# AHartmaier/pyLabFEA

Hardware: AMD Instinct MI355X
Metric: integration-point updates/sec (wall-clock per load step in ms_per_step) (higher is better)
Workload: dtype f64

## Files before the change

### include/plfx.h

```cpp
#ifndef PLFX_H
#define PLFX_H

#include <stddef.h>
#include <stdint.h>

#ifdef __cplusplus
extern "C" {
#endif

typedef struct plfx_ctx plfx_ctx;

enum {
    PLFX_ELASTIC = 0,
    PLFX_HILL6 = 1,
    PLFX_PRINC3 = 2,
    PLFX_SVC6 = 3,
    PLFX_TRESCA = 4,
    PLFX_BARLAT = 5,
    PLFX_SVC3 = 6,
    PLFX_SVC_WH = 7,
    PLFX_SVC6_COLS = 8
};

enum {
// ... 29 lines not shown
int plfx_create(int device, plfx_ctx **out);
void plfx_destroy(plfx_ctx *ctx);
const char *plfx_last_error(plfx_ctx *ctx);
const char *plfx_version(void);
int plfx_device_count(void);
int plfx_device_info(plfx_ctx *ctx, char *name, int len, int *cus, int64_t *hbm_bytes);
void *plfx_stream(plfx_ctx *ctx);
int plfx_sync(plfx_ctx *ctx);

int plfx_set_materials(plfx_ctx *ctx, int nmat, const plfx_material *mats);

int plfx_seq_batch(plfx_ctx *ctx, int mat, int n, const double *sig, double *seq);
int plfx_fgrad_batch(plfx_ctx *ctx, int mat, int n, const double *sig, double *fgrad);
int plfx_fgrad_seq_batch(plfx_ctx *ctx, int mat, int n, const double *sig, const double *seq, double *fgrad);
int plfx_yf_batch(plfx_ctx *ctx, int mat, int n, const double *sig, const double *epl, double *yf);
int plfx_full_yf_batch(plfx_ctx *ctx, int mat, int n, const double *sig, const double *epl,
                       const double *ld, double *yf, int32_t *status);
int plfx_response_batch(plfx_ctx *ctx, int n, const int32_t *mat_id, const double *sig,
                        const double *epl, const double *deps, double *fy, double *sig_out,
                        double *depl, double *ct , int32_t *nsteps);
int plfx_set_response_maxit(plfx_ctx *ctx, int maxit);
int plfx_sig_princ_host(int n, const double *sig, double *sp);
int plfx_eig3_host(int n, const double *sig, double *w, double *V);
int plfx_response_batch_kh(plfx_ctx *ctx, int n, const int32_t *mat_id, const double *sig, const double *epl,
                           const double *deps, const double *khard_in, double *fy, double *sig_out, double *depl,
                           double *ct, int32_t *nsteps, double *khard_out);
int plfx_fgrad_batch_wh(plfx_ctx *ctx, int mat, int n, const double *sig, const double *epl, double *fgrad, double *khard_raw);
int plfx_hessian_batch(plfx_ctx *ctx, int mat, int n, const double *sig, const double *epl, double *hess);
int plfx_yield_scale(plfx_ctx *ctx, int mat, int n, const double *su, const double *epl, const double *x0, double *x,
                     int32_t *status);
int plfx_flow_curve(plfx_ctx *ctx, int mat, int n, const double *su, const double *epl0, int max_steps, double depl,
                    double epl_max, double predictor, double *x, double *epl, double *yf, double *hk, int32_t *nsteps,
                    int32_t *status);
int plfx_flow_info(plfx_ctx *ctx, int64_t *launches);

int plfx_load_path(plfx_ctx *ctx, int mat, int n, int K, const double *dload, int shared, const int32_t *control,
                   const double *sig0, const double *epl0, const int32_t *tex_id, int maxit, int newton, double stol,
                   double eps_cap, double *sig, double *epl, double *deps, double *fy, int32_t *nsteps, int32_t *newton_out,
                   int32_t *ksteps, int32_t *status, double *ct);
int plfx_load_path_info(plfx_ctx *ctx, int64_t *launches);

int plfx_committee_yf(plfx_ctx *ctx, int nmem, const int32_t *mats, const double *scale, int n, const double *su, double *yf,
                      double *mean, double *var, int32_t *best, double *best_var);
int plfx_committee_info(plfx_ctx *ctx, int64_t *launches, int32_t *staged_members);

int plfx_tex_svc_set(plfx_ctx *ctx, int nsv, int tdim, const double *sv, const double *dual, double intercept, double gamma,
                     const double *mean, const double *scale, int dev_only);
int plfx_tex_svc_yf(plfx_ctx *ctx, int n, const double *sig, int ntex, const double *tex, const int32_t *tex_id, double *yf);
int plfx_tex_svc_yield_scale(plfx_ctx *ctx, int nray, const double *su, int ntex, const double *tex, const double *x0, double *x,
                             int32_t *status);
int plfx_tex_svc_info(plfx_ctx *ctx, int *nsv, int *tdim, int64_t *yf_launches, int64_t *ray_launches, int *staged);
int plfx_tex_svc_fgrad(plfx_ctx *ctx, int n, const double *sig, int ntex, const double *tex, const int32_t *tex_id, double *grad);
int plfx_tex_svc_full_yf(plfx_ctx *ctx, int n, const double *sig, int ntex, const double *tex, const int32_t *tex_id, double *f,
                         int32_t *status);
int plfx_tex_svc_response(plfx_ctx *ctx, int mat, int n, const double *sig, const double *epl, const double *deps, int ntex,
                          const double *tex, const int32_t *tex_id, int maxit, double *fy, double *sig_out, double *depl,
                          double *ct, int32_t *nsteps);
int plfx_tex_svc_flow_info(plfx_ctx *ctx, int64_t *fgrad_launches, int64_t *full_yf_launches, int64_t *response_launches);

int plfx_gen_structured(int NX, int NY, int32_t *conn, int32_t *noleft, int32_t *noright, int32_t *nobot, int32_t *notop);

int plfx_set_mesh(plfx_ctx *ctx, int nel, int nnode, const int32_t *conn, const int32_t *mat_id,
                  const double *lxy, double thick, int planestress, int el_begin, int el_end);
int plfx_set_mesh_structured(plfx_ctx *ctx, int NX, int NY, const int32_t *mat_col, const int32_t *mat_el, const double *dx_col,
                             double dy, double thick, int planestress, int el_begin, int el_end);
int plfx_pattern_selftest(int nx, int ny);
int plfx_set_grid(plfx_ctx *ctx, int nx, int ny);
int plfx_set_precond(plfx_ctx *ctx, int kind, double omega, int nu);
int plfx_precond_info(plfx_ctx *ctx, int *kind_in_use, int *levels);
int plfx_precond_apply(plfx_ctx *ctx, const double *r, double *z);
int plfx_precond_bench(plfx_ctx *ctx, int reps, double *us_per_cycle, double *us_coarse);
int plfx_solve_fallbacks(plfx_ctx *ctx, int64_t *count);
int plfx_indefinite_info(plfx_ctx *ctx, int64_t *solves, int64_t *by_minres_surrogate, int64_t *by_gmres,
                         int64_t *surrogates_built, int64_t *elements_shifted);
int plfx_set_operator(plfx_ctx *ctx, int kind);
int plfx_matvec(plfx_ctx *ctx, const double *x, double *y);
int plfx_operator_info(plfx_ctx *ctx, int *matrix_free, int *levels_matrix_free);
int plfx_reuse_info(plfx_ctx *ctx, int *assemblies, int *bc_applications, int *solves);
int plfx_predict_info(plfx_ctx *ctx, int64_t *applied, int64_t *skipped, int64_t *rejected);
int plfx_sweep_info(plfx_ctx *ctx, int64_t *sweeps, int64_t *tangents_rewritten);
int plfx_sweep_launch_info(plfx_ctx *ctx, int64_t *heavy_skipped, int64_t *heavy_recovered);
int plfx_bc_info(plfx_ctx *ctx, int64_t *rhs_rows_only, int64_t *dinv_kept, int64_t *dinv_refreshed, int64_t *du_early);
int plfx_short_info(plfx_ctx *ctx, int64_t *dinv_deferred, int64_t *dinv_formed_late, int64_t *d_kept, int64_t *spec_merged);
int plfx_dead_store_info(plfx_ctx *ctx, int64_t *armed_sweeps, int64_t *tangents_rewritten_in_armed_sweeps,
                         int64_t *test_only_starts, int64_t *test_only_retries);
enum {
    PLFX_PLANE_ON = 0,
    PLFX_PLANE_NEVER_ON = 1,
    PLFX_PLANE_SWITCH = 2,
    PLFX_PLANE_SHARDED = 3,
    PLFX_PLANE_MATERIALS = 4,
    PLFX_PLANE_STATE_SET = 5,
    PLFX_PLANE_TANGENT_SET = 6
};
int plfx_plane_info(plfx_ctx *ctx, int *mode_on, int64_t *plane_sweeps, int64_t *plane_updates, int *switched_off_by);
enum {
    PLFX_MG_TAIL_NONE = 0,
    PLFX_MG_TAIL_GENERIC = 1,
    PLFX_MG_TAIL_LDS = 2,
    PLFX_MG_TAIL_MF = 3,
    PLFX_MG_TAIL_MF_RAGGED = 4
};
enum {
    PLFX_MG_COARSE_DENSE = 0,
    PLFX_MG_COARSE_CHEBY = 1,
    PLFX_MG_COARSE_PCG = 2
};
int plfx_mg_info(plfx_ctx *ctx, int max_levels, int *levels, int *dims, double *ratios, int *matfree, int *tail_level,
                 int *tail_kernel, int *coarse_solver, int *cheby_steps, double *cheby_kappa, int *march);
int plfx_svc_info(plfx_ctx *ctx, int *row_materials, int *thread_materials, int64_t *row_launches, int64_t *thread_launches);
int plfx_get_bmat(plfx_ctx *ctx, int e, double *B);
int plfx_get_kel(plfx_ctx *ctx, int e, double *Kel);

int plfx_state_get(plfx_ctx *ctx, int which, double *out);
int plfx_state_set(plfx_ctx *ctx, int which, const double *in);
int plfx_state_reset(plfx_ctx *ctx);
int plfx_gather(plfx_ctx *ctx, int which, int n, const int32_t *idx, double *out);

enum {
    PLFX_FIELD_STRAIN1 = 0,
    PLFX_FIELD_STRAIN2 = 1,
    PLFX_FIELD_STRAIN12 = 2,
    PLFX_FIELD_STRESS1 = 3,
    PLFX_FIELD_STRESS2 = 4,
    PLFX_FIELD_STRESS12 = 5,
    PLFX_FIELD_PLASTIC1 = 6,
    PLFX_FIELD_PLASTIC2 = 7,
    PLFX_FIELD_PLASTIC12 = 8,
    PLFX_FIELD_SEQ = 9,
    PLFX_FIELD_SEQJ2 = 10,
    PLFX_FIELD_PEEQ = 11,
    PLFX_FIELD_ETOT = 12,
    PLFX_FIELD_UX = 13,
    PLFX_FIELD_UY = 14
};
int plfx_element_fields(plfx_ctx *ctx, int nsel, const int32_t *sel, double *out, double *range);

int plfx_assemble(plfx_ctx *ctx);
int plfx_get_csr(plfx_ctx *ctx, int64_t *nnz, int32_t *rowptr, int32_t *colidx, double *val);

int plfx_apply_bc(plfx_ctx *ctx, int n, const int32_t *presc_idx, const double *du_presc,
                  const double *w, const double *fext);
int plfx_set_bc_plan(plfx_ctx *ctx, int nseg, const int32_t *seg_len, const int32_t *idx);
int plfx_apply_bc_plan(plfx_ctx *ctx, const double *seg_val, const double *fext, int *inconsistent_entry);
int plfx_solve(plfx_ctx *ctx, double rtol, int maxit, int warm, int *iters, double *relres);

int plfx_sweep(plfx_ctx *ctx, int nit, int *changed, int *conv);
int plfx_set_wh_mode(plfx_ctx *ctx, int sequential);
int plfx_wh_info(plfx_ctx *ctx, int *sequential_in_use, int64_t *sweeps, int64_t *passes,
                 int64_t *unresolved );
int plfx_wh_carry(plfx_ctx *ctx, int mat, const double *set, double *get);
int plfx_scf_stats(plfx_ctx *ctx, const double *sld, double *sum, double *sumsq_c, double *minv,
                   int64_t *count, double mean_in, int pass);
int plfx_scf_all(plfx_ctx *ctx, const double *sld, int64_t *count, double *minv, double *sum, double *sumsq_c);
int plfx_update_state(plfx_ctx *ctx);
int plfx_set_finish_set(plfx_ctx *ctx, int n, const int32_t *idx);
int plfx_finish_step(plfx_ctx *ctx, double *u_at , double *f_at , double *sums18);
int plfx_global_sums(plfx_ctx *ctx, double *out18);

typedef struct plfx_step {
    int32_t il, nonlin, has_nodeset, warm, maxit;
    int32_t defer_slot;
    double rtol;
    double bcl0[2], bcb0[2];
    double max_dbcr[2], max_dbct[2], max_dbcn[2];
    double bcr[2], bct[2], bcn[2];
// ... 65 lines not shown
```

### pylabfea_amd/_lib.py

```python
import ctypes as C
import os

import numpy as np

_HERE = os.path.dirname(os.path.abspath(__file__))
LIB_PATH = os.environ.get('PLFX_LIB', os.path.join(_HERE, 'libplfx.so'))

ELASTIC, HILL6, PRINC3, SVC6, TRESCA, BARLAT, SVC3, SVC_WH, SVC6_COLS = 0, 1, 2, 3, 4, 5, 6, 7, 8

ST_SIG, ST_EPS, ST_EPL, ST_RES_SIG, ST_RES_DEPL, ST_ELSTIFF, ST_U, ST_F, ST_DU, ST_FYN, ST_MAXSTEPS, ST_KHARD = range(12)

FIELD_NAMES = ('strain1', 'strain2', 'strain12', 'stress1', 'stress2', 'stress12', 'plastic1', 'plastic2', 'plastic12',
               'seq', 'seqJ2', 'peeq', 'etot', 'ux', 'uy')
FIELD_ID = {n: i for i, n in enumerate(FIELD_NAMES)}

T_SWEEP, T_SPMV, T_CGUPD, T_ASSEMBLE, T_VCYCLE, T_SMOOTH, T_SWEEP_HEAVY, T_COMM = range(8)


class PlfxError(RuntimeError):
    pass


class CMaterial(C.Structure):
    _fields_ = [('kind', C.c_int32), ('sdim', C.c_int32), ('CV', C.c_double * 36),
                ('E', C.c_double), ('nu', C.c_double), ('sy', C.c_double), ('khard', C.c_double),
                ('hill', C.c_double * 6), ('drucker', C.c_double), ('nsv', C.c_int32),
                ('nfeat', C.c_int32), ('dev_only', C.c_int32), ('_pad', C.c_int32),
                ('gamma', C.c_double), ('intercept', C.c_double), ('scale_seq', C.c_double),
                ('sv', C.c_void_p), ('dual', C.c_void_p), ('barlat', C.c_double * 18),
                ('barlat_exp', C.c_double), ('barlat_normal', C.c_int32), ('_pad2', C.c_int32),
                ('scale_wh', C.c_double)]


SYMBOLS = [
    'plfx_create', 'plfx_destroy', 'plfx_last_error', 'plfx_version', 'plfx_device_count', 'plfx_device_info',
    'plfx_stream', 'plfx_sync', 'plfx_set_materials', 'plfx_seq_batch', 'plfx_fgrad_batch',
    'plfx_yf_batch', 'plfx_full_yf_batch', 'plfx_response_batch', 'plfx_set_mesh', 'plfx_get_bmat',
    'plfx_get_kel', 'plfx_state_get', 'plfx_state_set', 'plfx_state_reset', 'plfx_gather',
    'plfx_assemble', 'plfx_get_csr', 'plfx_apply_bc', 'plfx_solve', 'plfx_sweep', 'plfx_scf_stats',
    'plfx_update_state', 'plfx_global_sums', 'plfx_comm_unique_id', 'plfx_comm_init',
    'plfx_timing_get', 'plfx_timing_reset', 'plfx_timing_enable', 'plfx_set_grid', 'plfx_set_precond',
    'plfx_precond_info', 'plfx_set_operator', 'plfx_operator_info', 'plfx_gen_structured', 'plfx_reuse_info', 'plfx_timing_select', 'plfx_finish_fetch', 'plfx_sweep_info', 'plfx_matvec', 'plfx_set_bc_plan', 'plfx_apply_bc_plan',
    'plfx_set_finish_set', 'plfx_finish_step', 'plfx_scf_all', 'plfx_comm_info', 'plfx_comm_init_callback',
    'plfx_set_bc_sources',
    'plfx_load_step', 'plfx_set_strip', 'plfx_strip_info', 'plfx_allreduce_host',
    'plfx_response_batch_kh', 'plfx_fgrad_batch_wh', 'plfx_timing_sample', 'plfx_solve_fallbacks', 'plfx_comm_selftest',
    'plfx_indefinite_info', 'plfx_pattern_selftest', 'plfx_precond_bench', 'plfx_set_wh_mode', 'plfx_wh_info', 'plfx_wh_carry', 'plfx_set_mesh_structured',
    'plfx_svc_info', 'plfx_fgrad_seq_batch', 'plfx_precond_apply', 'plfx_predict_info',
    'plfx_set_response_maxit', 'plfx_sig_princ_host', 'plfx_eig3_host',
    'plfx_svc_fit_batch', 'plfx_svc_decision_batch', 'plfx_svc_fit_wide', 'plfx_hessian_batch',
    'plfx_svr_fit_batch', 'plfx_svr_predict_multi', 'plfx_set_svr_flow', 'plfx_svr_flow_info',
    'plfx_sweep_launch_info', 'plfx_element_fields', 'plfx_bc_info', 'plfx_yield_scale',
    'plfx_committee_yf', 'plfx_committee_info',
    'plfx_tex_svc_set', 'plfx_tex_svc_yf', 'plfx_tex_svc_yield_scale', 'plfx_tex_svc_info',
    'plfx_tex_svc_fgrad', 'plfx_tex_svc_full_yf', 'plfx_tex_svc_response', 'plfx_tex_svc_flow_info',
    'plfx_flow_curve', 'plfx_flow_info', 'plfx_load_path', 'plfx_load_path_info',
    'plfx_dead_store_info', 'plfx_plane_info', 'plfx_short_info',
    'plfx_set_svc_cols', 'plfx_mg_info',
    'plfx_set_svc_textures', 'plfx_set_element_textures', 'plfx_response_batch_tid', 'plfx_full_yf_batch_tid',
    'plfx_svc_textures_info',
]

_lib = None


def load():
    global _lib
    if _lib is not None:
        return _lib
    if not os.path.exists(LIB_PATH):
        raise PlfxError('libplfx.so not found at %s - build it first (__graft_entry__.build()); '
                        'pylabfea_amd has no CPU fallback' % LIB_PATH)
    lib = C.CDLL(LIB_PATH)
    lib.plfx_last_error.restype = C.c_char_p
    lib.plfx_version.restype = C.c_char_p
    lib.plfx_stream.restype = C.c_void_p
    lib.plfx_destroy.restype = None
    _lib = lib
    return lib


class CStep(C.Structure):
    _fields_ = [('il', C.c_int32), ('nonlin', C.c_int32), ('has_nodeset', C.c_int32), ('warm', C.c_int32),
                ('maxit', C.c_int32), ('defer_slot', C.c_int32), ('rtol', C.c_double),
                ('bcl0', C.c_double * 2), ('bcb0', C.c_double * 2),
                ('max_dbcr', C.c_double * 2), ('max_dbct', C.c_double * 2), ('max_dbcn', C.c_double * 2),
                ('bcr', C.c_double * 2), ('bct', C.c_double * 2), ('bcn', C.c_double * 2),
                ('bcr0', C.c_double * 2), ('bct0', C.c_double * 2), ('bcn0', C.c_double * 2),
                ('sld', C.c_double * 6),
                ('dbcr', C.c_double * 2), ('dbct', C.c_double * 2), ('dbcn', C.c_double * 2),
                ('scale_bc', C.c_double),
                ('nit', C.c_int32), ('nconv', C.c_int32), ('nsweeps', C.c_int32), ('nsolves', C.c_int32),
                ('soft_fail', C.c_int32), ('inconsistent_entry', C.c_int32),
                ('its', C.c_int32 * 40), ('relres', C.c_double * 40)]


def device_count():
    return int(load().plfx_device_count())


def _dp(a):
    return a.ctypes.data_as(C.c_void_p) if a is not None else None


def _f64(a):
    return np.ascontiguousarray(a, dtype=np.float64)


def _i32(a):
    return np.ascontiguousarray(a, dtype=np.int32)


def gen_structured(NX, NY):
    lib = load()
    conn = np.empty((NX * NY, 4), dtype=np.int32)
    le, ri = np.empty(NY + 1, dtype=np.int32), np.empty(NY + 1, dtype=np.int32)
    bo, to = np.empty(NX + 1, dtype=np.int32), np.empty(NX + 1, dtype=np.int32)
    rc = lib.plfx_gen_structured(int(NX), int(NY), _dp(conn), _dp(le), _dp(ri), _dp(bo), _dp(to))
    if rc:
        raise PlfxError('plfx_gen_structured(%d, %d): error %d' % (NX, NY, rc))
    return conn, le, ri, bo, to


def sig_princ_host(sig):
    lib = load()
    s = _f64(sig).reshape(-1, 6)
    sp = np.empty((len(s), 3))
    rc = lib.plfx_sig_princ_host(len(s), _dp(s), _dp(sp))
    if rc < 0:
        raise PlfxError('plfx_sig_princ_host: error %d' % rc)
    return sp


def eig3_host(sig):
    lib = load()
    s = _f64(sig).reshape(-1, 6)
    w, V = np.empty((len(s), 3)), np.empty((len(s), 3, 3))
    rc = lib.plfx_eig3_host(len(s), _dp(s), _dp(w), _dp(V))
    if rc < 0:
        raise PlfxError('plfx_eig3_host: error %d' % rc)
# ... 514 lines not shown
            try:
                return self.response(sig, epl, deps, mat_id, khard_in, return_khard, tex_id=tex_id)
            finally:
                self.set_response_maxit(50)
        sig = _f64(sig).reshape(-1, 6)
        n = len(sig)
        epl = _f64(epl).reshape(-1, 6)
        deps = _f64(deps).reshape(-1, 6)
        mid = None if mat_id is None else _i32(mat_id)
        fy = np.empty(n)
        so = np.empty((n, 6))
        dp = np.empty((n, 6))
        ct = np.empty((n, 36))
        ns = np.empty(n, dtype=np.int32)
        if khard_in is not None or return_khard:
            kin = None if khard_in is None else _f64(np.broadcast_to(np.asarray(khard_in, dtype=float), (n,)).copy())
            kout = np.empty(n)
            self._chk(self.lib.plfx_response_batch_kh(self.h, n, _dp(mid), _dp(sig), _dp(epl), _dp(deps), _dp(kin),
                                                      _dp(fy), _dp(so), _dp(dp), _dp(ct), _dp(ns), _dp(kout)))
            if return_khard:
                return fy, so, dp, ct, ns, kout
            return fy, so, dp, ct, ns
        if tex_id is not None:
            tid = _i32(tex_id).reshape(-1)
            if len(tid) != n:
                raise ValueError('response: one texture row per point expected')
            self._chk(self.lib.plfx_response_batch_tid(self.h, n, _dp(mid), _dp(sig), _dp(epl), _dp(deps),
                                                       _dp(fy), _dp(so), _dp(dp), _dp(ct), _dp(ns), _dp(tid)))
            return fy, so, dp, ct, ns
        self._chk(self.lib.plfx_response_batch(self.h, n, _dp(mid), _dp(sig), _dp(epl), _dp(deps),
                                               _dp(fy), _dp(so), _dp(dp), _dp(ct), _dp(ns)))
        return fy, so, dp, ct, ns

    def set_mesh(self, conn, mat_id, lxy, nnode, thick, planestress, el_begin=0, el_end=None):
        conn = _i32(conn).reshape(-1, 4)
        nel = len(conn)
        mat_id = _i32(mat_id)
        lxy = _f64(lxy).reshape(nel, 2)
        if el_end is None:
            el_end = nel
        self._chk(self.lib.plfx_set_mesh(self.h, nel, int(nnode), _dp(conn), _dp(mat_id), _dp(lxy),
                                         C.c_double(thick), int(bool(planestress)), int(el_begin),
                                         int(el_end)))
        self.nel = nel
        self.nel_owned = el_end - el_begin
        self.ndof = 2 * int(nnode)

    def set_mesh_structured(self, NX, NY, dx_col, dy, thick, planestress, mat_col=None, mat_el=None, el_begin=0, el_end=None):
        nel = int(NX) * int(NY)
        dx = _f64(dx_col).reshape(int(NX))
        mc = None if mat_col is None else _i32(mat_col).reshape(int(NX))
        me = None if mat_el is None else _i32(mat_el).reshape(nel)
        if el_end is None:
            el_end = nel
        self._chk(self.lib.plfx_set_mesh_structured(self.h, int(NX), int(NY), _dp(mc), _dp(me), _dp(dx), C.c_double(dy),
                                                    C.c_double(thick), int(bool(planestress)), int(el_begin), int(el_end)))
        self.nel = nel
        self.nel_owned = el_end - el_begin
        self.ndof = 2 * (int(NX) + 1) * (int(NY) + 1)

    def set_grid(self, nx, ny):
        self._chk(self.lib.plfx_set_grid(self.h, int(nx), int(ny)))

    def sweep_info(self):
        a, b = C.c_int64(), C.c_int64()
        self._chk(self.lib.plfx_sweep_info(self.h, C.byref(a), C.byref(b)))
        return a.value, b.value

    def sweep_launch_info(self):
        a, b = C.c_int64(), C.c_int64()
        self._chk(self.lib.plfx_sweep_launch_info(self.h, C.byref(a), C.byref(b)))
        return a.value, b.value

    def bc_info(self):
        a, b, r, d = C.c_int64(), C.c_int64(), C.c_int64(), C.c_int64()
        self._chk(self.lib.plfx_bc_info(self.h, C.byref(a), C.byref(b), C.byref(r), C.byref(d)))
        return a.value, b.value, r.value, d.value

    def short_info(self):
        a, b, r, d = C.c_int64(), C.c_int64(), C.c_int64(), C.c_int64()
        self._chk(self.lib.plfx_short_info(self.h, C.byref(a), C.byref(b), C.byref(r), C.byref(d)))
        return a.value, b.value, r.value, d.value

    def dead_store_info(self):
        a, b, r, d = C.c_int64(), C.c_int64(), C.c_int64(), C.c_int64()
        self._chk(self.lib.plfx_dead_store_info(self.h, C.byref(a), C.byref(b), C.byref(r), C.byref(d)))
        return a.value, b.value, r.value, d.value

    PLANE_OFF_REASONS = ('on', 'no state reset yet', 'switch', 'sharded', 'materials', 'state_set', 'tangent set')

    def plane_info(self):
        on, a, b, why = C.c_int(), C.c_int64(), C.c_int64(), C.c_int()
        self._chk(self.lib.plfx_plane_info(self.h, C.byref(on), C.byref(a), C.byref(b), C.byref(why)))
        return bool(on.value), a.value, b.value, why.value

    MG_TAIL_KERNELS = ('none', 'tail', 'tail_lds', 'tail_mf', 'tail_mf_ragged')
    MG_COARSE_SOLVERS = ('dense', 'cheby', 'pcg')

    def mg_info(self):
        cap = 64
        nl, tl, tk, cs, st, ma = (C.c_int() for _ in range(6))
        kap = C.c_double()
        dims, rat, mf = np.zeros((cap, 2), dtype=np.int32), np.zeros((cap, 2)), np.zeros(cap, dtype=np.int32)
        self._chk(self.lib.plfx_mg_info(self.h, cap, C.byref(nl), _dp(dims), _dp(rat), _dp(mf), C.byref(tl), C.byref(tk),
                                        C.byref(cs), C.byref(st), C.byref(kap), C.byref(ma)))
        n = min(nl.value, cap)
        return {'levels': [(int(dims[l, 0]), int(dims[l, 1]), float(rat[l, 0]), float(rat[l, 1]), bool(mf[l])) for l in range(n)],
                'tail_level': tl.value, 'tail_kernel': self.MG_TAIL_KERNELS[tk.value],
                'coarse_solver': self.MG_COARSE_SOLVERS[cs.value], 'cheby_steps': st.value, 'cheby_kappa': kap.value,
                'march': bool(ma.value)}

    def svc_info(self):
        a, b, r, t = C.c_int(), C.c_int(), C.c_int64(), C.c_int64()
        self._chk(self.lib.plfx_svc_info(self.h, C.byref(a), C.byref(b), C.byref(r), C.byref(t)))
        return a.value, b.value, r.value, t.value

    def reuse_info(self):
        a, b, s = C.c_int(), C.c_int(), C.c_int()
        self._chk(self.lib.plfx_reuse_info(self.h, C.byref(a), C.byref(b), C.byref(s)))
        return a.value, b.value, s.value

    def predict_info(self):
        a, b, r = C.c_int64(), C.c_int64(), C.c_int64()
        self._chk(self.lib.plfx_predict_info(self.h, C.byref(a), C.byref(b), C.byref(r)))
        return a.value, b.value, r.value

    def set_precond(self, kind, omega=0., nu=0):
        self._chk(self.lib.plfx_set_precond(self.h, int(kind), C.c_double(omega), int(nu)))

    def precond_info(self):
        k = C.c_int()
        lv = C.c_int()
        self._chk(self.lib.plfx_precond_info(self.h, C.byref(k), C.byref(lv)))
        return k.value, lv.value

    def precond_apply(self, r):
        r = _f64(r).reshape(-1)
        z = np.empty_like(r)
        self._chk(self.lib.plfx_precond_apply(self.h, _dp(r), _dp(z)))
        return z

    def precond_bench(self, reps=100):
        a, b = C.c_double(), C.c_double()
        self._chk(self.lib.plfx_precond_bench(self.h, int(reps), C.byref(a), C.byref(b)))
        return a.value, b.value

    def set_wh_mode(self, sequential):
        self._chk(self.lib.plfx_set_wh_mode(self.h, 1 if sequential else 0))

    def wh_info(self):
        a, b, c_, u = C.c_int(), C.c_int64(), C.c_int64(), C.c_int64()
        self._chk(self.lib.plfx_wh_info(self.h, C.byref(a), C.byref(b), C.byref(c_), C.byref(u)))
        self.wh_unresolved = u.value
        return bool(a.value), b.value, c_.value

    def wh_unresolved_sweeps(self):
        self.wh_info()
        return self.wh_unresolved

    def wh_carry(self, mat, value=None):
        g = C.c_double()
        sv = None if value is None else C.byref(C.c_double(float(value)))
        self._chk(self.lib.plfx_wh_carry(self.h, int(mat), sv, C.byref(g)))
        return g.value

    def solve_fallbacks(self):
# ... 246 lines not shown
```

### pylabfea_amd/csrc/plfx.hip

```cpp
#define PLFX_UNIT_CONTEXT
#define PLFX_UNIT_MESH
#define PLFX_UNIT_OPERATOR
#include "plfx_host.hpp"
#include "plfx_mg.hpp"

namespace plfx {
namespace host {

typedef struct { char internal[128]; } ncclUniqueId;
typedef int (*fn_ncclGetUniqueId)(ncclUniqueId *);
typedef int (*fn_ncclCommInitRank)(ncclComm_t *, int, ncclUniqueId, int);
typedef int (*fn_ncclAllReduce)(const void *, void *, size_t, int, int, ncclComm_t, hipStream_t);
typedef int (*fn_ncclCommDestroy)(ncclComm_t);
typedef int (*fn_ncclSend)(const void *, size_t, int, int, ncclComm_t, hipStream_t);
typedef int (*fn_ncclRecv)(void *, size_t, int, int, ncclComm_t, hipStream_t);
typedef int (*fn_ncclGroup)(void);
struct Rccl {
    void *h = nullptr;
    fn_ncclGetUniqueId GetUniqueId = nullptr;
    fn_ncclCommInitRank CommInitRank = nullptr;
    fn_ncclAllReduce AllReduce = nullptr;
    fn_ncclCommDestroy CommDestroy = nullptr;
    fn_ncclSend Send = nullptr;
    fn_ncclRecv Recv = nullptr;
// ... 383 lines not shown
    dfree(c->eps);
    dfree(c->res_sig);
    dfree(c->res_depl);
    dfree(c->fld_buf);
    dfree(c->fld_part);
    c->fld_cap = 0;
    tan_free(c);
    dfree(c->Mel);
    dfree(c->fyn);
    dfree(c->scf_hh);
    dfree(c->kh_el);
    dfree(c->kh_out); dfree(c->kh_new); dfree(c->wh_snap_el); dfree(c->wh_snap_M); dfree(c->wh_snap_ms);
    dfree(c->kh_touch); dfree(c->wh_bmax); dfree(c->wh_cnt);
    c->kh_out_valid = false;
    dfree(c->max_steps);
    dfree(c->scf_mult);
    dfree(c->heavy_list);
    dfree(c->u);
    dfree(c->f);
    dfree(c->du);
    dfree(c->rhs);
    dfree(c->dinv);
    dfree(c->diag);
    dfree(c->is_presc);
    dfree(c->dup);
    dfree(c->wv);
    dfree(c->fext);
    dfree(c->x);
    dfree(c->r);
    dfree(c->z);
    dfree(c->q);
    dfree(c->pred_x);
    dfree(c->pred_d);
    c->pred_valid = c->pred_d_kept = false;
    for (auto &b : c->gm_blk) dfree(b);
    c->gm_blk.clear();
    c->gm_m = 0;
    dfree(c->gm_part);
    dfree(c->gm_part2);
    dfree(c->gm_red);
    dfree(c->gm_coef);
    dfree(c->p[0]);
    dfree(c->p[1]);
    for (auto &L : c->mg) {
        if (!L.owned) continue;
        dfree(L.col);
        dfree(L.contrib);
        dfree(L.cls0);
        dfree(L.val);
        dfree(L.diag);
        dfree(L.dinv);
        dfree(L.Mel);
        dfree(L.x);
        dfree(L.b);
    }
    for (auto &L : c->mg) {
        dfree(L.t);
        dfree(L.res);
        dfree(L.ainv);
    }
    c->mg.clear();
    dfree(c->mg_cls);
    dfree(c->mg_dev);
    dfree(c->dtab);
    dfree(c->Mop);
    dfree(c->colr);
    c->grid_ok = false;
    c->val_valid = false;
    c->mg_tail = -1;
    c->gx = c->gy = 0;
    c->assembled = c->bc_set = false;
    c->M_dirty = true;
    c->x_is_du = false;
    c->bc_valid = false;
    c->bc_idx.clear();
    c->plan.valid = false;
    dfree(c->fin_idx);
    dfree(c->fin_dev);
    c->fin_n = 0;
    dfree(c->kw);
    dfree(c->bc_rows);
    c->bc_nrows = 0;
    c->rhs_rows_ok = c->dinv_ok = c->dinv_late = false;
    dfree(c->tex_ids);
    c->htex_ids.clear();
    c->tex_ids_ok = false;
}

int ensure_tmp(plfx_ctx *c, size_t n)
{
    if (n <= c->tmp_cap) return 0;
    dfree(c->idx_tmp);
    dfree(c->val_tmp);
    int rc = dalloc(c, &c->idx_tmp, n);
    if (rc) return rc;
    rc = dalloc(c, &c->val_tmp, 4 * n);
    if (rc) return rc;
    c->tmp_cap = n;
    return 0;
}

int march_env()
{
    static const int v = getenv("PLFX_MARCH") ? atoi(getenv("PLFX_MARCH")) : -1;
    return v;
}
bool march_pcg(const plfx_ctx *c) { return matfree(c) && march_env() != 0 && !c->op.colr; }
bool march_mg(const plfx_ctx *c)
{
    if (!matfree(c) || march_env() == 0) return false;
    return march_env() == 1 || (size_t)c->nnode * 112 > ((size_t)192 << 20);
}
bool tail_mf(const plfx_ctx *c)
{
    return matfree(c) && c->mg_tail_T > 0 && c->mg_tail_E > 0 && c->mg_nu == 2 && !c->mg.empty() && c->mg.back().ainv;
}

void launch_spmv_plain(plfx_ctx *c, const double *in, double *out, CgScalars *sc)
{
    LAUNCH_OP2(k_spmv, 0, matfree(c), dim3(c->grid_nodes), c->op, 0, c->nnode, (const double2 *)in, nullptr, nullptr,
               (double2 *)out, nullptr, nullptr, nullptr, 0, nullptr, sc, 0, 0, 0);
}

int plain_spmv(plfx_ctx *c, const double *in, double *out)
{
    launch_spmv_plain(c, in, out, nullptr);
    HIPCHK(c, hipGetLastError());
    return 0;
}

int allreduce(plfx_ctx *c, void *dev, size_t count, int nccl_dtype, int nccl_op, const char *what)
{
    c->last_coll = what;
    c->n_coll++;
    if (c->comm) {
        EvPair *ev;
        tim_begin(c, 7, &ev);
        const int rcn = g_rccl.AllReduce(dev, dev, count, nccl_dtype, nccl_op, c->comm, c->stream);
        tim_end(c, ev);
        if (rcn != 0) return fail(c, PLFX_ERR_HIP, "ncclAllReduce(%s) failed", what);
        return 0;
    }
    if (c->host_ar) {
        const size_t bytes = count * (nccl_dtype == NCCL_INT32 ? 4 : 8);
        if (c->host_ar_buf.size() < bytes) c->host_ar_buf.resize(bytes);
        HIPCHK(c, hipMemcpyAsync(c->host_ar_buf.data(), dev, bytes, hipMemcpyDeviceToHost, c->stream));
        HIPCHK(c, stream_sync(c));
        if (c->host_ar(c->host_ar_user, c->host_ar_buf.data(), count, nccl_dtype == NCCL_INT32 ? 1 : 0,
                       nccl_op == NCCL_MIN ? 3 : 0) != 0)
            return fail(c, PLFX_ERR_HIP, "host all-reduce callback failed (%s)", what);
        HIPCHK(c, hipMemcpyAsync(dev, c->host_ar_buf.data(), bytes, hipMemcpyHostToDevice, c->stream));
        HIPCHK(c, stream_sync(c));
        return 0;
    }
    return 0;
}

int sync_M(plfx_ctx *c)
{
    if (!comm_active(c) || !c->sharded) return 0;
    if (c->strip.on) return strip_sync_M(c);
    hipLaunchKernelGGL(k_zero_foreign_M, dim3(grid_for((size_t)6 * c->nel_total)), dim3(BLOCK), 0, c->stream,
                       c->nel_total, c->e0, c->e0 + c->nel, c->Mel);
    HIPCHK(c, hipGetLastError());
    return allreduce(c, c->Mel, (size_t)6 * c->nel_total, NCCL_FLOAT64, NCCL_SUM, "M");
}


bool strip_coll(const plfx_ctx *c)
{
    static const bool force = getenv("PLFX_STRIP_FORCE_COLL") && atoi(getenv("PLFX_STRIP_FORCE_COLL")) != 0;
    return c->nranks > 1 || (force && (c->comm || c->host_ar));
}

int part_allreduce(plfx_ctx *c, double *p, size_t n)
{
    if (!c->strip.on || !strip_coll(c)) return 0;
    c->strip.n_part++;
    return allreduce(c, p, n, NCCL_FLOAT64, NCCL_SUM, "partial sums");
}

int halo_refresh(plfx_ctx *c, double *v)
{
    auto &S = c->strip;
    if (!S.on || !strip_coll(c)) return 0;
    const int nyn = c->gy + 1;
    const size_t n = (size_t)S.W * nyn * 2;
    double *sendL = v + (size_t)2 * (S.oc0 + 1) * nyn, *recvL = v + (size_t)2 * (S.oc0 - S.W) * nyn;
    double *sendR = v + (size_t)2 * (S.oc1 - S.W) * nyn, *recvR = v + (size_t)2 * (S.oc1 + 1) * nyn;
    S.n_halo++;
    c->last_coll = "halo refresh (ncclSend / ncclRecv with the strip neighbours)";
    c->n_coll++;
    if (c->comm) {
        if (!g_rccl.Send || !g_rccl.Recv || !g_rccl.GroupStart || !g_rccl.GroupEnd)
            return fail(c, PLFX_ERR_UNSUPPORTED, "this RCCL has no ncclSend/ncclRecv");
        EvPair *ev;
        tim_begin(c, 7, &ev);
        int rc = g_rccl.GroupStart();
        if (!rc && S.has_left) {
            rc = g_rccl.Send(sendL, n, NCCL_FLOAT64, c->rank - 1, c->comm, c->stream);
            if (!rc) rc = g_rccl.Recv(recvL, n, NCCL_FLOAT64, c->rank - 1, c->comm, c->stream);
        }
        if (!rc && S.has_right) {
            rc = g_rccl.Send(sendR, n, NCCL_FLOAT64, c->rank + 1, c->comm, c->stream);
            if (!rc) rc = g_rccl.Recv(recvR, n, NCCL_FLOAT64, c->rank + 1, c->comm, c->stream);
        }
        const int rc2 = g_rccl.GroupEnd();
        tim_end(c, ev);
        if (rc || rc2) return fail(c, PLFX_ERR_HIP, "halo refresh (ncclSend/ncclRecv) failed: %d / %d", rc, rc2);
        return 0;
    }
    if (c->host_ar) {
        S.hbuf.assign(2 * n, 0.);
        if (S.has_left) HIPCHK(c, hipMemcpyAsync(S.hbuf.data(), sendL, 8 * n, hipMemcpyDeviceToHost, c->stream));
        if (S.has_right) HIPCHK(c, hipMemcpyAsync(S.hbuf.data() + n, sendR, 8 * n, hipMemcpyDeviceToHost, c->stream));
        HIPCHK(c, stream_sync(c));
        if (c->host_ar(c->host_ar_user, S.hbuf.data(), 2 * n, 0, 100) != 0)
            return fail(c, PLFX_ERR_HIP, "host halo-exchange callback failed");
        if (S.has_left) HIPCHK(c, hipMemcpyAsync(recvL, S.hbuf.data(), 8 * n, hipMemcpyHostToDevice, c->stream));
        if (S.has_right) HIPCHK(c, hipMemcpyAsync(recvR, S.hbuf.data() + n, 8 * n, hipMemcpyHostToDevice, c->stream));
        HIPCHK(c, stream_sync(c));
    }
    return 0;
}

int strip_sync_M(plfx_ctx *c)
{
    auto &S = c->strip;
    if (!S.on || !strip_coll(c)) return 0;
    const int ny = c->gy;
    const size_t n = (size_t)S.W * ny, tot = (size_t)c->nel_total;
    double *M = c->Mel;
    const size_t sL = (size_t)S.oc0 * ny, rL = (size_t)(S.oc0 - S.W) * ny, sR = (size_t)(S.oc1 - S.W) * ny, rR = (size_t)S.oc1 * ny;
    S.n_gen++;
    c->last_coll = "stiffness generators of the halo columns (ncclSend / ncclRecv with the strip neighbours)";
    c->n_coll++;
    if (c->comm) {
        if (!g_rccl.Send || !g_rccl.Recv || !g_rccl.GroupStart || !g_rccl.GroupEnd)
            return fail(c, PLFX_ERR_UNSUPPORTED, "this RCCL has no ncclSend/ncclRecv");
        EvPair *ev;
        tim_begin(c, 7, &ev);
        int rc = g_rccl.GroupStart();
        for (int k = 0; k < 6 && !rc; k++) {
            if (S.has_left) {
                rc = g_rccl.Send(M + k * tot + sL, n, NCCL_FLOAT64, c->rank - 1, c->comm, c->stream);
                if (!rc) rc = g_rccl.Recv(M + k * tot + rL, n, NCCL_FLOAT64, c->rank - 1, c->comm, c->stream);
            }
            if (!rc && S.has_right) {
                rc = g_rccl.Send(M + k * tot + sR, n, NCCL_FLOAT64, c->rank + 1, c->comm, c->stream);
                if (!rc) rc = g_rccl.Recv(M + k * tot + rR, n, NCCL_FLOAT64, c->rank + 1, c->comm, c->stream);
            }
        }
        const int rc2 = g_rccl.GroupEnd();
        tim_end(c, ev);
        if (rc || rc2) return fail(c, PLFX_ERR_HIP, "generator halo exchange (ncclSend/ncclRecv) failed: %d / %d", rc, rc2);
        return 0;
    }
    if (c->host_ar) {
        S.hbuf.assign(12 * n, 0.);
        for (int k = 0; k < 6; k++) {
            if (S.has_left) HIPCHK(c, hipMemcpyAsync(S.hbuf.data() + k * n, M + k * tot + sL, 8 * n, hipMemcpyDeviceToHost, c->stream));
            if (S.has_right) HIPCHK(c, hipMemcpyAsync(S.hbuf.data() + (6 + k) * n, M + k * tot + sR, 8 * n, hipMemcpyDeviceToHost, c->stream));
        }
        HIPCHK(c, stream_sync(c));
        if (c->host_ar(c->host_ar_user, S.hbuf.data(), 12 * n, 0, 100) != 0)
            return fail(c, PLFX_ERR_HIP, "host halo-exchange callback failed (generators)");
        for (int k = 0; k < 6; k++) {
            if (S.has_left) HIPCHK(c, hipMemcpyAsync(M + k * tot + rL, S.hbuf.data() + k * n, 8 * n, hipMemcpyHostToDevice, c->stream));
            if (S.has_right) HIPCHK(c, hipMemcpyAsync(M + k * tot + rR, S.hbuf.data() + (6 + k) * n, 8 * n, hipMemcpyHostToDevice, c->stream));
        }
        HIPCHK(c, stream_sync(c));
    }
    return 0;
}


KOp make_op(const plfx_ctx *c, int nnode, int nslot, const int32_t *col, const double *val, int nx, int ny, int nel,
            const double *M, double rx, double ry)
{
    KOp o;
    o.rx = rx;
    o.ry = ry;
    o.nnode = nnode;
    o.nslot = nslot;
    o.col = col;
    o.val = val;
    o.nxn = nx + 1;
    o.nyn = ny + 1;
    o.nel = nel;
    o.M = M;
    o.tab = c->dtab;
    return o;
}

int ensure_dinv(plfx_ctx *c)
{
    if (!c->dinv_late) return 0;
    hipLaunchKernelGGL(k_dinv, dim3(grid_for(c->ndof)), dim3(BLOCK), 0, c->stream, (size_t)c->ndof, c->diag, c->is_presc, c->dinv);
    HIPCHK(c, hipGetLastError());
    c->dinv_late = false;
    c->n_dinv_late++;
    return 0;
}

int assemble_fine_val(plfx_ctx *c)
{
    if (int rc = ensure_dinv(c)) return rc;
    hipLaunchKernelGGL(k_assemble, dim3(grid_for(c->nnode), c->nslot), dim3(BLOCK), 0, c->stream,
                       c->dcls, c->ncls, c->nnode, c->nslot, c->nq, c->nel_total, c->dcontrib, c->dcls_all,
                       (matfree(c) && c->assembled) ? c->Mop : c->Mel, c->dcol, c->dval, c->diag,
                       (matfree(c) && c->assembled) ? 1 : 0);
    HIPCHK(c, hipGetLastError());
    c->dinv_ok = false;
    c->val_valid = true;
    return 0;
}

static bool level_from_generators(const plfx_ctx *c, int l)
{
    return matfree(c) && (c->mg[l].matfree || (tail_mf(c) && l < (int)c->mg.size() - 1));
}

int mg_assemble(plfx_ctx *c)
{
    const bool mf = matfree(c);
    const int nl = (int)c->mg.size();
    c->mg_dinv_current = mf && c->bc_valid;
    for (int l = 1; l < nl; l++) {
        auto &F = c->mg[l - 1];
        auto &L = c->mg[l];
        if (!(mf && (F.matfree || tail_mf(c))) || !level_plain(F))
            hipLaunchKernelGGL(k_mg_coarsen_M, dim3(grid_for(L.nel)), dim3(BLOCK), 0, c->stream, L.nx, L.ny, F.ny,
                               F.nel, (l == 1 && mf) ? c->mg[0].op.M : F.Mel, L.Mel, mf ? 1 : 0, mf ? 1 : 0, F.rx, F.ry);
        const bool setup_mf = level_from_generators(c, l);
        if (setup_mf)
            LAUNCH_SETUP(1, L.op, (double2 *)L.diag,
                               (double *)nullptr, (l + 1 < nl && level_plain(L)) ? c->mg[l + 1].Mel : (double *)nullptr,
                               (const double2 *)c->dinv, c->mg[0].ny + 1, l,
                               c->mg_dinv_current ? (double2 *)L.dinv : (double2 *)nullptr, c->mg[0].nx + 1);
        else
            hipLaunchKernelGGL(k_assemble, dim3(grid_for(L.nnode), L.nslot), dim3(BLOCK), 0, c->stream, L.cls4 ? L.cls4 : c->mg_cls,
                               L.cls4 ? 4 : 1, L.nnode, L.nslot, L.nq, L.nel, L.contrib, L.cls0, L.Mel, L.col, L.val, L.diag, mf ? 1 : 0);
    }
    HIPCHK(c, hipGetLastError());
    c->mg_inv_valid = false;
    return 0;
}

int mg_update_dinv(plfx_ctx *c, bool same_set)
{
    for (size_t l = 1; l < c->mg.size(); l++) {
        auto &F = c->mg[l - 1];
        auto &L = c->mg[l];
        if (same_set && c->mg_dinv_current && matfree(c) && (L.matfree || (tail_mf(c) && l + 1 < c->mg.size())))
            continue;
        hipLaunchKernelGGL(k_mg_coarse_dinv, dim3(grid_for(L.nnode)), dim3(BLOCK), 0, c->stream, L.nx + 1,
                           L.ny + 1, F.ny + 1, (const double2 *)F.dinv, (const double2 *)L.diag,
                           (double2 *)L.dinv, F.nx + 1, F.rx, F.ry);
    }
    auto &Lc = c->mg.back();
    if (Lc.ainv && !(c->mg_inv_valid && same_set)) {
        const int n = 2 * Lc.nnode;
        hipLaunchKernelGGL(k_mg_coarse_invert, dim3(1), dim3(BLOCK), (size_t)n * n * sizeof(double), c->stream,
                           Lc.nnode, Lc.nslot, Lc.col, Lc.val, (const double2 *)Lc.dinv, Lc.ainv);
        c->mg_inv_valid = true;
    }
    HIPCHK(c, hipGetLastError());
    return 0;
}

inline int level_nu(const plfx_ctx *c, int l)
{
    static const int nc = getenv("PLFX_MG_NU_COARSE") ? atoi(getenv("PLFX_MG_NU_COARSE")) : 0;
    return (nc > 0 && l >= 2 && !c->strip.on) ? nc : c->mg_nu;
}

int mg_down_level(plfx_ctx *c, int l)
{
    const double om = c->mg_omega;
    auto &L = c->mg[l];
    auto &C = c->mg[l + 1];
    const bool mf = L.matfree && matfree(c);
    const int nu = level_nu(c, l);
    EvPair *ev = nullptr;
    (void)ev;
    const bool march = l == 0 && mf && march_mg(c);
    if (nu == 2) {
        if (march)
            hipLaunchKernelGGL(k_mg_smooth2_zero_march, dim3(L.grid), dim3(BLOCK), 0, c->stream, L.op, (const double2 *)L.dinv,
                               (const double2 *)L.b, (double2 *)L.x, om, c->sc);
        else if (l == 0)
            LAUNCH_OP2(k_mg_smooth2_zero, 1, mf, dim3(L.grid), L.op, (const double2 *)L.dinv, (const double2 *)L.b,
                       (double2 *)L.x, om, c->sc);
        else
            LAUNCH_OP2R(k_mg_smooth2_zero, 0, mf, L.op, dim3(L.grid), L.op, (const double2 *)L.dinv, (const double2 *)L.b,
                       (double2 *)L.x, om, c->sc);
    } else {
        double *src = nullptr, *dst = (nu & 1) ? L.x : L.t;
        for (int k = 0; k < nu; k++) {
            if (l == 0)
                LAUNCH_OP2(k_mg_smooth, 1, mf, dim3(L.grid), L.op, (const double2 *)L.dinv, (const double2 *)L.b,
                           (const double2 *)src, (double2 *)dst, om, k == 0, c->sc);
            else
                LAUNCH_OP2R(k_mg_smooth, 0, mf, L.op, dim3(L.grid), L.op, (const double2 *)L.dinv, (const double2 *)L.b,
                           (const double2 *)src, (double2 *)dst, om, k == 0, c->sc);
            src = dst;
            dst = (dst == L.x) ? L.t : L.x;
        }
    }
// ... 292 lines not shown
    return rc;
}

int strip_child_dinv(plfx_ctx *c)
{
    auto &S = c->strip;
    plfx_ctx *k = S.child;
    auto &L = c->mg[S.Ld];
    const StripWin w = strip_window(c);
    const size_t nyc = L.ny + 1;
    const size_t nd = (size_t)2 * k->nnode;
    hipLaunchKernelGGL(k_strip_pack, dim3(grid_for(nd)), dim3(BLOCK), 0, c->stream, 1, nd, (size_t)2 * L.nnode,
                       (size_t)2 * (w.g0 + w.jc0) * nyc, (size_t)2 * (w.jc1 - w.jc0) * nyc, (size_t)2 * w.jc0 * nyc,
                       (const double *)L.dinv, k->dinv);
    HIPCHK(c, hipGetLastError());
    if (strip_coll(c)) {
        const int rc = allreduce(c, k->dinv, nd, NCCL_FLOAT64, NCCL_SUM, "coarse Jacobi scaling");
        if (rc) return rc;
    }
    k->mg_inv_valid = false;
    const int rc = mg_update_dinv(k, false);
    if (rc) c->err = k->err;
    return rc;
}

void strip_free(plfx_ctx *c)
{
    mg_graph_drop(c);
    plfx_ctx *k = c->strip.child;
    if (k) {
        mg_graph_drop(k);
        dfree(k->Mel);
        dfree(k->Mop);
        dfree(k->diag);
        dfree(k->dinv);
        dfree(k->r);
        dfree(k->z);
        for (auto &L : k->mg) {
            if (L.owned) {
                dfree(L.col); dfree(L.contrib); dfree(L.cls0); dfree(L.val); dfree(L.diag); dfree(L.dinv);
                dfree(L.Mel); dfree(L.x); dfree(L.b);
            }
            dfree(L.t); dfree(L.res); dfree(L.ainv); dfree(L.cls4);
        }
        dfree(k->mg_cls);
        dfree(k->mg_dev);
        delete k;
    }
    c->strip = plfx_ctx::Strip();
}

void plane_off(plfx_ctx *c, int why)
{
    if (c->plane_cols) c->plane_off_by = why;
    c->plane_cols = false;
}

void launch_jacobi_z(plfx_ctx *c)
{
    hipLaunchKernelGGL(k_jacobi_z, dim3(grid_for(c->nnode)), dim3(BLOCK), 0, c->stream, c->nnode, (const double2 *)c->dinv,
                       (const double2 *)c->r, (double2 *)c->z, c->sc);
}

void launch_mbox_post(plfx_ctx *c, const double *src, int n, double *dst, CgMbox *mb, unsigned long long seq)
{
    hipLaunchKernelGGL(k_mbox_post, dim3(1), dim3(BLOCK), 0, c->stream, src, n, dst, mb, seq);
}

void launch_kdu_uf(plfx_ctx *c, CgScalars *spec)
{
    LAUNCH_OP2(k_spmv, 3, matfree(c), dim3(c->grid_nodes), c->op, 0, c->nnode, (const double2 *)c->du, nullptr, (double2 *)c->u,
               (double2 *)c->f, nullptr, nullptr, nullptr, 0, nullptr, spec, 0, 0, 0);
}

void launch_spec_setup(plfx_ctx *c)
{
    KOp live = c->op;
    live.M = c->Mel;
    LAUNCH_SETUP(0, live, (double2 *)c->diag,
                       c->Mop, (mg_active(c) && level_plain(c->mg[0])) ? c->mg[1].Mel : (double *)nullptr, (const double2 *)nullptr, 0, 0,
                       (double2 *)nullptr, 0x7fffffff, (const int *)(c->flags + 8));
}

}
}

extern "C" {

const char *plfx_version(void) { return PLFX_VERSION; }

int plfx_create(int device, plfx_ctx **out)
{
    if (!out) return PLFX_ERR_ARG;
    *out = nullptr;
    plfx_ctx *c = new plfx_ctx();
    *out = c;
    c->device = device;
    int ndev = 0;
    hipError_t e = hipGetDeviceCount(&ndev);
    if (e != hipSuccess || ndev == 0)
        return fail(c, PLFX_ERR_HIP, "no HIP device available (%s); libplfx has no CPU fallback",
                    hipGetErrorString(e));
    HIPCHK(c, hipSetDevice(device));
    HIPCHK(c, hipGetDeviceProperties(&c->prop, device));
    HIPCHK(c, hipStreamCreateWithFlags(&c->stream, hipStreamNonBlocking));
    if (const char *e2 = getenv("PLFX_MATFREE")) c->want_matfree = atoi(e2) ? 1 : 0;
    if (const char *e3 = getenv("PLFX_SVC_WAVE")) c->want_svc_wave = atoi(e3) ? 1 : 0;
    if (const char *e4 = getenv("PLFX_COLL_TIMEOUT")) c->coll_timeout_s = atof(e4);
    if (const char *e4 = getenv("PLFX_MG_GRAPH")) c->want_mg_graph = atoi(e4) ? 1 : 0;
    if (const char *e8 = getenv("PLFX_REUSE")) c->reuse = atoi(e8) != 0;
    if (const char *e9 = getenv("PLFX_BC_ROWS")) c->bc_rows_on = atoi(e9) != 0;
    if (const char *e10 = getenv("PLFX_DEAD_STORES")) {
        const int v = atoi(e10);
        c->dead_stores = v == 1 || v == 2;
        c->test_starts = v == 1 || v == 3;
    }
    if (!c->reuse) c->dead_stores = c->test_starts = false;
    if (const char *e11 = getenv("PLFX_PLANE_COLS")) c->plane_switch = atoi(e11) != 0;
    if (!c->reuse) c->plane_switch = false;
    if (const char *e12 = getenv("PLFX_SHORT_SOLVE")) c->short_solve = atoi(e12) & 3;
    if (!c->reuse) c->short_solve = 0;
    if (const char *e9 = getenv("PLFX_PREDICT")) c->predict = atoi(e9) != 0;
    {
        const char *e5 = getenv("PLFX_MAILBOX");
        if (!e5 || atoi(e5)) {
            if (hipHostMalloc((void **)&c->mbox, sizeof(CgMbox), hipHostMallocMapped | hipHostMallocCoherent) == hipSuccess)
                memset(c->mbox, 0, sizeof(CgMbox));
            else
                c->mbox = nullptr;
            c->mb_cap = 1 << 16;
            if (c->mbox && hipHostMalloc((void **)&c->mb_buf, (size_t)8 * c->mb_cap,
                                         hipHostMallocMapped | hipHostMallocCoherent) != hipSuccess) {
                c->mb_buf = nullptr;
                c->mb_cap = 0;
            }
        }
    }
    size_t lds = std::max((size_t)c->prop.sharedMemPerBlock, (size_t)c->prop.maxSharedMemoryPerMultiProcessor);
    lds = std::min(lds, (size_t)160 * 1024);
    const size_t reserve = sizeof(MatDev) * MAXMAT + sizeof(ClassDev) * MAXCLS + 1024;
    c->lds_doubles = lds > reserve ? (int)((lds - reserve) / 8) : 0;
    int rc;
    if ((rc = dalloc(c, &c->part, (size_t)8 * MAXPART))) return rc;
    if ((rc = dalloc(c, &c->part_g, (size_t)18 * SUMPART))) return rc;
    if ((rc = dalloc(c, &c->sc, 1))) return rc;
    if ((rc = dalloc(c, &c->flags, 16))) return rc;
    if ((rc = dalloc(c, &c->spec_sc, 1))) return rc;
    if ((rc = dalloc(c, &c->bflags, (size_t)2 * SWEEP_SLOTS))) return rc;
    if ((rc = dalloc(c, &c->small, 64))) return rc;
    HIPCHK(c, stream_sync(c));
    return PLFX_OK;
}

void plfx_destroy(plfx_ctx *c)
{
    if (!c) return;
    if (c->stream) stream_sync(c);
#ifdef PLFX_PROF_REGIONS
    {
        unsigned long long h[16] = {0};
        if (prof_regions_add_step(h) && prof_regions_add_material(h) && h[7]) {
            static const char *nm[8] = {"fgrad", "plain", "ray_sample pass", "ray_sample post", "march", "brentq", "full() in corrector", "corrector loop"};
            for (int i = 0; i < 8; i++) fprintf(stderr, "[prof] %-22s %14llu ticks  %5.1f %% of the corrector loop\n", nm[i], h[i], 100. * h[i] / h[7]);
            fprintf(stderr, "[prof] rows: ray searches %llu, direct evaluations %llu (no polynomial %llu, outside its interval %llu, inside the margin %llu), of the outside ones: below lo %llu, at brentq iterates %llu, at the start point %llu\n",
                    h[8], h[9], h[10], h[11], h[12], h[13], h[14], h[15]);
        }
    }
#endif
    if (c->comm && g_rccl.CommDestroy) g_rccl.CommDestroy(c->comm);
    for (auto &e : c->tim.ring) {
        hipEventDestroy(e.a);
        hipEventDestroy(e.b);
    }
    free_mesh(c);
    free_materials(c);
    dfree(c->tex_sv);
    dfree(c->tex_dual);
    dfree(c->part);
    dfree(c->part_g);
    dfree(c->sc);
    dfree(c->flags);
    dfree(c->spec_sc);
    dfree(c->bflags);
    dfree(c->small);
    dfree(c->idx_tmp);
    dfree(c->val_tmp);
    if (c->stage) hipHostFree(c->stage);
    for (int h = 0; h < 2; h++)
        if (c->stage_ev[h]) hipEventDestroy(c->stage_ev[h]);
    dfree(c->bc_idx_dev);
    dfree(c->plan.seg4);
    dfree(c->bc_rows);
    dfree(c->kw);
    dfree(c->fin_idx);
    dfree(c->fin_dev);
    if (c->fin_host) hipHostFree(c->fin_host);
    for (int q = 0; q < 2; q++) {
        if (c->fin_pin[q]) hipHostFree(c->fin_pin[q]);
        if (c->fin_box[q]) hipHostFree(c->fin_box[q]);
    }
    if (c->mbox) hipHostFree(c->mbox);
    if (c->mb_buf) hipHostFree(c->mb_buf);
    if (c->stream) hipStreamDestroy(c->stream);
    delete c;
// ... 181 lines not shown
        HIPCHK(c, hipMemcpyAsync(c->dcol, c->hcol.data(), c->hcol.size() * 4, hipMemcpyHostToDevice, c->stream));
        HIPCHK(c, hipMemcpyAsync(c->dcontrib, hcontrib.data(), hcontrib.size() * 4, hipMemcpyHostToDevice, c->stream));
    }
    HIPCHK(c, stream_sync(c));
    c->grid_nodes = grid_xcd(nnode);
    c->grid_el = grid_xcd(nown);
    if (const char *cap = getenv("PLFX_SWEEP_BLOCKS"))
        if (atoi(cap) > 0 && c->grid_el > atoi(cap)) c->grid_el = atoi(cap);
    c->grid_ok = false;
    c->val_valid = false;
    c->op = make_op(c, nnode, nslot, c->dcol, c->dval, 0, 0, nel, c->Mel);
    return plfx_state_reset(c);
}

int plfx_set_mesh(plfx_ctx *c, int nel, int nnode, const int32_t *conn, const int32_t *mat_id,
                  const double *lxy, double thick, int planestress, int el_begin, int el_end)
{
    return set_mesh_impl(c, nel, nnode, conn, mat_id, lxy, thick, planestress, el_begin, el_end, nullptr);
}

int plfx_set_mesh_structured(plfx_ctx *c, int NX, int NY, const int32_t *mat_col, const int32_t *mat_el, const double *dx_col, double dy,
                             double thick, int planestress, int el_begin, int el_end)
{
    if (!c) return PLFX_ERR_STATE;
    if (NX < 1 || NY < 1 || (!mat_col && !mat_el) || !dx_col || (int64_t)(NX + 1) * (NY + 1) > INT32_MAX)
        return fail(c, PLFX_ERR_ARG, "bad structured mesh description");
    const int nel = NX * NY, nyn = NY + 1;
    std::vector<int32_t> conn((size_t)4 * nel), mid((size_t)nel);
    std::vector<double> lxy((size_t)2 * nel);
    bool uniform = true;
    for (int j = 0; j < NX; j++) {
        const double dx = dx_col[j];
        if (std::fabs(dx - dx_col[0]) > 1e-12 * std::fabs(dx_col[0])) uniform = false;
        const int32_t mc = mat_col ? mat_col[j] : 0;
        if (mat_col && (mc < 0 || mc >= c->nmat)) return fail(c, PLFX_ERR_ARG, "mat_col[%d] out of range", j);
        int32_t *q = conn.data() + (size_t)4 * j * NY;
        double *l = lxy.data() + (size_t)2 * j * NY;
        int32_t *m = mid.data() + (size_t)j * NY;
        const int32_t *me = mat_el ? mat_el + (size_t)j * NY : nullptr;
        const int n0 = j * nyn;
        for (int k = 0; k < NY; k++) {
            const int n1 = n0 + k;
            q[4 * k] = n1;
            q[4 * k + 1] = n1 + 1;
            q[4 * k + 2] = n1 + nyn;
            q[4 * k + 3] = n1 + nyn + 1;
            l[2 * k] = dx;
            l[2 * k + 1] = dy;
            m[k] = me ? me[k] : mc;
            if (me && (me[k] < 0 || me[k] >= c->nmat)) return fail(c, PLFX_ERR_ARG, "mat_el[%d] out of range", j * NY + k);
        }
    }
    const StructHint hint{NX, NY, uniform};
    return set_mesh_impl(c, nel, (NX + 1) * nyn, conn.data(), mid.data(), lxy.data(), thick, planestress, el_begin, el_end, &hint);
}

int plfx_get_bmat(plfx_ctx *c, int e, double *B)
{
    if (!c || c->hcls.empty()) return c ? fail(c, PLFX_ERR_STATE, "set_mesh first") : PLFX_ERR_STATE;
    if (e < 0 || e >= c->nel_total || !B) return fail(c, PLFX_ERR_ARG, "bad argument");
    const ClassDev &k = c->hcls[c->hcls_id[e]];
    for (int g = 0; g < 4; g++) {
        double x, y, bx[4], by[4];
        gauss_point(k.lx, k.ly, g, &x, &y);
        shape_b(k.lx, k.ly, x, y, bx, by);
        double *Bg = B + 48 * g;
        for (int i = 0; i < 48; i++) Bg[i] = 0.;
        for (int a = 0; a < 4; a++) {
            Bg[0 * 8 + 2 * a] = bx[a];
            Bg[1 * 8 + 2 * a + 1] = by[a];
            Bg[5 * 8 + 2 * a] = by[a];
            Bg[5 * 8 + 2 * a + 1] = bx[a];
            Bg[2 * 8 + 2 * a] = k.kappa * bx[a];
            Bg[2 * 8 + 2 * a + 1] = k.kappa * by[a];
        }
    }
    return PLFX_OK;
}

int plfx_get_kel(plfx_ctx *c, int e, double *Kel)
{
    if (!c || !c->Mel) return c ? fail(c, PLFX_ERR_STATE, "set_mesh first") : PLFX_ERR_STATE;
    if (e < c->e0 || e >= c->e0 + c->nel || !Kel) return fail(c, PLFX_ERR_ARG, "element not owned");
    double M[6];
    for (int k = 0; k < 6; k++)
        HIPCHK(c, hipMemcpy(&M[k], c->Mel + (size_t)k * c->nel_total + e, 8, hipMemcpyDeviceToHost));
    const ClassDev &k = c->hcls[c->hcls_id[e]];
    for (int a = 0; a < 4; a++)
        for (int b = 0; b < 4; b++) {
            const double sxx = k.Sxx[a * 4 + b], sxy = k.Sxy[a * 4 + b], syx = k.Sxy[b * 4 + a], syy = k.Syy[a * 4 + b];
            Kel[(2 * a) * 8 + 2 * b] = M[0] * sxx + M[2] * (sxy + syx) + M[5] * syy;
            Kel[(2 * a) * 8 + 2 * b + 1] = M[1] * sxy + M[2] * sxx + M[4] * syy + M[5] * syx;
            Kel[(2 * a + 1) * 8 + 2 * b] = M[1] * syx + M[4] * syy + M[2] * sxx + M[5] * sxy;
            Kel[(2 * a + 1) * 8 + 2 * b + 1] = M[3] * syy + M[4] * (syx + sxy) + M[5] * sxx;
        }
    return PLFX_OK;
}

static int build_hierarchy(plfx_ctx *c, int nx, int ny, const ClassDev &geom)
{
    int rc;
    std::vector<std::pair<int, int>> dims;
    dims.push_back({nx, ny});
    static const long long coarsest = getenv("PLFX_MG_COARSEST_ELEMS") ? atoll(getenv("PLFX_MG_COARSEST_ELEMS")) : 4;
    const int odd_mode = getenv("PLFX_MG_ODD") ? atoi(getenv("PLFX_MG_ODD")) : 1;
    const bool finest_odd = ((nx | ny) & 1) && (long long)(nx + 1) * (ny + 1) > 150000 && c->want_matfree;
    std::vector<std::pair<double, double>> ratio;
    ratio.push_back({1., 1.});
    for (;;) {
        const int fx = dims.back().first, fy = dims.back().second;
        const double rx = ratio.back().first, ry = ratio.back().second;
        const long long ne = (long long)fx * fy;
        const bool plain = fx % 2 == 0 && fy % 2 == 0 && rx == 1. && ry == 1.;
        const bool big = (long long)(fx + 1) * (fy + 1) > MG_COARSE_MAX;
        if (!(ne > 4 && (ne > coarsest || dims.size() < 2))) break;
        if (!plain && !((odd_mode == 1 || (odd_mode == 2 && finest_odd)) && (big || rx != 1. || ry != 1.) && fx >= 2 && fy >= 2)) break;
        if (plain) {
            ratio.push_back({1., 1.});
            dims.push_back({fx / 2, fy / 2});
        } else {
            ratio.push_back({mg_coarse_ratio(fx, rx), mg_coarse_ratio(fy, ry)});
            dims.push_back({mg_coarse_cells(fx, rx), mg_coarse_cells(fy, ry)});
        }
    }
    if (dims.size() < 2) return PLFX_OK;
    if (!c->mg_cls) {
        if ((rc = dalloc(c, &c->mg_cls, 1))) return rc;
        HIPCHK(c, hipMemcpyAsync(c->mg_cls, &geom, sizeof(ClassDev), hipMemcpyHostToDevice, c->stream));
        HIPCHK(c, stream_sync(c));
    }
    c->mg.resize(dims.size());
    for (size_t l = 0; l < dims.size(); l++) {
        auto &L = c->mg[l];
        L.nx = dims[l].first;
        L.ny = dims[l].second;
        L.rx = ratio[l].first;
        L.ry = ratio[l].second;
        L.nnode = (L.nx + 1) * (L.ny + 1);
        L.nel = L.nx * L.ny;
        L.grid = grid_xcd(L.nnode);
        if ((rc = dalloc(c, &L.t, (size_t)2 * L.nnode))) return rc;
        if ((rc = dalloc(c, &L.res, (size_t)2 * L.nnode))) return rc;
        if (l == 0) {
            L.owned = false;
            L.nslot = c->nslot;
            L.nq = c->nq;
            L.col = c->dcol;
            L.val = c->dval;
            L.diag = c->diag;
            L.dinv = c->dinv;
            L.Mel = c->Mel;
            L.nel = c->nel_total;
            L.x = c->z;
            L.b = c->r;
            continue;
        }
        L.owned = true;
        std::vector<int32_t> conn, hcol, hcontrib;
        const bool closed = L.nx >= 2 && L.ny >= 2 && !(getenv("PLFX_PATTERN_CLOSED_FORM") && atoi(getenv("PLFX_PATTERN_CLOSED_FORM")) == 0);
        if (closed) {
            L.nslot = 9;
            L.nq = 4;
        } else {
            conn.resize((size_t)4 * L.nel);
            const int nr = L.ny + 1;
            for (int e = 0; e < L.nel; e++) {
// ... 49 lines not shown
            if ((rc = dalloc(c, &Lc.ainv, (size_t)n * n))) return rc;
            HIPCHK(c, set_dyn_lds((const void *)k_mg_coarse_invert, n * n * (int)sizeof(double)));
        }
    }
    c->mg_cheby = 0;
    const bool small_coarsest = c->mg.back().nnode <= MG_COARSE_MAX;
    if (small_coarsest) {
        const int lds = c->mg.back().nnode * 4 * (int)sizeof(double2);
        HIPCHK(c, set_dyn_lds((const void *)k_mg_coarse_solve, lds));
        HIPCHK(c, set_dyn_lds((const void *)k_mg_tail, lds));
    }
    {
        std::vector<MgLevDev> hd(c->mg.size());
        c->mg_tail = -1;
        for (size_t l = 0; l < c->mg.size(); l++) {
            auto &L = c->mg[l];
            if (c->mg_tail < 0 && l > 0 && L.nnode <= MG_TAIL_NODES) c->mg_tail = (int)l;
            int off = 0;
            if (c->mg_tail >= 0)
                for (size_t m = c->mg_tail; m < l; m++) off += c->mg[m].nnode;
            int eoff = 0;
            if (c->mg_tail >= 0)
                for (size_t m = c->mg_tail; m < l; m++) eoff += c->mg[m].nel;
            hd[l] = MgLevDev{L.nx, L.ny, L.nnode, L.nslot, L.ainv, off, 0, L.col, L.val, (const double2 *)L.dinv,
                             (double2 *)L.x, (double2 *)L.b, (double2 *)L.t, (double2 *)L.res, L.Mel, L.nel, eoff, L.rx, L.ry};
        }
        c->mg_tail_T = 0;
        if (c->mg_tail >= 0 && c->mg.back().ainv && c->mg_nu == 2) {
            int T = 0;
            bool ok = true;
            for (size_t m = c->mg_tail; m < c->mg.size(); m++) {
                T += c->mg[m].nnode;
                ok = ok && c->mg[m].nslot <= 9;
            }
            const size_t bytes = (size_t)T * (4 * sizeof(double2) + 9 * sizeof(int));
            if (ok && bytes <= 150 * 1024) {
                c->mg_tail_T = T;
                HIPCHK(c, set_dyn_lds((const void *)k_mg_tail_lds, (int)bytes));
            }
            int E = 0;
            for (size_t m = c->mg_tail; m + 1 < c->mg.size(); m++) E += c->mg[m].nel;
            const size_t bytes_mf = (size_t)T * 3 * sizeof(double2) + (size_t)E * 6 * sizeof(double);
            c->mg_tail_lds = bytes_mf;
            c->mg_tail_E = 0;
            if (c->grid_ok && bytes_mf <= 154 * 1024 && E > 0 && c->mg.size() <= 16) {
                c->mg_tail_E = E;
                HIPCHK(c, set_dyn_lds((const void *)k_mg_tail_mf<false>, (int)bytes_mf));
                HIPCHK(c, set_dyn_lds((const void *)k_mg_tail_mf<true>, (int)bytes_mf));
            }
        }
        {
            const int nl = (int)c->mg.size();
            const int lt = (c->mg_tail > 0) ? c->mg_tail : nl - 1;
            c->mg_cheby = 0;
            if (!c->mg.back().ainv && lt == nl - 1) {
                const int n = std::max(c->mg.back().nx, c->mg.back().ny);
                c->mg_cheby = std::min(std::max(n, 16), 160);
                c->mg_cheby_kappa = std::max(4., 0.5 * (double)n * n);
                if (const char *e6 = getenv("PLFX_MG_CHEBY")) c->mg_cheby = std::max(0, atoi(e6));
                if (const char *e7 = getenv("PLFX_MG_CHEBY_KAPPA")) c->mg_cheby_kappa = std::max(1.5, atof(e7));
            }
            for (int l = 0; l < nl; l++) {
                auto &L = c->mg[l];
                L.op = make_op(c, L.nnode, L.nslot, L.col, L.val, L.nx, L.ny, L.nel, l == 0 ? c->Mop : L.Mel, L.rx, L.ry);
                L.matfree = l < lt || (c->mg_cheby > 0 && l == nl - 1);
            }
            if (c->mg_cheby == 0 && c->mg.back().nnode > MG_COARSE_MAX) c->precond = 0;
        }
        dfree(c->mg_dev);
        if ((rc = dalloc(c, &c->mg_dev, hd.size()))) return rc;
        HIPCHK(c, hipMemcpyAsync(c->mg_dev, hd.data(), hd.size() * sizeof(MgLevDev), hipMemcpyHostToDevice, c->stream));
        HIPCHK(c, stream_sync(c));
    }
    return PLFX_OK;
}

int plfx_set_grid(plfx_ctx *c, int nx, int ny)
{
    if (!c || !c->dval) return c ? fail(c, PLFX_ERR_STATE, "set_mesh first") : PLFX_ERR_STATE;
    if (nx < 1 || ny < 1 || (long long)nx * ny != c->nel_total || (long long)(nx + 1) * (ny + 1) != c->nnode)
        return fail(c, PLFX_ERR_ARG, "grid %dx%d does not match the mesh", nx, ny);
    if (c->strip.on)
        return fail(c, PLFX_ERR_STATE, "plfx_set_grid after plfx_set_strip: call plfx_set_mesh again");
    const int nrow = ny + 1;
    const bool known = c->hint_nx == nx && c->hint_ny == ny;
    for (int e = 0; e < c->nel_total && !known; e++) {
        const int n1 = (e / ny) * nrow + e % ny;
        const int32_t *q = &c->hconn[4 * (size_t)e];
        if (q[0] != n1 || q[1] != n1 + 1 || q[2] != n1 + nrow || q[3] != n1 + nrow + 1)
            return fail(c, PLFX_ERR_ARG, "connectivity of element %d is not the structured numbering", e);
    }
    c->gx = nx;
    c->gy = ny;
    mg_graph_drop(c);
    for (auto &L : c->mg) {
        if (L.owned) {
            dfree(L.col); dfree(L.contrib); dfree(L.cls0); dfree(L.val); dfree(L.diag); dfree(L.dinv);
            dfree(L.Mel); dfree(L.x); dfree(L.b);
        }
        dfree(L.t); dfree(L.res); dfree(L.ainv); dfree(L.cls4);
    }
    c->mg.clear();
    c->grid_ok = false;
    c->op = make_op(c, c->nnode, c->nslot, c->dcol, c->dval, 0, 0, c->nel_total, c->Mel);
    dfree(c->colr);
    c->colr = nullptr;
    bool uniform = known && c->hint_uniform;
    if (!uniform) {
        uniform = true;
        bool columns = true;
        std::vector<double> cr(nx, 1.);
        const double lx0 = c->hlxy[0], ly0 = c->hlxy[1];
        double rmin = 1., rmax = 1.;
        for (int e = 0; e < c->nel_total && columns; e++) {
            const double lx = c->hlxy[2 * (size_t)e], ly = c->hlxy[2 * (size_t)e + 1];
            const int j = e / ny;
            if (std::fabs(ly - ly0) > 1e-12 * std::fabs(ly0)) columns = false;
            if (e % ny == 0) {
                cr[j] = (std::fabs(lx - lx0) > 1e-12 * std::fabs(lx0)) ? lx / lx0 : 1.;
                if (cr[j] != 1.) uniform = false;
                rmin = std::min(rmin, cr[j]);
                rmax = std::max(rmax, cr[j]);
            } else if (std::fabs(lx - c->hlxy[2 * (size_t)(j * ny)]) > 1e-12 * std::fabs(lx0))
                columns = false;
        }
        if (!columns) return PLFX_OK;
        if (!uniform) {
            if (!(rmin > 0.) || rmax / rmin > 1.5) return PLFX_OK;
            int rc0;
            if ((rc0 = dalloc(c, &c->colr, (size_t)nx))) return rc0;
            HIPCHK(c, hipMemcpyAsync(c->colr, cr.data(), (size_t)8 * nx, hipMemcpyHostToDevice, c->stream));
            HIPCHK(c, stream_sync(c));
            c->colr_ratio = rmax / rmin;
        }
    }
    int rc;
    {
        double tab[64];
        const ClassDev &g = c->hcls[0];
        for (int pj = 0; pj < 2; pj++)
            for (int pk = 0; pk < 2; pk++) {
                const int a = (1 - pj) * 2 + (1 - pk), p = pj * 2 + pk;
                for (int b = 0; b < 4; b++) {
                    tab[p * 16 + b * 4 + 0] = g.Sxx[a * 4 + b];
                    tab[p * 16 + b * 4 + 1] = g.Syy[a * 4 + b];
                    tab[p * 16 + b * 4 + 2] = g.Sxy[a * 4 + b];
                    tab[p * 16 + b * 4 + 3] = g.Sxy[b * 4 + a];
                }
            }
        if (!c->dtab && (rc = dalloc(c, &c->dtab, 64))) return rc;
        HIPCHK(c, hipMemcpyAsync(c->dtab, tab, sizeof(tab), hipMemcpyHostToDevice, c->stream));
        HIPCHK(c, stream_sync(c));
        if ((rc = dalloc(c, &c->Mop, (size_t)6 * c->nel_total))) return rc;
        c->op = make_op(c, c->nnode, c->nslot, c->dcol, c->dval, nx, ny, c->nel_total, c->Mop);
        c->op.colr = c->colr;
        c->grid_ok = true;
    }
    if ((rc = build_hierarchy(c, nx, ny, c->hcls[0]))) return rc;
    c->assembled = false, c->M_dirty = true;
    return PLFX_OK;
}

int plfx_set_strip(plfx_ctx *c, int own_col0, int own_col1, int global_col0, int global_nx, int coarse_level)
{
    if (!c || !c->dval) return c ? fail(c, PLFX_ERR_STATE, "set_mesh / set_grid first") : PLFX_ERR_STATE;
    if (!c->grid_ok || !c->want_matfree || c->mg.size() < 2)
        return fail(c, PLFX_ERR_UNSUPPORTED, "a strip needs the uniform structured grid (matrix-free operator + multigrid)");
    if (c->colr) return fail(c, PLFX_ERR_UNSUPPORTED, "a strip needs element columns of one width");
    const int nx = c->gx, ny = c->gy, Ld = coarse_level;
    if (c->sharded && (c->e0 != own_col0 * ny || c->nel != (own_col1 - own_col0) * ny))
        return fail(c, PLFX_ERR_STATE, "the owned element range of plfx_set_mesh must be the owned columns of the strip (or the whole local mesh)");
    if (Ld < 1 || Ld >= (int)c->mg.size())
        return fail(c, PLFX_ERR_ARG, "coarse level %d outside 1..%d of the local hierarchy", Ld, (int)c->mg.size() - 1);
    const int al = 1 << Ld;
    if (own_col0 < 0 || own_col1 > nx || own_col0 >= own_col1) return fail(c, PLFX_ERR_ARG, "bad owned column range");
    const bool hl = own_col0 > 0, hr = own_col1 < nx;
    const int W = hl ? own_col0 : (hr ? nx - own_col1 : 0);
    if ((hl && own_col0 != W) || (hr && nx - own_col1 != W)) return fail(c, PLFX_ERR_ARG, "halo widths of the two sides differ");
    if ((own_col0 | own_col1 | global_col0 | global_nx | ny | W | nx) & (al - 1))
        return fail(c, PLFX_ERR_ARG, "columns, halo and NY must be multiples of 2^level = %d", al);
    if (global_col0 < 0 || global_col0 + nx > global_nx) return fail(c, PLFX_ERR_ARG, "local grid outside the global one");
    if ((hl != (global_col0 + own_col0 > 0)) || (hr != (global_col0 + own_col1 < global_nx)))
        return fail(c, PLFX_ERR_ARG, "a halo is needed exactly on the interior sides of the strip");
    if ((hl || hr) && own_col1 - own_col0 < W) return fail(c, PLFX_ERR_ARG, "owned width %d below the halo width %d", own_col1 - own_col0, W);
    if ((hl || hr) && c->nranks < 2) return fail(c, PLFX_ERR_STATE, "interior strip edges need a communicator (plfx_comm_init*)");
    if (c->mg_nu != 2) return fail(c, PLFX_ERR_UNSUPPORTED, "the validity widths of a strip are worked out for V(2,2)");
    if (hl || hr) {
        std::vector<int> a(Ld + 1);
        int v = W;
        for (int l = 0; l < Ld; l++) {
            a[l] = std::min(v, (W >> l) - 1);
            v = (a[l] - 3) >= 0 ? (a[l] - 3) / 2 : -1;
        }
        int g = W >> Ld;
        for (int l = Ld - 1; l >= 0 && v >= 0; l--) g = std::min(a[l] - 1, 2 * g) - 2;
        if (v < 0 || g < 1)
            return fail(c, PLFX_ERR_ARG, "halo of %d columns is too narrow for coarse level %d (need 4 * 2^level: 32 for level 3, 64 for level 4)", W, Ld);
    }
    mg_graph_drop(c);
    strip_free(c);
    auto &S = c->strip;
    for (size_t l = Ld + 1; l < c->mg.size(); l++) {
        auto &L = c->mg[l];
        if (L.owned) {
            dfree(L.col); dfree(L.contrib); dfree(L.cls0); dfree(L.val); dfree(L.diag); dfree(L.dinv);
            dfree(L.Mel); dfree(L.x); dfree(L.b);
        }
        dfree(L.t); dfree(L.res); dfree(L.ainv); dfree(L.cls4);
    }
    c->mg.resize(Ld + 1);
    dfree(c->mg.back().ainv);
    c->mg_tail = -1;
    c->mg_tail_T = c->mg_tail_E = 0;
    c->mg_cheby = 0;
    c->precond = 1;
    for (auto &L : c->mg) L.matfree = true;
    S.oc0 = own_col0;
    S.oc1 = own_col1;
    S.W = W;
    S.Ld = Ld;
    S.gcol0 = global_col0;
    S.gnx = global_nx;
    S.has_left = hl;
    S.has_right = hr;
    const int nyn = ny + 1;
    S.own_lo = own_col0 * nyn;
    S.own_hi = (hr ? own_col1 : nx + 1) * nyn;
    S.eown_lo = c->sharded ? 0 : own_col0 * ny;
    S.eown_hi = c->sharded ? c->nel : own_col1 * ny;
    plfx_ctx *k = new plfx_ctx();
    S.child = k;
    k->is_child = true;
    k->device = c->device;
    k->stream = c->stream;
    k->prop = c->prop;
    k->sc = c->sc;
    k->dtab = c->dtab;
    k->want_matfree = 1;
    k->want_mg_graph = c->want_mg_graph;
    k->mg_omega = c->mg_omega;
    k->mg_nu = c->mg_nu;
    k->gx = global_nx >> Ld;
    k->gy = ny >> Ld;
    k->nel_total = k->nel = k->gx * k->gy;
    k->nnode = (k->gx + 1) * (k->gy + 1);
    k->ndof = 2 * k->nnode;
    int rc;
#define KALLOC(ptr, n)                               \
    if ((rc = dalloc(c, &(ptr), (size_t)(n)))) {     \
        strip_free(c);                               \
        return rc;                                   \
    }
    KALLOC(k->Mel, (size_t)6 * k->nel_total);
    KALLOC(k->Mop, (size_t)6 * k->nel_total);
    KALLOC(k->diag, k->ndof);
    KALLOC(k->dinv, k->ndof);
    KALLOC(k->r, k->ndof);
    KALLOC(k->z, k->ndof);
#undef KALLOC
    k->grid_ok = true;
    k->grid_nodes = grid_xcd(k->nnode);
    k->op = make_op(k, k->nnode, 0, nullptr, nullptr, k->gx, k->gy, k->nel_total, k->Mop);
    rc = build_hierarchy(k, k->gx, k->gy, c->hcls[0]);
    if (rc || !mg_active(k)) {
        if (!rc) rc = fail(c, PLFX_ERR_UNSUPPORTED, "the global coarse grid %d x %d has no usable hierarchy", k->gx, k->gy);
        else c->err = k->err;
        strip_free(c);
        return rc;
    }
    S.on = true;
    c->grid_nodes = MAXPART;
    c->assembled = false, c->M_dirty = true;
    c->bc_set = false;
    c->bc_valid = false;
    c->rhs_rows_ok = c->dinv_ok = false;
    c->dinv_late = c->pred_d_kept = false;
    c->x_is_du = false;
    c->memo.valid = false;
    return PLFX_OK;
}

int plfx_strip_info(plfx_ctx *c, int *active, int *halo, int *coarse_level, int *coarse_levels, int64_t *halo_refreshes,
                    int64_t *coarse_gathers, int64_t *partial_allreduces, int64_t *generator_exchanges)
{
    if (!c) return PLFX_ERR_ARG;
    const auto &S = c->strip;
    if (active) *active = S.on ? 1 : 0;
    if (halo) *halo = S.W;
    if (coarse_level) *coarse_level = S.Ld;
    if (coarse_levels) *coarse_levels = S.child ? (int)S.child->mg.size() : 0;
    if (halo_refreshes) *halo_refreshes = S.n_halo;
    if (coarse_gathers) *coarse_gathers = S.n_coarse;
    if (partial_allreduces) *partial_allreduces = S.n_part;
    if (generator_exchanges) *generator_exchanges = S.n_gen;
    return PLFX_OK;
}

int plfx_allreduce_host(plfx_ctx *c, double *buf, int n, int op)
{
    if (!c || !c->small) return PLFX_ERR_STATE;
    if (!buf || n < 0 || n > 32 || (op != 0 && op != 3)) return fail(c, PLFX_ERR_ARG, "n must be in 0..32, op 0 (sum) or 3 (min)");
    if (n == 0 || !comm_active(c)) return PLFX_OK;
    HIPCHK(c, hipMemcpyAsync(c->small, buf, (size_t)8 * n, hipMemcpyHostToDevice, c->stream));
    const int rc = allreduce(c, c->small, n, NCCL_FLOAT64, op == 3 ? NCCL_MIN : NCCL_SUM, "host scalars");
    if (rc) return rc;
    HIPCHK(c, hipMemcpyAsync(buf, c->small, (size_t)8 * n, hipMemcpyDeviceToHost, c->stream));
    HIPCHK(c, stream_sync(c));
    return PLFX_OK;
}

int plfx_set_operator(plfx_ctx *c, int kind)
{
    if (!c) return PLFX_ERR_ARG;
    if (kind != 0 && kind != 1) return fail(c, PLFX_ERR_ARG, "operator kind must be 0 (assembled) or 1 (matrix-free)");
    if (c->strip.on && kind != 1) return fail(c, PLFX_ERR_UNSUPPORTED, "a strip (plfx_set_strip) runs the matrix-free operator only");
    if (kind != c->want_matfree) {
        mg_graph_drop(c);
        c->want_matfree = kind;
        c->assembled = false, c->M_dirty = true;
        c->bc_set = false;
    }
    return PLFX_OK;
}

int plfx_operator_info(plfx_ctx *c, int *matrix_free, int *levels_matrix_free)
{
    if (!c) return PLFX_ERR_ARG;
    if (matrix_free) *matrix_free = matfree(c) ? 1 : 0;
    if (levels_matrix_free) {
        int n = 0;
        if (matfree(c))
            for (auto &L : c->mg) n += L.matfree ? 1 : 0;
        *levels_matrix_free = n;
    }
    return PLFX_OK;
}

int plfx_sweep_info(plfx_ctx *c, int64_t *sweeps, int64_t *tangents_rewritten)
{
    if (!c) return PLFX_ERR_ARG;
    if (sweeps) *sweeps = c->n_sweeps;
    if (tangents_rewritten) *tangents_rewritten = c->n_tangents_rewritten;
    return PLFX_OK;
}

int plfx_bc_info(plfx_ctx *c, int64_t *rhs_rows_only, int64_t *dinv_kept, int64_t *dinv_refreshed, int64_t *du_early)
{
    if (!c) return PLFX_ERR_ARG;
    if (rhs_rows_only) *rhs_rows_only = c->n_rhs_rows;
    if (dinv_kept) *dinv_kept = c->n_dinv_kept;
    if (dinv_refreshed) *dinv_refreshed = c->n_dinv_refreshed;
    if (du_early) *du_early = c->n_du_early;
    return PLFX_OK;
}

int plfx_short_info(plfx_ctx *c, int64_t *dinv_deferred, int64_t *dinv_formed_late, int64_t *d_kept, int64_t *spec_merged)
{
    if (!c) return PLFX_ERR_ARG;
    if (dinv_deferred) *dinv_deferred = c->n_dinv_deferred;
    if (dinv_formed_late) *dinv_formed_late = c->n_dinv_late;
    if (d_kept) *d_kept = c->n_d_kept;
    if (spec_merged) *spec_merged = 0;
    return PLFX_OK;
}

int plfx_dead_store_info(plfx_ctx *c, int64_t *armed_sweeps, int64_t *tangents_rewritten_in_armed_sweeps, int64_t *test_only_starts,
                         int64_t *test_only_retries)
{
    if (!c) return PLFX_ERR_ARG;
    if (armed_sweeps) *armed_sweeps = c->n_dead_sweeps;
    if (tangents_rewritten_in_armed_sweeps) *tangents_rewritten_in_armed_sweeps = c->n_dead_tangents;
    if (test_only_starts) *test_only_starts = c->n_test_starts;
    if (test_only_retries) *test_only_retries = c->n_test_retries;
    return PLFX_OK;
}

int plfx_plane_info(plfx_ctx *c, int *mode_on, int64_t *plane_sweeps, int64_t *plane_updates, int *switched_off_by)
{
    if (!c) return PLFX_ERR_ARG;
    const bool on = plane_active(c);
    if (mode_on) *mode_on = on ? 1 : 0;
    if (plane_sweeps) *plane_sweeps = c->n_plane_sweeps;
    if (plane_updates) *plane_updates = c->n_plane_updates;
    if (switched_off_by) *switched_off_by = on ? PLFX_PLANE_ON : c->plane_cols ? PLFX_PLANE_SHARDED : c->plane_off_by;
    return PLFX_OK;
}

int plfx_mg_info(plfx_ctx *c, int max_levels, int *levels, int *dims, double *ratios, int *matfree_level, int *tail_level,
                 int *tail_kernel, int *coarse_solver, int *cheby_steps, double *cheby_kappa, int *march)
{
    if (!c) return PLFX_ERR_ARG;
    const int nl = mg_active(c) ? (int)c->mg.size() : 0;
    if (levels) *levels = nl;
    for (int l = 0; l < nl && l < max_levels; l++) {
        const auto &L = c->mg[l];
        if (dims) dims[2 * l] = L.nx, dims[2 * l + 1] = L.ny;
        if (ratios) ratios[2 * l] = L.rx, ratios[2 * l + 1] = L.ry;
        if (matfree_level) matfree_level[l] = (l == 0 ? matfree(c) : level_from_generators(c, l)) ? 1 : 0;
    }
    const int tail = (nl && !c->strip.on) ? mg_tail_kernel(c) : PLFX_MG_TAIL_NONE;
    if (tail_kernel) *tail_kernel = tail;
    if (tail_level) *tail_level = tail != PLFX_MG_TAIL_NONE ? c->mg_tail : -1;
    const bool dense = nl && c->mg.back().ainv;
    const bool cheby = nl && !dense && tail == PLFX_MG_TAIL_NONE && c->mg_cheby > 0;
    if (coarse_solver) *coarse_solver = dense ? PLFX_MG_COARSE_DENSE : cheby ? PLFX_MG_COARSE_CHEBY : PLFX_MG_COARSE_PCG;
    if (cheby_steps) *cheby_steps = cheby ? c->mg_cheby : 0;
    if (cheby_kappa) *cheby_kappa = cheby ? c->mg_cheby_kappa : 0.;
    if (march) *march = (nl && c->mg[0].matfree && march_mg(c)) ? 1 : 0;
    return PLFX_OK;
}

int plfx_sweep_launch_info(plfx_ctx *c, int64_t *heavy_skipped, int64_t *heavy_recovered)
{
    if (!c) return PLFX_ERR_ARG;
    if (heavy_skipped) *heavy_skipped = c->n_heavy_skipped;
    if (heavy_recovered) *heavy_recovered = c->n_heavy_recovered;
    return PLFX_OK;
}

int plfx_svc_info(plfx_ctx *c, int *row_materials, int *thread_materials, int64_t *row_launches, int64_t *thread_launches)
{
    if (!c) return PLFX_ERR_ARG;
    if (row_materials) *row_materials = (int)c->svc_row_all;
    if (thread_materials) *thread_materials = (int)(c->svc6_mask & ~c->svc_row_all);
    if (row_launches) *row_launches = c->n_svc_row_launches;
    if (thread_launches) *thread_launches = c->n_svc_thread_launches;
    return PLFX_OK;
}

int plfx_reuse_info(plfx_ctx *c, int *assemblies, int *bc_applications, int *solves)
{
    if (!c) return PLFX_ERR_ARG;
    if (assemblies) *assemblies = c->n_reuse_assemble;
    if (bc_applications) *bc_applications = c->n_reuse_bc;
    if (solves) *solves = c->n_reuse_solve;
    return PLFX_OK;
}

int plfx_gen_structured(int NX, int NY, int32_t *conn, int32_t *noleft, int32_t *noright, int32_t *nobot, int32_t *notop)
{
    if (NX < 1 || NY < 1 || (int64_t)(NX + 1) * (NY + 1) > INT32_MAX) return PLFX_ERR_ARG;
    const int nyn = NY + 1;
    if (conn)
        for (int ih = 0; ih < NX * NY; ih++) {
            const int n1 = (ih / NY) * nyn + ih % NY;
            conn[4 * (size_t)ih + 0] = n1;
            conn[4 * (size_t)ih + 1] = n1 + 1;
            conn[4 * (size_t)ih + 2] = n1 + nyn;
            conn[4 * (size_t)ih + 3] = n1 + nyn + 1;
        }
    for (int k = 0; k <= NY; k++) {
        if (noleft) noleft[k] = k;
        if (noright) noright[k] = NX * nyn + k;
    }
    for (int j = 0; j <= NX; j++) {
        if (nobot) nobot[j] = j * nyn;
        if (notop) notop[j] = j * nyn + NY;
    }
    return PLFX_OK;
}

int plfx_pattern_selftest(int nx, int ny)
{
    if (nx < 2 || ny < 2 || (int64_t)(nx + 1) * (ny + 1) > (1 << 24)) return PLFX_ERR_ARG;
    const int nel = nx * ny, nnode = (nx + 1) * (ny + 1), nyn = ny + 1;
    std::vector<int32_t> conn((size_t)4 * nel), hcol, hcontrib;
    for (int e = 0; e < nel; e++) {
        const int n1 = (e / ny) * nyn + e % ny;
        conn[4 * (size_t)e] = n1;
        conn[4 * (size_t)e + 1] = n1 + 1;
        conn[4 * (size_t)e + 2] = n1 + nyn;
        conn[4 * (size_t)e + 3] = n1 + nyn + 1;
    }
    int gx = 0, gy = 0;
    if (!structured_dims(nel, nnode, conn.data(), &gx, &gy) || gx != nx || gy != ny) return 1;
    int nslot = 0, nq = 0, nb = 0, ne = 0;
    if (!build_pattern(nnode, conn.data(), 0, nel, hcol, hcontrib, nslot, nq, nb, ne)) return 2;
    if (nslot != 9 || nq != 4 || nb != 0 || ne != nnode) return 3;
    for (int i = 0; i < nnode; i++)
        for (int s = 0; s < 9; s++) {
            int32_t cj, codes[4];
            structured_slot(nx, ny, i, s, &cj, codes);
            if (cj != hcol[(size_t)s * nnode + i]) return 4;
            for (int q = 0; q < 4; q++)
                if (codes[q] != hcontrib[((size_t)s * 4 + q) * nnode + i]) return 5;
        }
    std::swap(conn[4], conn[5]);
    if (structured_dims(nel, nnode, conn.data(), &gx, &gy)) return 6;
    return PLFX_OK;
}

int plfx_set_precond(plfx_ctx *c, int kind, double omega, int nu)
{
    if (!c) return PLFX_ERR_STATE;
    if (kind != 0 && kind != 1) return fail(c, PLFX_ERR_ARG, "precond kind must be 0 (Jacobi) or 1 (multigrid)");
    if (c->strip.on) {
        if (kind != 1 || (nu > 0 && nu != c->mg_nu) || (omega > 0. && omega != c->mg_omega))
            return fail(c, PLFX_ERR_UNSUPPORTED, "plfx_set_precond after plfx_set_strip: a strip runs multigrid V(2,2) with the "
                        "smoother chosen before plfx_set_strip");
        return PLFX_OK;
    }
    c->precond = kind;
    if (omega > 0.) c->mg_omega = omega;
    if (nu > 0) c->mg_nu = nu;
    mg_graph_drop(c);
    c->M_dirty = true;
    return PLFX_OK;
}

int plfx_precond_info(plfx_ctx *c, int *kind, int *levels)
{
    if (!c) return PLFX_ERR_STATE;
    if (kind) *kind = mg_active(c) ? 1 : 0;
    if (levels) *levels = (int)c->mg.size();
    return PLFX_OK;
}

int plfx_precond_apply(plfx_ctx *c, const double *r, double *z)
{
    if (!c || !mg_active(c) || c->strip.on || !c->assembled || !r || !z)
        return c ? fail(c, PLFX_ERR_STATE, "needs the multigrid hierarchy of a single-GPU solve, assembled") : PLFX_ERR_STATE;
    HIPCHK(c, hipMemsetAsync(&c->sc->done, 0, sizeof(int), c->stream));
    HIPCHK(c, hipMemcpyAsync(c->r, r, (size_t)8 * c->ndof, hipMemcpyHostToDevice, c->stream));
    const int rc = mg_vcycle(c);
    if (rc) return rc;
    HIPCHK(c, hipMemcpyAsync(z, c->z, (size_t)8 * c->ndof, hipMemcpyDeviceToHost, c->stream));
    HIPCHK(c, stream_sync(c));
    c->memo.valid = false;
    return PLFX_OK;
}

int plfx_precond_bench(plfx_ctx *c, int reps, double *us_per_cycle, double *us_coarse)
{
    if (!c || !mg_active(c) || c->strip.on) return c ? fail(c, PLFX_ERR_STATE, "needs the multigrid hierarchy of a single-GPU solve") : PLFX_ERR_STATE;
    if (reps < 1) reps = 1;
    {
        const int e = mg_ensure(c);
        if (e) return e;
    }
    hipEvent_t e0, e1;
    HIPCHK(c, hipEventCreate(&e0));
    HIPCHK(c, hipEventCreate(&e1));
    HIPCHK(c, hipMemsetAsync(&c->sc->done, 0, sizeof(int), c->stream));
    int rc = 0;
    float ms = 0.f;
    for (int w = 0; w < 3 && !rc; w++) rc = mg_vcycle(c);
    HIPCHK(c, hipEventRecord(e0, c->stream));
    for (int k = 0; k < reps && !rc; k++) {
        rc = mg_vcycle(c);
        if ((k & 63) == 63) HIPCHK(c, stream_sync(c));
    }
    HIPCHK(c, hipEventRecord(e1, c->stream));
    HIPCHK(c, hipEventSynchronize(e1));
    HIPCHK(c, hipEventElapsedTime(&ms, e0, e1));
    if (us_per_cycle) *us_per_cycle = 1e3 * ms / reps;
    if (us_coarse && !rc) {
        const int nl = (int)c->mg.size();
        const int lt = (c->mg_tail > 0) ? c->mg_tail : nl - 1;
        auto coarse_only = [&]() -> int {
            if (lt < 2 || !c->want_mg_graph) return mg_coarse_part(c);
            if (!c->mg_graph_exec) return mg_vcycle_rest(c, nullptr, nullptr);
            return hipGraphLaunch(c->mg_graph_exec, c->stream) == hipSuccess ? 0 : PLFX_ERR_HIP;
        };
        auto &L = c->mg[0];
        auto &C1 = c->mg[1];
        HIPCHK(c, hipEventRecord(e0, c->stream));
        for (int k = 0; k < reps && !rc; k++) {
            hipLaunchKernelGGL(k_mg_restrict, dim3(grid_for(C1.nnode)), dim3(BLOCK), 0, c->stream, C1.nx + 1, C1.ny + 1, L.nx + 1, L.ny + 1,
                               (const double2 *)L.res, (const double2 *)C1.dinv, (double2 *)C1.b);
            rc = coarse_only();
            hipLaunchKernelGGL(k_mg_prolong_add, dim3(grid_for(L.nnode)), dim3(BLOCK), 0, c->stream, L.nx + 1, L.ny + 1, C1.ny + 1,
                               (const double2 *)C1.x, (const double2 *)L.dinv, (double2 *)L.x);
        }
        HIPCHK(c, hipEventRecord(e1, c->stream));
        HIPCHK(c, hipEventSynchronize(e1));
        HIPCHK(c, hipEventElapsedTime(&ms, e0, e1));
        *us_coarse = 1e3 * ms / reps;
    }
    hipEventDestroy(e0);
    hipEventDestroy(e1);
    c->x_is_du = c->x_is_du && true;
    return rc;
}

int plfx_assemble(plfx_ctx *c)
{
    if (!c || !c->dval) return c ? fail(c, PLFX_ERR_STATE, "set_mesh first") : PLFX_ERR_STATE;
    const bool setup_done = c->spec_setup && c->spec_was_clean && c->spec_h0 != 0 && matfree(c);
    c->spec_setup = c->spec_kdu = false;
    if (c->reuse && c->assembled && !c->M_dirty) {
        c->n_reuse_assemble++;
        return PLFX_OK;
    }
    EvPair *ev;
    tim_begin(c, 3, &ev);
    if (matfree(c)) {
        KOp live = c->op;
        live.M = c->Mel;
        if (setup_done)
            c->n_spec_setup++;
        else
            LAUNCH_SETUP(0, live, (double2 *)c->diag,
                               c->Mop, (mg_active(c) && level_plain(c->mg[0])) ? c->mg[1].Mel : (double *)nullptr, (const double2 *)nullptr, 0, 0,
                               (double2 *)nullptr);
        c->dinv_ok = false;
        c->val_valid = false;
    } else {
        int rc = assemble_fine_val(c);
        if (rc) return rc;
    }
    tim_end(c, ev);
    HIPCHK(c, hipGetLastError());
    if (mg_active(c)) {
        if (mg_lazy(c)) {
            if (c->mg_pending) c->n_mg_setup_skipped++;
            else c->mg_pending_same = true;
            c->mg_pending = true;
        } else {
            int rc = mg_assemble(c);
            if (rc) return rc;
        }
    }
    if (c->strip.on) {
        int rc = strip_child_assemble(c);
        if (rc) return rc;
    }
    c->assembled = true;
    c->M_dirty = false;
    c->op_epoch++;
    c->memo.valid = false;
    return PLFX_OK;
}

int plfx_get_csr(plfx_ctx *c, int64_t *nnz, int32_t *rowptr, int32_t *colidx, double *val)
{
    if (!c || !c->assembled) return c ? fail(c, PLFX_ERR_STATE, "assemble first") : PLFX_ERR_STATE;
    const int nn = c->nnode, ns = c->nslot;
    int64_t cnt = 0;
    for (int i = 0; i < nn; i++) {
        int k = 0;
        for (int s = 0; s < ns; s++)
            if (host_col(c, s, i) >= 0) k++;
        cnt += 4 * (int64_t)k;
    }
    if (nnz) *nnz = cnt;
    if (!rowptr || !colidx || !val) return PLFX_OK;
    if (!c->val_valid) {
        int rc = assemble_fine_val(c);
        if (rc) return rc;
    }
    std::vector<double> hv((size_t)ns * 4 * nn);
    HIPCHK(c, hipMemcpyAsync(hv.data(), c->dval, hv.size() * 8, hipMemcpyDeviceToHost, c->stream));
    HIPCHK(c, stream_sync(c));
    int64_t pos = 0;
    for (int i = 0; i < nn; i++)
        for (int rr = 0; rr < 2; rr++) {
            rowptr[2 * i + rr] = (int32_t)pos;
            for (int s = 0; s < ns; s++) {
                const int j = host_col(c, s, i);
                if (j < 0) continue;
                for (int cc = 0; cc < 2; cc++) {
                    colidx[pos] = 2 * j + cc;
                    val[pos] = hv[((size_t)s * 4 + rr * 2 + cc) * nn + i];
                    pos++;
                }
            }
        }
    rowptr[2 * nn] = (int32_t)pos;
    return PLFX_OK;
}

namespace {
int apply_bc_impl(plfx_ctx *c, int n, const int32_t *idx, const double *du_presc, const double *w, const double *fext,
                  const int32_t *seg4, const BcSegVals *segv)
{
    const size_t nd = c->ndof;
    int rc = ensure_tmp(c, std::max(n, 1));
    if (rc) return rc;
    const bool same_set = c->bc_valid && (int)c->bc_idx.size() == n &&
                          (n == 0 || memcmp(c->bc_idx.data(), idx, (size_t)4 * n) == 0);
    if (!same_set) {
        c->x_is_du = false;
        c->pred_d_kept = false;
        HIPCHK(c, hipMemsetAsync(c->is_presc, 0, 8 * nd, c->stream));
        HIPCHK(c, hipMemsetAsync(c->dup, 0, 8 * nd, c->stream));
        HIPCHK(c, hipMemsetAsync(c->wv, 0, 8 * nd, c->stream));
        c->bc_idx.assign(idx, idx + n);
// ... 16 lines not shown
                }
            }
            std::vector<int32_t> rows;
            for (int i = 0; i < nn; i++)
                if (mark[i]) rows.push_back(i);
            c->bc_nrows = (int)rows.size();
            dfree(c->bc_rows);
            if ((rc = dalloc(c, &c->bc_rows, rows.size()))) return rc;
            if (!rows.empty())
                HIPCHK(c, hipMemcpyAsync(c->bc_rows, rows.data(), rows.size() * 4, hipMemcpyHostToDevice, c->stream));
            if (!c->kw && (rc = dalloc(c, &c->kw, nd))) return rc;
            HIPCHK(c, hipMemsetAsync(c->kw, 0, 8 * nd, c->stream));
            c->rhs_rows_ok = false;
            HIPCHK(c, stream_sync(c));
        }
        c->bc_valid = true;
        c->rhs_rows_ok = c->dinv_ok = false;
    }
    if (c->reuse && seg4 && same_set && c->bc_set && c->bc_memo && c->bc_epoch == c->op_epoch && !fext && !c->bc_memo_fext &&
        memcmp(&c->bc_last, segv, sizeof(BcSegVals)) == 0) {
        c->n_reuse_bc++;
        return PLFX_OK;
    }
    c->memo.valid = false;
    c->bc_memo = seg4 != nullptr;
    if (seg4) {
        c->bc_last = *segv;
        c->bc_epoch = c->op_epoch;
        c->bc_memo_fext = fext != nullptr;
    }
    if (n > 0 && seg4) {
        hipLaunchKernelGGL(k_scatter_bc_plan, dim3((n + BLOCK - 1) / BLOCK), dim3(BLOCK), 0, c->stream, n, c->bc_idx_dev,
                           seg4, *segv, c->dup, c->wv, c->is_presc, same_set ? 0 : 1);
        HIPCHK(c, hipGetLastError());
    } else if (n > 0) {
        if ((size_t)n > c->stage_cap) {
            HIPCHK(c, stream_sync(c));
            if (c->stage) hipHostFree(c->stage);
            c->stage = nullptr;
            HIPCHK(c, hipHostMalloc((void **)&c->stage, (size_t)32 * n));
            c->stage_cap = n;
            c->stage_busy[0] = c->stage_busy[1] = false;
        }
        const int h = c->stage_flip;
        c->stage_flip ^= 1;
        if (!c->stage_ev[h]) HIPCHK(c, hipEventCreateWithFlags(&c->stage_ev[h], hipEventDisableTiming));
        if (c->stage_busy[h]) HIPCHK(c, hipEventSynchronize(c->stage_ev[h]));
        double *st = c->stage + (size_t)h * 2 * c->stage_cap;
        memcpy(st, du_presc, (size_t)8 * n);
        memcpy(st + n, w, (size_t)8 * n);
        HIPCHK(c, hipMemcpyAsync(c->val_tmp, st, (size_t)16 * n, hipMemcpyHostToDevice, c->stream));
        HIPCHK(c, hipEventRecord(c->stage_ev[h], c->stream));
        c->stage_busy[h] = true;
        hipLaunchKernelGGL(k_scatter_bc, dim3((n + BLOCK - 1) / BLOCK), dim3(BLOCK), 0, c->stream, n, c->bc_idx_dev,
                           c->val_tmp, c->val_tmp + n, c->dup, c->wv, c->is_presc, same_set ? 0 : 1);
        HIPCHK(c, hipGetLastError());
    }
    if (fext) HIPCHK(c, hipMemcpyAsync(c->fext, fext, 8 * nd, hipMemcpyHostToDevice, c->stream));
    const bool rows_only = c->bc_rows_on && c->reuse && !c->strip.on && !comm_active(c) && c->rhs_rows_ok && same_set && !fext &&
                           c->bc_nrows > 0;
    const double2 *rm = rows_only ? (const double2 *)c->is_presc : nullptr;
    double2 *rr = rows_only ? (double2 *)c->rhs : nullptr;
    if (c->bc_nrows > 0)
    {
        if (matfree(c) && c->op.colr)
            hipLaunchKernelGGL(HIP_KERNEL_NAME(k_spmv_rows<2>), dim3((c->bc_nrows + BLOCK - 1) / BLOCK), dim3(BLOCK), 0,
                               c->stream, c->bc_nrows, c->bc_rows, c->op, (const double2 *)c->wv, (double2 *)c->kw, rm, rr);
        else if (matfree(c))
            hipLaunchKernelGGL(HIP_KERNEL_NAME(k_spmv_rows<1>), dim3((c->bc_nrows + BLOCK - 1) / BLOCK), dim3(BLOCK), 0,
                               c->stream, c->bc_nrows, c->bc_rows, c->op, (const double2 *)c->wv, (double2 *)c->kw, rm, rr);
        else
            hipLaunchKernelGGL(HIP_KERNEL_NAME(k_spmv_rows<0>), dim3((c->bc_nrows + BLOCK - 1) / BLOCK), dim3(BLOCK), 0,
                               c->stream, c->bc_nrows, c->bc_rows, c->op, (const double2 *)c->wv, (double2 *)c->kw, rm, rr);
    }
    if (rows_only) {
        c->n_rhs_rows++;
        if (c->dinv_ok)
            c->n_dinv_kept++;
        else if ((c->short_solve & 1) && mg_lazy(c) && mg_active(c) && c->mg_pending) {
            c->dinv_late = true;
            c->n_dinv_refreshed++;
            c->n_dinv_deferred++;
        } else {
            hipLaunchKernelGGL(k_dinv, dim3(grid_for(nd)), dim3(BLOCK), 0, c->stream, nd, c->diag, c->is_presc, c->dinv);
            c->n_dinv_refreshed++;
            c->dinv_late = false;
        }
    } else {
        hipLaunchKernelGGL(k_bc_finish, dim3(grid_for(nd)), dim3(BLOCK), 0, c->stream, nd,
                           fext ? c->fext : nullptr, c->kw, c->diag, c->is_presc, c->rhs, c->dinv);
        c->rhs_rows_ok = !fext;
        c->dinv_late = false;
    }
    c->dinv_ok = true;
    HIPCHK(c, hipGetLastError());
    if (fext) HIPCHK(c, stream_sync(c));
    if (mg_active(c)) {
        if (c->mg_pending)
            c->mg_pending_same = c->mg_pending_same && same_set;
        else {
            rc = mg_update_dinv(c, same_set);
            if (rc) return rc;
        }
    }
    if (c->strip.on && (rc = strip_child_dinv(c))) return rc;
    c->bc_set = true;
    return PLFX_OK;
}
}

int plfx_apply_bc(plfx_ctx *c, int n, const int32_t *idx, const double *du_presc, const double *w,
                  const double *fext)
{
    if (!c || !c->assembled) return c ? fail(c, PLFX_ERR_STATE, "assemble first") : PLFX_ERR_STATE;
    if (n < 0 || (n > 0 && (!idx || !du_presc || !w))) return fail(c, PLFX_ERR_ARG, "bad argument");
    for (int k = 0; k < n; k++)
        if (idx[k] < 0 || idx[k] >= c->ndof) return fail(c, PLFX_ERR_ARG, "presc_idx[%d] out of range", k);
    return apply_bc_impl(c, n, idx, du_presc, w, fext, nullptr, nullptr);
}

int plfx_set_bc_plan(plfx_ctx *c, int nseg, const int32_t *seg_len, const int32_t *idx)
{
    if (!c || !c->u) return c ? fail(c, PLFX_ERR_STATE, "set_mesh first") : PLFX_ERR_STATE;
    if (nseg < 0 || (nseg > 0 && (!seg_len || !idx))) return fail(c, PLFX_ERR_ARG, "bad argument");
    auto &P = c->plan;
    P.valid = false;
    c->bc_memo = false;
    c->memo.valid = false;
    P.nseg = nseg;
    P.seg_of.clear();
    std::vector<int32_t> all;
    for (int s2 = 0, o = 0; s2 < nseg; s2++) {
        if (seg_len[s2] < 0) return fail(c, PLFX_ERR_ARG, "negative segment length");
        for (int k = 0; k < seg_len[s2]; k++, o++) {
            if (idx[o] < 0 || idx[o] >= c->ndof) return fail(c, PLFX_ERR_ARG, "plan index %d out of range", o);
            all.push_back(idx[o]);
            P.seg_of.push_back(s2);
        }
    }
    const int n = (int)all.size();
    std::vector<int32_t> order(n);
    for (int i = 0; i < n; i++) order[i] = i;
    std::stable_sort(order.begin(), order.end(), [&](int a2, int b2) { return all[a2] < all[b2]; });
    P.presc.clear();
    P.first_pos.clear();
    P.inv.assign(n, 0);
    for (int q2 = 0; q2 < n; q2++) {
        const int i = order[q2];
        if (q2 == 0 || all[i] != all[order[q2 - 1]]) {
            P.presc.push_back(all[i]);
            P.first_pos.push_back(i);
        }
        P.inv[i] = (int32_t)P.presc.size() - 1;
    }
    P.first.assign(P.presc.size(), 0.);
    P.w.assign(P.presc.size(), 0.);
    dfree(P.seg4);
    if (nseg <= BcSegVals::N && !P.presc.empty()) {
        const size_t np = P.presc.size();
        std::vector<int32_t> t(4 * np, -1);
        std::vector<int> cnt(np, 0);
        bool ok = true;
        for (int i = 0; i < n && ok; i++) {
            const int k = P.inv[i];
            if (cnt[k] == 4)
                ok = false;
            else
                t[4 * (size_t)k + cnt[k]++] = P.seg_of[i];
        }
        if (ok) {
            int rc = dalloc(c, &P.seg4, t.size());
// ... 219 lines not shown
```

### pylabfea_amd/csrc/plfx_host.hpp

```cpp
#pragma once
#include "../../include/plfx.h"
#include "plfx_kernels.hpp"
#include "plfx_tex.hpp"
#include "plfx_path.hpp"

#include <dlfcn.h>
#include <algorithm>
#include <chrono>
#include <thread>
#include <cmath>
#include <cstdarg>
#include <cstdio>
#include <cstring>
#include <map>
#include <memory>
#include <mutex>
#include <string>
#include <type_traits>
#include <vector>

#define PLFX_VERSION "0.1.0-r1"

namespace plfx {
struct MgLevDev;
// ... 82 lines not shown

    int nel_total = 0, nnode = 0, ndof = 0, e0 = 0, nel = 0;
    int planestress = 0;
    double thick = 1.;
    int ncls = 0;
    std::vector<ClassDev> hcls;
    std::vector<int32_t> hcls_id;
    std::vector<int32_t> hconn;
    std::vector<double> hlxy;
    ClassDev *dcls = nullptr;
    int32_t *dconn = nullptr, *dcls_id = nullptr;
    int32_t *dcls_all = nullptr;
    bool sharded = false;
    int own_n0 = 0, own_n1 = 0;
    int nslot = 0, nq = 0;
    int32_t *dcol = nullptr, *dcontrib = nullptr;
    std::vector<int32_t> hcol;
    int pat_nx = 0, pat_ny = 0;
    double *dval = nullptr;
    int n_begin = 0, n_end = 0;
    bool nonlin = false;

    double *sig = nullptr, *epl = nullptr, *eps = nullptr, *res_sig = nullptr, *res_depl = nullptr;
    bool res_is_sig = false, res_fresh = false, eps_stale = false;
    double *fld_buf = nullptr, *fld_part = nullptr;
    size_t fld_cap = 0;
    std::vector<double> fld_host;
    double *Mel = nullptr, *fyn = nullptr, *scf_hh = nullptr;
    double *tan_buf = nullptr, *elstiff = nullptr, *elfac = nullptr;
    uint8_t *eltag = nullptr;
    double *kh_el = nullptr;
    int hint_nx = 0, hint_ny = 0;
    bool hint_uniform = false;
    double *colr = nullptr;
    double colr_ratio = 1.;
    int wh_mode = 1;
    double wh_carry[16] = {0};
    double *kh_out = nullptr, *kh_new = nullptr, *wh_snap_el = nullptr, *wh_snap_M = nullptr;
    int32_t *wh_snap_ms = nullptr;
    int32_t *kh_touch = nullptr, *wh_bmax = nullptr, *wh_cnt = nullptr;
    bool kh_out_valid = false;
    int64_t n_wh_passes = 0, n_wh_sweeps = 0, n_wh_unresolved = 0;
    int32_t *max_steps = nullptr, *scf_mult = nullptr, *heavy_list = nullptr;
    double *u = nullptr, *f = nullptr, *du = nullptr, *rhs = nullptr, *dinv = nullptr, *diag = nullptr,
           *is_presc = nullptr, *dup = nullptr, *wv = nullptr, *fext = nullptr;
    double *x = nullptr, *r = nullptr, *z = nullptr, *q = nullptr, *p[2] = {nullptr, nullptr};
    double *part = nullptr;
    double *part_g = nullptr;
    CgScalars *sc = nullptr;
    int *flags = nullptr;
    int *bflags = nullptr;
    double *small = nullptr;
    int32_t *idx_tmp = nullptr;
    double *val_tmp = nullptr;
    size_t tmp_cap = 0;
    bool assembled = false, bc_set = false;
    std::vector<int32_t> bc_idx;
    bool bc_valid = false;
    double *stage = nullptr;
    size_t stage_cap = 0;
    hipEvent_t stage_ev[2] = {nullptr, nullptr};
    bool stage_busy[2] = {false, false};
    int stage_flip = 0;
    int32_t *bc_idx_dev = nullptr;
    size_t bc_idx_cap = 0;
    int32_t *bc_rows = nullptr;
    int bc_nrows = 0;
    double *kw = nullptr;
    bool bc_rows_on = true;
    bool rhs_rows_ok = false, dinv_ok = false;
    long long n_rhs_rows = 0, n_dinv_kept = 0, n_dinv_refreshed = 0, n_du_early = 0;
    int short_solve = 3;
    bool dinv_late = false, pred_d_kept = false;
    long long n_dinv_deferred = 0, n_dinv_late = 0, n_d_kept = 0;
    int last_heavy = -1;
    long long n_heavy_skipped = 0, n_heavy_recovered = 0;
    bool x_is_du = false;
    double *pred_x = nullptr, *pred_d = nullptr;
    bool pred_valid = false;
    bool predict = true;
    bool mg_pending = false, mg_pending_same = true;
    long long n_mg_setup = 0, n_mg_setup_skipped = 0;
    bool spec_arm = false, spec_setup = false, spec_kdu = false, spec_was_clean = false;
    bool dead_stores = true, test_starts = true, dead_arm = false, res_partial = false;
    long long n_dead_sweeps = 0, n_dead_tangents = 0, n_test_starts = 0, n_test_retries = 0;
    bool plane_switch = true, plane_mats_ok = false, plane_cols = false;
    int plane_off_by = PLFX_PLANE_NEVER_ON;
    long long n_plane_sweeps = 0, n_plane_updates = 0;
    bool first_test_hint[2] = {false, false};
    int spec_h0 = 0, spec_h1 = 0;
    CgScalars *spec_sc = nullptr;
    long long n_spec_setup = 0, n_spec_kdu = 0;
    int resp_maxit = MAXIT;
    long long n_pred = 0, n_pred_skipped = 0, n_pred_rejected = 0;
    bool reuse = true;
    bool M_dirty = true;
    unsigned long long op_epoch = 0;
    bool bc_memo = false, bc_memo_fext = false;
    unsigned long long bc_epoch = 0;
    BcSegVals bc_last{};
    struct { bool valid = false; double rtol = 0., relres = 0.; } memo;
    int n_reuse_assemble = 0, n_reuse_bc = 0, n_reuse_solve = 0;
    long long n_sweeps = 0, n_tangents_rewritten = 0;
    long long n_svc_row_launches = 0, n_svc_thread_launches = 0;
    struct BcPlan {
        int nseg = 0;
        std::vector<int32_t> seg_of;
        std::vector<int32_t> presc;
        std::vector<int32_t> first_pos;
        std::vector<int32_t> inv;
        std::vector<double> first, w;
        bool valid = false;
        int32_t *seg4 = nullptr;
        std::vector<int32_t> src, k, fsrc, fk, flen, fidx;
        std::vector<double> fshare, fext;
        bool sources = false;
    } plan;
    int32_t *fin_idx = nullptr;
    int fin_n = 0;
    double *fin_dev = nullptr;
    double *fin_host = nullptr;
    CgMbox *fin_box[2] = {nullptr, nullptr};
    double *fin_pin[2] = {nullptr, nullptr};
    unsigned long long fin_seq[2] = {0, 0};
    bool fin_pending[2] = {false, false};
    int fin_pin_n = 0;
    int fin_defer = -1;
    int mg_fallbacks = 0;
    int n_indefinite = 0;
    std::vector<double *> gm_blk;
    double *gm_part = nullptr;
    double *gm_part2 = nullptr, *gm_red = nullptr, *gm_coef = nullptr;
    long long n_gmres_its = 0;
    int n_gmres = 0, gm_m = 0;
    bool strip_jacobi = false;
    int grid_nodes = 0, grid_el = 0;

    struct MgLevel {
        int nx = 0, ny = 0, nnode = 0, nel = 0, nslot = 0, nq = 0, grid = 1;
        int32_t *col = nullptr, *contrib = nullptr, *cls0 = nullptr;
        double *val = nullptr, *diag = nullptr, *dinv = nullptr, *Mel = nullptr;
        double *x = nullptr, *b = nullptr, *t = nullptr, *res = nullptr;
        double *ainv = nullptr;
        KOp op{};
        double rx = 1., ry = 1.;
        ClassDev *cls4 = nullptr;
        bool matfree = false;
        bool owned = false;
    };
    std::vector<MgLevel> mg;
    ClassDev *mg_cls = nullptr;
    MgLevDev *mg_dev = nullptr;
    int mg_tail = -1;
    int mg_tail_T = 0;
    int mg_cheby = 0;
    double mg_cheby_kappa = 1.;
    int mg_tail_E = 0;
    size_t mg_tail_lds = 0;
    bool mg_inv_valid = false;
    bool mg_dinv_current = false;
    CgMbox *mbox = nullptr;
    unsigned long long mbox_seq = 0;
    double *mb_buf = nullptr;
    int mb_cap = 0;
    hipGraph_t mg_graph = nullptr;
    hipGraphExec_t mg_graph_exec = nullptr;
// ... 160 lines not shown
            else                                                                                                         \
                hipLaunchKernelGGL(HIP_KERNEL_NAME(kern<false, true, true, TexFieldDev>), grid, dim3(512), 0, (c)->stream, __VA_ARGS__, tf_);  \
            (c)->tex_field_launches[k]++;                                                                                \
        } else if ((((c)->svc_row_lds >> (k)) & 1u) && cols_)                                                                   \
            hipLaunchKernelGGL(HIP_KERNEL_NAME(kern<true, true>), grid, dim3(512), (size_t)(c)->svc_wave_lds, (c)->stream, __VA_ARGS__);  \
        else if (cols_)                                                                                                  \
            hipLaunchKernelGGL(HIP_KERNEL_NAME(kern<false, true>), grid, dim3(512), 0, (c)->stream, __VA_ARGS__);        \
        else if (((c)->svc_row_lds >> (k)) & 1u)                                                                         \
            hipLaunchKernelGGL(kern<true>, grid, dim3(512), (size_t)(c)->svc_wave_lds, (c)->stream, __VA_ARGS__);        \
        else                                                                                                             \
            hipLaunchKernelGGL(kern<false>, grid, dim3(512), 0, (c)->stream, __VA_ARGS__);                               \
    } while (0)
#define LAUNCH_ROW2(c, k, ids_, kern, H, grid, ...)                                                                         \
    do {                                                                                                                 \
        const bool cols_ = ((c)->svc_cols_mask >> (k)) & 1u;                                                             \
        if (((c)->tex_field_mask >> (k)) & 1u) {                                                                         \
            TexFieldDev tf_ = (c)->tex_field[k];                                                                         \
            tf_.ids = (ids_);                                                                                            \
            if (((c)->svc_row_lds >> (k)) & 1u)                                                                          \
                hipLaunchKernelGGL(HIP_KERNEL_NAME(kern<H, true, true, true, TexFieldDev>), grid, dim3(512), (size_t)(c)->svc_wave_lds, (c)->stream, __VA_ARGS__, tf_);  \
            else                                                                                                         \
                hipLaunchKernelGGL(HIP_KERNEL_NAME(kern<H, false, true, true, TexFieldDev>), grid, dim3(512), 0, (c)->stream, __VA_ARGS__, tf_);  \
            (c)->tex_field_launches[k]++;                                                                                \
        } else if ((((c)->svc_row_lds >> (k)) & 1u) && cols_)                                                                   \
            hipLaunchKernelGGL(HIP_KERNEL_NAME(kern<H, true, true>), grid, dim3(512), (size_t)(c)->svc_wave_lds, (c)->stream, __VA_ARGS__);   \
        else if (cols_)                                                                                                  \
            hipLaunchKernelGGL(HIP_KERNEL_NAME(kern<H, false, true>), grid, dim3(512), 0, (c)->stream, __VA_ARGS__);     \
        else if (((c)->svc_row_lds >> (k)) & 1u)                                                                         \
            hipLaunchKernelGGL(HIP_KERNEL_NAME(kern<H, true>), grid, dim3(512), (size_t)(c)->svc_wave_lds, (c)->stream, __VA_ARGS__);   \
        else                                                                                                             \
            hipLaunchKernelGGL(HIP_KERNEL_NAME(kern<H, false>), grid, dim3(512), 0, (c)->stream, __VA_ARGS__);           \
    } while (0)

inline bool plane_active(const plfx_ctx *c) { return c->plane_cols && !c->strip.on && !comm_active(c) && !c->sharded; }

inline int row16_block(const plfx_ctx *c, int n, int cap)
{
    int block = 64;
    while (block < cap && (n + block / 16 - 1) / (block / 16) > 2 * c->prop.multiProcessorCount) block *= 2;
    return block;
}

inline dim3 row16_grid(const plfx_ctx *c, int n, int block, int rounds)
{
    const int rpb = block / 16;
    return dim3(std::max(1, std::min((n + rpb - 1) / rpb, rounds * c->prop.multiProcessorCount)));
}

hipError_t set_dyn_lds(const void *fn, int bytes);
int tan_alloc(plfx_ctx *c, size_t n);
void tan_free(plfx_ctx *c);
int grid_for(size_t n, int cap = MAXPART);
int grid_xcd(size_t n);
void tim_begin(plfx_ctx *c, int which, EvPair **out);
void tim_end(plfx_ctx *c, EvPair *e);
void tim_flush(plfx_ctx *c);
hipError_t stream_sync(plfx_ctx *c);
int mbox_wait(plfx_ctx *c, unsigned long long seq, CgMbox *box = nullptr);
int fetch_results(plfx_ctx *c, const double *src_dev, int n, double *dst_host);
int ensure_tmp(plfx_ctx *c, size_t n);
int allreduce(plfx_ctx *c, void *dev, size_t count, int nccl_dtype, int nccl_op, const char *what);
int part_allreduce(plfx_ctx *c, double *p, size_t n);
int halo_refresh(plfx_ctx *c, double *v);
int strip_sync_M(plfx_ctx *c);
int sync_M(plfx_ctx *c);
void plane_off(plfx_ctx *c, int why);
KOp make_op(const plfx_ctx *c, int nnode, int nslot, const int32_t *col, const double *val, int nx, int ny, int nel,
            const double *M, double rx = 1., double ry = 1.);
void mg_graph_drop(plfx_ctx *c);
int strip_coarse(plfx_ctx *c);
void strip_free(plfx_ctx *c);
int plain_spmv(plfx_ctx *c, const double *in, double *out);
bool march_pcg(const plfx_ctx *c);
int ensure_dinv(plfx_ctx *c);
int mg_ensure(plfx_ctx *c);
int mg_vcycle_head(plfx_ctx *c);
int mg_vcycle_rest(plfx_ctx *c, double *rz_part, bool *wrote);
int mg_vcycle(plfx_ctx *c);
void launch_spmv_plain(plfx_ctx *c, const double *in, double *out, CgScalars *sc);
void launch_jacobi_z(plfx_ctx *c);
void launch_mbox_post(plfx_ctx *c, const double *src, int n, double *dst, CgMbox *mb, unsigned long long seq);
void launch_kdu_uf(plfx_ctx *c, CgScalars *spec);
void launch_spec_setup(plfx_ctx *c);

int ensure_eps(plfx_ctx *c);
int split_res_sig(plfx_ctx *c);
int raise_step_lds(plfx_ctx *c);
void launch_response_row(plfx_ctx *c, int k, const int32_t *tex_id, int n, const int32_t *mat_id, const double *sig, const double *epl,
                         const double *deps, double *fy, double *sig_out, double *depl, double *ct, int32_t *nsteps);
void launch_path_row(plfx_ctx *c, int k, const int32_t *tex_id, const PathArgs &a);
void launch_tangent_expand(plfx_ctx *c, double *out, int to_full);
#ifdef PLFX_PROF_REGIONS
bool prof_regions_add_step(unsigned long long h[16]);
#endif

void free_materials(plfx_ctx *c);
#ifdef PLFX_PROF_REGIONS
bool prof_regions_add_material(unsigned long long h[16]);
#endif

int solve_impl(plfx_ctx *c, double rtol, int maxit, int warm, int site, int *iters, double *relres);

}
}
```

### pylabfea_amd/csrc/plfx_kernels.hpp

```cpp
#pragma once
#include "plfx_device.hpp"
#include "plfx_rayroot.hpp"

namespace plfx {

constexpr int BLOCK = 256;
constexpr int MAXMAT = 16;
constexpr int MAXCLS = 16;
constexpr int MAXPART = 1024;
#ifndef PLFX_SWEEP_WAVES
#define PLFX_SWEEP_WAVES 1
#endif

struct ClassDev {
    double bxs[4], bys[4];
    double Sxx[16], Sxy[16], Syy[16];
    double kappa, vel, lx, ly;
    int32_t mat, _pad;
};

__device__ __forceinline__ double wave_sum(double v)
{
#pragma unroll
    for (int off = 32; off > 0; off >>= 1) v += __shfl_down(v, off, 64);
// ... 704 lines not shown
    e[0] = ex;
    e[1] = ey;
    e[2] = c.kappa * (ex + ey);
    e[3] = 0.;
    e[4] = 0.;
    e[5] = gxy;
}

__device__ __forceinline__ void tangent_to_M(const double *D, double kappa, double *M)
{
    const double k = kappa;
    M[0] = D[sym_idx(0, 0)] + k * (2. * D[sym_idx(0, 2)] + k * D[sym_idx(2, 2)]);
    M[1] = D[sym_idx(0, 1)] + k * (D[sym_idx(0, 2)] + D[sym_idx(1, 2)] + k * D[sym_idx(2, 2)]);
    M[2] = D[sym_idx(0, 5)] + k * D[sym_idx(2, 5)];
    M[3] = D[sym_idx(1, 1)] + k * (2. * D[sym_idx(1, 2)] + k * D[sym_idx(2, 2)]);
    M[4] = D[sym_idx(1, 5)] + k * D[sym_idx(2, 5)];
    M[5] = D[sym_idx(5, 5)];
}

enum : uint8_t { TAN_CV = 0, TAN_FAC = 1, TAN_FULL = 2 };
struct TanStore {
    uint8_t *tag;
    double *fac;
    double *full;
};

__device__ __forceinline__ double tan_fac_entry(const double *CV, const double *f, int i, int j)
{
    return fma(-f[0] * f[1 + i], f[1 + j], CV[sym_idx(i, j)]);
}

__device__ __forceinline__ void tan_expand(int form, const double *CV, const double *T, double *D)
{
    if (form == TAN_FULL) {
#pragma unroll
        for (int k = 0; k < 21; k++) D[k] = T[k];
    } else if (form == TAN_FAC) {
#pragma unroll
        for (int i = 0; i < 6; i++)
#pragma unroll
            for (int j = i; j < 6; j++) D[sym_idx(i, j)] = tan_fac_entry(CV, T, i, j);
    } else {
#pragma unroll
        for (int k = 0; k < 21; k++) D[k] = CV[k];
    }
}

__device__ __forceinline__ void tan_load(const TanStore &ts, int nel, int e, const double *CV, double *D)
{
    const int form = ts.tag[e];
    if (form == TAN_FULL) {
#pragma unroll
        for (int k = 0; k < 21; k++) D[k] = ts.full[(size_t)k * nel + e];
    } else if (form == TAN_FAC) {
        double f[7];
#pragma unroll
        for (int k = 0; k < 7; k++) f[k] = ts.fac[(size_t)k * nel + e];
        tan_expand(TAN_FAC, CV, f, D);
    } else {
        tan_expand(TAN_CV, CV, nullptr, D);
    }
}

__device__ __forceinline__ int tan_load_fac(const TanStore &ts, int nel, int e, double *f)
{
    const int form = ts.tag[e];
    if (form == TAN_FAC) {
#pragma unroll
        for (int k = 0; k < 7; k++) f[k] = ts.fac[(size_t)k * nel + e];
    }
    return form;
}

constexpr __device__ __host__ bool plane_col(int k) { return k != 3 && k != 4; }
constexpr __device__ __host__ bool plane_fac(int k) { return k != 4 && k != 5; }

template <bool MAY_SKIP = false, bool PLANE = false, bool AHEAD = false>
__device__ __forceinline__ void sweep_epilogue(const ClassDev &c, const MatDev &m, int e, int nel,
                                               const double *s, const double *ep, const double *depl,
                                               int form, const double *Ct, double fy, int ns, const TanStore &ts,
                                               int oform, const double *ofac, int omax,
                                               double *Mel, int mel_stride, double *res_sig,
                                               double *res_depl, double *fyn, int32_t *max_steps, int nit,
                                               int &changed, int &nconv, double kh = -1., int dead_ok = 0)
{
    const bool late = MAY_SKIP && dead_ok;
    if (!late) {
#pragma unroll
        for (int k = 0; k < 6; k++) {
            if (PLANE && !plane_col(k)) continue;
            res_sig[(size_t)k * nel + e] = s[k];
            res_depl[(size_t)k * nel + e] = depl[k];
        }
    }
    const double f = fy / (kh >= 0. ? m.sy + eps_eq(ep) * kh : sflow_of(m, ep));
    if (!late) fyn[e] = f;
    if (!(f <= YF_TOL * 1.0001)) nconv = 1;
    double Dold[21], Dnew[21];
    if (oform == TAN_FULL) {
#pragma unroll
        for (int k = 0; k < 21; k++) Dold[k] = ts.full[(size_t)k * nel + e];
        if (AHEAD) {
#pragma unroll
            for (int k = 0; k < 21; k++) landed(Dold[k]);
        }
    } else {
        tan_expand(oform, m.CV, ofac, Dold);
    }
    tan_expand(form, m.CV, Ct, Dnew);
    double hh = 0.;
#pragma unroll
    for (int i = 0; i < 6; i++)
#pragma unroll
        for (int j = i; j < 6; j++) {
            const double d = Dold[sym_idx(i, j)] - Dnew[sym_idx(i, j)];
            hh += (i == j ? 1. : 2.) * d * d;
        }
    hh = sqrt(hh);
    if (late && !(hh > 1.e-3)) {
#pragma unroll
        for (int k = 0; k < 6; k++) {
            if (PLANE && !plane_col(k)) continue;
            res_sig[(size_t)k * nel + e] = s[k];
            res_depl[(size_t)k * nel + e] = depl[k];
        }
        fyn[e] = f;
    }
    if (hh > 1.e-3) {
        if (nit >= 15) {
#pragma unroll
            for (int k = 0; k < 21; k++) Dnew[k] = 0.5 * (Dnew[k] + Dold[k]);
            form = TAN_FULL;
        }
        ts.tag[e] = (uint8_t)form;
        if (form == TAN_FULL) {
#pragma unroll
            for (int k = 0; k < 21; k++) ts.full[(size_t)k * nel + e] = Dnew[k];
        } else if (form == TAN_FAC) {
#pragma unroll
            for (int k = 0; k < 7; k++)
                if (!PLANE || plane_fac(k)) ts.fac[(size_t)k * nel + e] = Ct[k];
        }
        double M[6];
        tangent_to_M(Dnew, c.kappa, M);
#pragma unroll
        for (int k = 0; k < 6; k++) Mel[(size_t)k * mel_stride + e] = M[k];
        changed += 1;
    }
    if (ns > omax) max_steps[e] = ns;
}

struct SweepIn {
    int cl, n[4], form, ms;
    double s[6], ep[6], fac[7];
};

template <bool PLANE = false, bool AHEAD = false>
__device__ __forceinline__ void sweep_in_load(SweepIn &in, long long e, int nel, int e_off, const int32_t *__restrict__ cls,
                                              const int32_t *__restrict__ conn, const double *__restrict__ sig,
                                              const double *__restrict__ epl, const TanStore &ts,
                                              const int32_t *max_steps)
{
    in = SweepIn{};
    if (AHEAD || e < nel) {
        const size_t ge = (size_t)e + e_off;
        in.cl = cls[e];
        if (!AHEAD) {
#pragma unroll
            for (int k = 0; k < 4; k++) in.n[k] = conn[ge * 4 + k];
        }
#pragma unroll
        for (int k = 0; k < 6; k++) {
            if (PLANE && !plane_col(k)) continue;
            in.s[k] = sig[(size_t)k * nel + e];
            in.ep[k] = epl[(size_t)k * nel + e];
        }
        in.form = ts.tag[e];
        if (!AHEAD) in.ms = max_steps[e];
#pragma unroll
        for (int k = 0; k < 7; k++)
            if (!PLANE || plane_fac(k)) in.fac[k] = ts.fac[(size_t)k * nel + e];
    }
}

struct SweepTables {
    MatDev smat[MAXMAT];
    ClassDev scls[MAXCLS];
};

__device__ __forceinline__ void stage_tables(SweepTables &t, const MatDev *gmat, int nmat,
                                             const ClassDev *gcls, int ncls)
{
    stage_materials(t.smat, gmat, nmat);
    const int words = ncls * (int)(sizeof(ClassDev) / 8);
    const double *src = reinterpret_cast<const double *>(gcls);
    double *dst = reinterpret_cast<double *>(t.scls);
    for (int i = threadIdx.x; i < words; i += blockDim.x) dst[i] = src[i];
}

constexpr int SWEEP_SLOTS = 1024;
static_assert(SWEEP_SLOTS >= MAXPART, "one slot per block of a sweep grid");

__device__ __forceinline__ void post_block_flags(int changed, int nconv, int *__restrict__ bflags)
{
    __shared__ int sh_c[16], sh_n[16];
    int cw = changed, nw = nconv ? 1 : 0;
    for (int o = 32; o; o >>= 1) {
        cw += __shfl_xor(cw, o, 64);
        nw |= __shfl_xor(nw, o, 64);
    }
    const int wave = threadIdx.x >> 6, nwaves = (blockDim.x + 63) >> 6;
    if ((threadIdx.x & 63) == 0) {
        sh_c[wave] = cw;
        sh_n[wave] = nw;
    }
    __syncthreads();
    if (threadIdx.x == 0) {
        int c2 = 0, n2 = 0;
        for (int w = 0; w < nwaves; w++) {
            c2 += sh_c[w];
            n2 |= sh_n[w];
        }
        if (c2) bflags[2 * blockIdx.x] += c2;
        if (n2) bflags[2 * blockIdx.x + 1] = 1;
    }
}

struct CgMbox;
__device__ void mbox_publish(CgMbox *mb, unsigned long long seq);
// ... 69 lines not shown
__global__ void __launch_bounds__(BLOCK, (KIND <= 2 && PLFX_SWEEP_WAVES < 2) ? 2 : PLFX_SWEEP_WAVES)
k_sweep_light(const MatDev *__restrict__ gmat, int nmat, const ClassDev *__restrict__ gcls, int ncls,
              int lds_doubles, int nel, int e_off, const int32_t *__restrict__ conn,
              const int32_t *__restrict__ cls, const double2 *__restrict__ du2,
              const double *__restrict__ sig, const double *__restrict__ epl, TanStore ts,
              double *Mel, int mel_stride, double *res_sig, double *res_depl, double *fyn,
              int32_t *max_steps, int nit, int *flags, int *bflags, int32_t *list, int first_kind, unsigned skip_mask,
              int dead_ok ,
              double *kh_el = nullptr ,
              double *kh_out = nullptr, int32_t *kh_touch = nullptr )
{
    __shared__ SweepTables tb;
    stage_tables(tb, gmat, nmat, gcls, ncls);
    __syncthreads();
    int svc_mat = -1;
    const double *sv = nullptr, *dual = nullptr;
    if (kind_is_svc(KIND)) {
        stage_svc(tb.smat, nmat, dyn_lds, lds_doubles, svc_mat, sv, dual, KIND);
        __syncthreads();
    }
    int changed = 0, nconv = 0;
    const int nb = gridDim.x;
    constexpr bool PREFETCH = (KIND == 1);
    constexpr bool DEAD_STORES = (KIND == 1 || KIND == 2);
    int t = xcd_tile(blockIdx.x, nb);
    SweepIn nx;
    if (PREFETCH) sweep_in_load(nx, (long long)t * BLOCK + threadIdx.x, nel, e_off, cls, conn, sig, epl, ts, max_steps);
    for (; t * BLOCK < nel; t += nb) {
        const int e = t * BLOCK + threadIdx.x;
        bool heavy = false;
        if (!PREFETCH) sweep_in_load(nx, (long long)t * BLOCK + threadIdx.x, nel, e_off, cls, conn, sig, epl, ts, max_steps);
        const SweepIn in = nx;
        if (PREFETCH) sweep_in_load(nx, (long long)(t + nb) * BLOCK + threadIdx.x, nel, e_off, cls, conn, sig, epl, ts, max_steps);
        asm volatile("" ::: "memory");
        if (e < nel) {
            const ClassDev &c = tb.scls[in.cl];
            const MatDev &m = tb.smat[c.mat];
            if (m.kind == 0) {
                if (first_kind) fyn[e] = 0.;
            } else if (m.kind == KIND && !((skip_mask >> c.mat) & 1u)) {
                double deps[6], s[6], ep[6], depl[6], Ct[21], dr[6], fy, st_scal;
                class_strain(c, du2, in.n[0], in.n[1], in.n[2], in.n[3], deps);
#pragma unroll
                for (int k = 0; k < 6; k++) {
                    s[k] = in.s[k];
                    ep[k] = in.ep[k];
                }
                const bool staged = (c.mat == svc_mat);
                const typename YfOf<KIND>::type yf =
                    make_policy<KIND>(m, staged ? sv : nullptr, staged ? dual : nullptr, (KIND == 7 && kh_el) ? kh_el[e] : m.khard);
                const int st = response_light<true>(m, yf, s, ep, deps, fy, depl, Ct, dr, st_scal);
                if (st == 2)
                    heavy = true;
                else {
                    sweep_epilogue<DEAD_STORES>(c, m, e, nel, s, ep, depl, st, Ct, fy, 0, ts, in.form, in.fac, in.ms, Mel, mel_stride, res_sig,
                                   res_depl, fyn, max_steps, nit, changed, nconv, KIND == 7 ? yf.kh() : -1., dead_ok);
                    if (KIND == 7 && kh_el) {
                        (kh_out ? kh_out : kh_el)[e] = yf.kh();
                        if (kh_touch) kh_touch[e] = yf.touched();
                    }
                }
            }
        }
        const unsigned long long mask = __ballot(heavy);
        if (mask) {
            const int lane = threadIdx.x & 63;
            int base = 0;
            if (lane == 0) base = atomicAdd(&flags[2], __popcll(mask));
            base = __shfl(base, 0, 64);
            if (heavy) list[base + __popcll(mask & ((1ull << lane) - 1ull))] = e;
        }
    }
    post_block_flags(changed, nconv, bflags);
}

constexpr int PLANE_SWEEP_WAVES = PLFX_SWEEP_WAVES < 2 ? 2 : PLFX_SWEEP_WAVES;
#ifdef PLFX_UNIT_STEP
__global__ void __launch_bounds__(BLOCK, PLANE_SWEEP_WAVES)
k_sweep_light_plane(const MatDev *__restrict__ gmat, int nmat, const ClassDev *__restrict__ gcls, int ncls,
                    int lds_doubles, int nel, int e_off, const int32_t *__restrict__ conn,
                    const int32_t *__restrict__ cls, const double2 *__restrict__ du2,
                    const double *__restrict__ sig, const double *__restrict__ epl, TanStore ts,
                    double *Mel, int mel_stride, double *res_sig, double *res_depl, double *fyn,
                    int32_t *max_steps, int nit, int *flags, int *bflags, int32_t *list, int first_kind, unsigned skip_mask, int dead_ok)
{
    __shared__ SweepTables tb;
    stage_tables(tb, gmat, nmat, gcls, ncls);
    __syncthreads();
    int changed = 0, nconv = 0;
    const int nb = gridDim.x;
    int t = xcd_tile(blockIdx.x, nb);
    const int4 *__restrict__ conn4 = reinterpret_cast<const int4 *>(conn);
    const auto el = [&](long long tile) { return (int)min(tile * BLOCK + threadIdx.x, (long long)nel - 1); };
    SweepIn nx;
    double2 nu[4];
    int4 cn;
    {
        const int4 c0 = conn4[(size_t)el(t) + e_off];
        cn = conn4[(size_t)el((long long)t + nb) + e_off];
        sweep_in_load<true, true>(nx, el(t), nel, e_off, cls, conn, sig, epl, ts, max_steps);
        nu[0] = du2[c0.x], nu[1] = du2[c0.y], nu[2] = du2[c0.z], nu[3] = du2[c0.w];
        landed(cn.x), landed(cn.y), landed(cn.z), landed(cn.w), landed(nx.cl), landed(nx.form);
#pragma unroll
        for (int k = 0; k < 7; k++) {
            if (k < 6 && plane_col(k)) landed(nx.s[k]), landed(nx.ep[k]);
            if (plane_fac(k)) landed(nx.fac[k]);
            if (k < 4) landed(nu[k].x), landed(nu[k].y);
        }
    }
    for (; t * BLOCK < nel; t += nb) {
        const int e = t * BLOCK + threadIdx.x;
        bool heavy = false;
        const SweepIn in = nx;
        const double2 u0 = nu[0], u1 = nu[1], u2_ = nu[2], u3 = nu[3];
        nu[0] = du2[cn.x], nu[1] = du2[cn.y], nu[2] = du2[cn.z], nu[3] = du2[cn.w];
        asm volatile("" ::: "memory");
        cn = conn4[(size_t)el((long long)t + 2 * nb) + e_off];
        asm volatile("" ::: "memory");
        sweep_in_load<true, true>(nx, el((long long)t + nb), nel, e_off, cls, conn, sig, epl, ts, max_steps);
        asm volatile("" ::: "memory");
        if (e < nel) {
            const ClassDev &c = tb.scls[in.cl];
            const MatDev &m = tb.smat[c.mat];
            if (m.kind == 0) {
                if (first_kind) fyn[e] = 0.;
            } else if (m.kind == 1 && !((skip_mask >> c.mat) & 1u)) {
                double deps[6], s[6], ep[6], depl[6], Ct[21], dr[6], fy, st_scal;
                class_strain_of(c, u0, u1, u2_, u3, deps);
#pragma unroll
                for (int k = 0; k < 6; k++) {
                    s[k] = in.s[k];
                    ep[k] = in.ep[k];
                }
                const YfOf<1>::type yf = make_policy<1>(m, nullptr, nullptr, m.khard);
                const int st = response_light<true>(m, yf, s, ep, deps, fy, depl, Ct, dr, st_scal);
                if (st == 2)
                    heavy = true;
                else
                    sweep_epilogue<true, true, true>(c, m, e, nel, s, ep, depl, st, Ct, fy, 0, ts, in.form, in.fac, 0, Mel, mel_stride,
                                                     res_sig, res_depl, fyn, max_steps, nit, changed, nconv, -1., dead_ok);
            }
        }
        const unsigned long long mask = __ballot(heavy);
        if (mask) {
            const int lane = threadIdx.x & 63;
            int base = 0;
            if (lane == 0) base = atomicAdd(&flags[2], __popcll(mask));
            base = __shfl(base, 0, 64);
            if (heavy) list[base + __popcll(mask & ((1ull << lane) - 1ull))] = e;
        }
    }
    post_block_flags(changed, nconv, bflags);
}
#endif

template <int KIND>
__global__ void __launch_bounds__(BLOCK)
k_sweep_heavy(const MatDev *__restrict__ gmat, int nmat, const ClassDev *__restrict__ gcls, int ncls,
              int lds_doubles, int nel, int e_off, const int32_t *__restrict__ conn,
              const int32_t *__restrict__ cls, const double2 *__restrict__ du2,
              const double *__restrict__ sig, const double *__restrict__ epl, TanStore ts,
              double *Mel, int mel_stride, double *res_sig, double *res_depl, double *fyn,
              int32_t *max_steps, int nit, int *flags, int *bflags, const int32_t *__restrict__ list, unsigned skip_mask,
              double *kh_el = nullptr, double *kh_out = nullptr, int32_t *kh_touch = nullptr)
{
    const int count = flags[2];
    if (count == 0) return;
    __shared__ SweepTables tb;
    stage_tables(tb, gmat, nmat, gcls, ncls);
    __syncthreads();
    int svc_mat = -1;
    const double *sv = nullptr, *dual = nullptr;
    if (kind_is_svc(KIND)) {
        stage_svc(tb.smat, nmat, dyn_lds, lds_doubles, svc_mat, sv, dual, KIND);
        __syncthreads();
    }
    int changed = 0, nconv = 0;
    for (int i = blockIdx.x * BLOCK + threadIdx.x; i < count; i += gridDim.x * BLOCK) {
        const int e = list[i];
        const ClassDev &c = tb.scls[cls[e]];
        const MatDev &m = tb.smat[c.mat];
        if (m.kind != KIND || ((skip_mask >> c.mat) & 1u)) continue;
        const size_t ge = (size_t)e + e_off;
        double deps[6], s[6], ep[6], depl[6], Ct[21], dr[6], ofac[7], fy, st_scal;
        class_strain(c, du2, conn[ge * 4], conn[ge * 4 + 1], conn[ge * 4 + 2], conn[ge * 4 + 3], deps);
#pragma unroll
        for (int k = 0; k < 6; k++) {
            s[k] = sig[(size_t)k * nel + e];
            ep[k] = epl[(size_t)k * nel + e];
        }
        const bool staged = (c.mat == svc_mat);
        const typename YfOf<KIND>::type yf =
            make_policy<KIND>(m, staged ? sv : nullptr, staged ? dual : nullptr, (KIND == 7 && kh_el) ? kh_el[e] : m.khard);
        response_light<true>(m, yf, s, ep, deps, fy, depl, Ct, dr, st_scal);
        response_heavy(m, yf, s, ep, dr, st_scal, fy, depl, Ct);
        sweep_epilogue(c, m, e, nel, s, ep, depl, TAN_FULL, Ct, fy, MAXIT - 1, ts, tan_load_fac(ts, nel, e, ofac), ofac, max_steps[e], Mel, mel_stride, res_sig,
                       res_depl, fyn, max_steps, nit, changed, nconv, KIND == 7 ? yf.kh() : -1.);
        if (KIND == 7 && kh_el) {
            (kh_out ? kh_out : kh_el)[e] = yf.kh();
            if (kh_touch) kh_touch[e] = yf.touched();
        }
    }
    post_block_flags(changed, nconv, bflags);
}

__device__ __forceinline__ int stage_svc_row(const MatDev *smat, int mat)
{
    const MatDev &m = smat[mat];
    const int n = m.nsv, npad = (n + 63) / 64 * 64;
    for (int i = threadIdx.x; i < npad; i += blockDim.x) {
#pragma unroll
        for (int c = 0; c < 6; c++) dyn_lds[c * npad + i] = (i < n) ? m.sv[6 * (size_t)i + c] : 0.;
        dyn_lds[6 * npad + i] = (i < n) ? m.dual[i] : 0.;
        double vv = 0.;
        if (i < n) {
#pragma unroll
            for (int c = 0; c < 6; c++) vv = fma(m.sv[6 * (size_t)i + c], m.sv[6 * (size_t)i + c], vv);
        }
        dyn_lds[7 * npad + i] = vv;
    }
    double *ext = dyn_lds + 9 * npad;
    for (int i = threadIdx.x; i < RAYPOLY_N * RAYPOLY_N; i += blockDim.x) ext[i] = RAYPOLY_MT[i];
    if (threadIdx.x < 64) {
// ... 203 lines not shown
                           max_steps, nit, changed, nconv, yf.kh());
            if (kh_el) {
                (kh_out ? kh_out : kh_el)[e] = yf.kh();
                if (kh_touch) kh_touch[e] = yf.touched();
            }
        }
    }
    post_block_flags(lane == 0 ? changed : 0, lane == 0 ? nconv : 0, bflags);
}

#ifdef PLFX_UNIT_STEP
__global__ void __launch_bounds__(BLOCK)
k_init_tangent(const MatDev *gmat, const ClassDev *gcls, int nel, const int32_t *cls,
               TanStore ts, double *Mel, int mel_stride)
{
    const int e = blockIdx.x * BLOCK + threadIdx.x;
    if (e >= nel) return;
    const ClassDev &c = gcls[cls[e]];
    const MatDev &m = gmat[c.mat];
    ts.tag[e] = TAN_CV;
    double M[6];
    tangent_to_M(m.CV, c.kappa, M);
#pragma unroll
    for (int k = 0; k < 6; k++) Mel[(size_t)k * mel_stride + e] = M[k];
}

__global__ void __launch_bounds__(BLOCK)
k_init_M_all(const MatDev *gmat, const ClassDev *gcls, int nel, const int32_t *cls, double *Mel)
{
    const int e = blockIdx.x * BLOCK + threadIdx.x;
    if (e >= nel) return;
    const ClassDev &c = gcls[cls[e]];
    double M[6];
    tangent_to_M(gmat[c.mat].CV, c.kappa, M);
#pragma unroll
    for (int k = 0; k < 6; k++) Mel[(size_t)k * nel + e] = M[k];
}
#endif

#ifdef PLFX_UNIT_OPERATOR
__global__ void __launch_bounds__(BLOCK)
k_zero_foreign_M(int nel_total, int e0, int e1, double *Mel)
{
    const size_t n = (size_t)6 * nel_total;
    for (size_t i = blockIdx.x * (size_t)BLOCK + threadIdx.x; i < n; i += (size_t)gridDim.x * BLOCK) {
        const int e = (int)(i % nel_total);
        if (e < e0 || e >= e1) Mel[i] = 0.;
    }
}
#endif

#ifdef PLFX_UNIT_STEP
__global__ void __launch_bounds__(BLOCK)
k_refresh_M(const MatDev *gmat, const ClassDev *gcls, int nel, const int32_t *cls, TanStore ts, double *Mel,
            int mel_stride)
{
    const int e = blockIdx.x * BLOCK + threadIdx.x;
    if (e >= nel) return;
    const ClassDev &c = gcls[cls[e]];
    double D[21], M[6];
    tan_load(ts, nel, e, gmat[c.mat].CV, D);
    tangent_to_M(D, c.kappa, M);
#pragma unroll
    for (int k = 0; k < 6; k++) Mel[(size_t)k * mel_stride + e] = M[k];
}

__global__ void __launch_bounds__(BLOCK)
k_tangent_expand(const MatDev *gmat, const ClassDev *gcls, int nel, const int32_t *cls, TanStore ts, double *out, int to_full)
{
    const int e = blockIdx.x * BLOCK + threadIdx.x;
    if (e >= nel) return;
    double D[21];
    tan_load(ts, nel, e, gmat[gcls[cls[e]].mat].CV, D);
#pragma unroll
    for (int k = 0; k < 21; k++) out[(size_t)k * nel + e] = D[k];
    if (to_full) ts.tag[e] = TAN_FULL;
}
#endif

__host__ __device__ __forceinline__ size_t gen_index(bool pair, int c, size_t nel, size_t e)
{
    return pair ? ((size_t)(c >> 1) * nel + e) * 2 + (c & 1) : (size_t)c * nel + e;
}

__host__ __device__ inline void structured_slot(int nx, int ny, int i, int s, int32_t *col, int32_t *codes )
{
    const int nyn = ny + 1;
    const int j = i / nyn, k = i - j * nyn;
    const int jlo = j > 0 ? j - 1 : 0, jhi = j < nx ? j + 1 : nx;
    const int klo = k > 0 ? k - 1 : 0, khi = k < ny ? k + 1 : ny;
    const int nkk = khi - klo + 1, cnt = (jhi - jlo + 1) * nkk;
    codes[0] = codes[1] = codes[2] = codes[3] = -1;
    if (s >= cnt) {
        *col = -1;
        return;
    }
    const int jj = jlo + s / nkk, kk = klo + s % nkk;
    *col = jj * nyn + kk;
    int qn = 0;
    for (int ej = j - 1; ej <= j; ej++) {
        if (ej < 0 || ej >= nx || jj < ej || jj > ej + 1) continue;
        for (int ek = k - 1; ek <= k; ek++) {
            if (ek < 0 || ek >= ny || kk < ek || kk > ek + 1) continue;
            const int e = ej * ny + ek, a = (j - ej) * 2 + (k - ek), b = (jj - ej) * 2 + (kk - ek);
            codes[qn++] = e * 16 + a * 4 + b;
        }
    }
}

#ifdef PLFX_UNIT_MESH
__global__ void __launch_bounds__(256)
k_structured_pattern(int nx, int ny, int32_t *__restrict__ col, int32_t *__restrict__ contrib)
{
    const int nnode = (nx + 1) * (ny + 1);
    for (int i = blockIdx.x * 256 + threadIdx.x; i < nnode; i += gridDim.x * 256) {
#pragma unroll
        for (int s = 0; s < 9; s++) {
            int32_t cj, codes[4];
            structured_slot(nx, ny, i, s, &cj, codes);
            col[(size_t)s * nnode + i] = cj;
#pragma unroll
            for (int q = 0; q < 4; q++) contrib[((size_t)s * 4 + q) * nnode + i] = codes[q];
        }
    }
}
#endif

#ifdef PLFX_UNIT_OPERATOR
__global__ void __launch_bounds__(BLOCK)
k_assemble(const ClassDev *gcls, int ncls, int nnode, int nslot, int nq, int nel,
           const int32_t *contrib, const int32_t *cls, const double *Mel, const int32_t *col,
           double *val, double *diag, int pair )
{
    __shared__ ClassDev scls[MAXCLS];
    {
        const int words = ncls * (int)(sizeof(ClassDev) / 8);
        const double *src = reinterpret_cast<const double *>(gcls);
        double *dst = reinterpret_cast<double *>(scls);
        for (int i = threadIdx.x; i < words; i += BLOCK) dst[i] = src[i];
    }
    __syncthreads();
    const int s = blockIdx.y;
    for (int i = blockIdx.x * BLOCK + threadIdx.x; i < nnode; i += gridDim.x * BLOCK) {
        double k00 = 0., k01 = 0., k10 = 0., k11 = 0.;
        for (int q = 0; q < nq; q++) {
            const int code = contrib[((size_t)s * nq + q) * nnode + i];
            if (code < 0) continue;
            const int e = code >> 4, a = (code >> 2) & 3, b = code & 3;
            const ClassDev &c = scls[cls[e]];
            const double Mxx = Mel[gen_index(pair, 0, nel, e)], Mxy = Mel[gen_index(pair, 1, nel, e)],
                         Mxs = Mel[gen_index(pair, 2, nel, e)], Myy = Mel[gen_index(pair, 3, nel, e)],
                         Mys = Mel[gen_index(pair, 4, nel, e)], Mss = Mel[gen_index(pair, 5, nel, e)];
            const double sxx = c.Sxx[a * 4 + b], sxy = c.Sxy[a * 4 + b], syx = c.Sxy[b * 4 + a],
                         syy = c.Syy[a * 4 + b];
            k00 += Mxx * sxx + Mxs * (sxy + syx) + Mss * syy;
            k01 += Mxy * sxy + Mxs * sxx + Mys * syy + Mss * syx;
            k10 += Mxy * syx + Mys * syy + Mxs * sxx + Mss * sxy;
            k11 += Myy * syy + Mys * (syx + sxy) + Mss * sxx;
        }
        val[((size_t)s * 4 + 0) * nnode + i] = k00;
        val[((size_t)s * 4 + 1) * nnode + i] = k01;
        val[((size_t)s * 4 + 2) * nnode + i] = k10;
        val[((size_t)s * 4 + 3) * nnode + i] = k11;
        if (col[(size_t)s * nnode + i] == i) {
            diag[2 * (size_t)i] = k00;
            diag[2 * (size_t)i + 1] = k11;
// ... 1793 lines not shown
```

### pylabfea_amd/csrc/plfx_step.hip

```cpp
#define PLFX_UNIT_STEP
#include "plfx_host.hpp"

using namespace plfx;
using namespace plfx::host;

namespace plfx {
namespace host {

int ensure_eps(plfx_ctx *c)
{
    if (!c->eps_stale) return 0;
    hipLaunchKernelGGL(k_eps_from_u, dim3(grid_for(c->nel, MAXPART)), dim3(BLOCK), 0, c->stream, c->dmat, c->nmat, c->dcls, c->ncls,
                       c->nel, c->e0, c->dconn, c->dcls_id, (const double2 *)c->u, c->eps);
    HIPCHK(c, hipGetLastError());
    c->eps_stale = false;
    return 0;
}

int split_res_sig(plfx_ctx *c)
{
    if (!c->res_is_sig) return 0;
    HIPCHK(c, hipMemcpyAsync(c->res_sig, c->sig, (size_t)48 * c->nel, hipMemcpyDeviceToDevice, c->stream));
    c->res_is_sig = false;
    return 0;
// ... 61 lines not shown
            HIPCHK(c, set_dyn_lds((const void *)k_response_row<true, true>, c->svc_wave_lds));
            HIPCHK(c, set_dyn_lds((const void *)k_response_row<true, true, true, TexFieldDev>, c->svc_wave_lds));
        }
        HIPCHK(c, set_dyn_lds((const void *)k_path_row<true>, c->svc_wave_lds));
        if (c->svc_cols_mask & c->svc_row_lds) {
            HIPCHK(c, set_dyn_lds((const void *)k_path_row<true, true>, c->svc_wave_lds));
            HIPCHK(c, set_dyn_lds((const void *)k_path_row<true, true, true, TexFieldDev>, c->svc_wave_lds));
        }
    }
    return 0;
}

void launch_path_row(plfx_ctx *c, int k, const int32_t *tex_id, const PathArgs &a)
{
    LAUNCH_ROW1(c, k, tex_id, k_path_row, dim3(std::max(1, std::min((a.n + 31) / 32, 1024))), c->dmat, c->nmat, k, a);
}

}
}

extern "C" {

static int plane_sweep_grid(const plfx_ctx *c)
{
    const int resident = c->prop.multiProcessorCount * (PLANE_SWEEP_WAVES * 4 * 64 / BLOCK);
    int g = std::min(c->grid_el, std::max(resident, 1));
    if (g >= 16) g &= ~7;
    return g;
}

static int tex_field_check(plfx_ctx *c)
{
    if (!c->tex_field_mask) return PLFX_OK;
    if (c->strip.on || c->sharded || comm_active(c))
        return fail(c, PLFX_ERR_UNSUPPORTED, "a texture field runs on one GPU without strips or shards");
    if (c->tex_ids_ok || !c->tex_ids) return PLFX_OK;
    for (int e = 0; e < c->nel; e++) {
        const int k = c->hcls[c->hcls_id[(size_t)c->e0 + e]].mat;
        if (!((c->tex_field_mask >> k) & 1u)) continue;
        const int32_t t = c->htex_ids[e];
        if (t < 0 || t >= c->tex_field_rows[k])
            return fail(c, PLFX_ERR_ARG, "texture row %d of element %d is outside the %d rows of material %d", (int)t, e,
                        c->tex_field_rows[k], k);
    }
    c->tex_ids_ok = true;
    return PLFX_OK;
}

int plfx_state_reset(plfx_ctx *c)
{
    if (!c || !c->sig) return c ? fail(c, PLFX_ERR_STATE, "set_mesh first") : PLFX_ERR_STATE;
    const size_t ne = c->nel, nd = c->ndof;
    HIPCHK(c, hipMemsetAsync(c->sig, 0, 48 * ne, c->stream));
    HIPCHK(c, hipMemsetAsync(c->epl, 0, 48 * ne, c->stream));
    HIPCHK(c, hipMemsetAsync(c->eps, 0, 48 * ne, c->stream));
    HIPCHK(c, hipMemsetAsync(c->res_sig, 0, 48 * ne, c->stream));
    HIPCHK(c, hipMemsetAsync(c->res_depl, 0, 48 * ne, c->stream));
    HIPCHK(c, hipMemsetAsync(c->fyn, 0, 8 * ne, c->stream));
    HIPCHK(c, hipMemsetAsync(c->max_steps, 0, 4 * ne, c->stream));
    HIPCHK(c, hipMemsetAsync(c->u, 0, 8 * nd, c->stream));
    HIPCHK(c, hipMemsetAsync(c->f, 0, 8 * nd, c->stream));
    HIPCHK(c, hipMemsetAsync(c->du, 0, 8 * nd, c->stream));
    HIPCHK(c, hipMemsetAsync(c->flags, 0, 32, c->stream));
    HIPCHK(c, hipMemsetAsync(c->bflags, 0, (size_t)8 * SWEEP_SLOTS, c->stream));
    {
        std::vector<double> kh(c->nel);
        for (int e = 0; e < c->nel; e++) kh[e] = c->hmat[c->hcls[c->hcls_id[c->e0 + e]].mat].khard;
        HIPCHK(c, hipMemcpyAsync(c->kh_el, kh.data(), (size_t)8 * c->nel, hipMemcpyHostToDevice, c->stream));
        HIPCHK(c, stream_sync(c));
        for (int m = 0; m < c->nmat && m < 16; m++) c->wh_carry[m] = c->hmat[m].khard;
        c->kh_out_valid = false;
    }
    hipLaunchKernelGGL(k_init_tangent, dim3((c->nel + BLOCK - 1) / BLOCK), dim3(BLOCK), 0, c->stream,
                       c->dmat, c->dcls, c->nel, c->dcls_id, tan_store(c), c->Mel + c->e0, c->nel_total);
    if (c->sharded)
        hipLaunchKernelGGL(k_init_M_all, dim3((c->nel_total + BLOCK - 1) / BLOCK), dim3(BLOCK), 0, c->stream,
                           c->dmat, c->dcls, c->nel_total, c->dcls_all, c->Mel);
    HIPCHK(c, hipGetLastError());
    c->plane_off_by = !c->plane_switch ? PLFX_PLANE_SWITCH : (c->sharded || c->strip.on || comm_active(c)) ? PLFX_PLANE_SHARDED :
                      !c->plane_mats_ok ? PLFX_PLANE_MATERIALS : PLFX_PLANE_ON;
    c->plane_cols = c->plane_off_by == PLFX_PLANE_ON;
    if (c->plane_cols) HIPCHK(c, hipMemsetAsync(c->elfac + 4 * ne, 0, 16 * ne, c->stream));
    c->assembled = false, c->M_dirty = true;
    c->x_is_du = false;
    c->rhs_rows_ok = c->dinv_ok = false;
    c->pred_d_kept = false;
    c->res_is_sig = c->res_fresh = c->eps_stale = c->res_partial = false;
    c->last_heavy = -1;
    return PLFX_OK;
}

static int finish_mode(plfx_ctx *c, bool *swap)
{
    *swap = c->nonlin && !c->has_elastic && c->res_fresh;
    if (*swap) return 0;
    return split_res_sig(c);
}

static void finish_done(plfx_ctx *c, bool swap)
{
    if (swap) {
        std::swap(c->sig, c->res_sig);
        c->res_is_sig = true;
        c->res_fresh = false;
    }
    c->eps_stale = true;
}

static int res_complete(plfx_ctx *c, const char *who)
{
    if (!c->res_partial) return 0;
    return fail(c, PLFX_ERR_STATE, "%s: the last sweep left res_sig / res_depl / fyn partial (a load step ended in an error "
                                   "between two sweeps): sweep again first", who);
}

static int state_ptr(plfx_ctx *c, int which, double **p, size_t *comps, size_t *n, bool *soa)
{
    *soa = true;
    *n = c->nel;
    if (which == 3 || which == 4 || which == 9) {
        const int rcp = res_complete(c, "state");
        if (rcp) return rcp;
    }
    if (which == 1 || which == 6) {
        const int rce = ensure_eps(c);
        if (rce) return rce;
    }
    switch (which) {
    case 0: *p = c->sig; *comps = 6; break;
    case 1: *p = c->eps; *comps = 6; break;
    case 2: *p = c->epl; *comps = 6; break;
    case 3: *p = c->res_is_sig ? c->sig : c->res_sig; *comps = 6; break;
    case 4: *p = c->res_depl; *comps = 6; break;
    case 5: *p = c->elstiff; *comps = 21; break;
    case 6: *p = c->u; *comps = 1; *n = c->ndof; *soa = false; break;
    case 7: *p = c->f; *comps = 1; *n = c->ndof; *soa = false; break;
    case 8: *p = c->du; *comps = 1; *n = c->ndof; *soa = false; break;
    case 9: *p = c->fyn; *comps = 1; *soa = false; break;
    case 11: *p = (wh_sequential(c) && c->kh_out_valid) ? c->kh_out : c->kh_el; *comps = 1; *soa = false; break;
    default: return fail(c, PLFX_ERR_ARG, "unknown state id %d", which);
    }
    return 0;
}

int plfx_state_get(plfx_ctx *c, int which, double *out)
{
    if (!c || !c->sig) return c ? fail(c, PLFX_ERR_STATE, "set_mesh first") : PLFX_ERR_STATE;
    if (!out) return fail(c, PLFX_ERR_ARG, "null output");
    if (which == 10) {
        std::vector<int32_t> t(c->nel);
        HIPCHK(c, hipMemcpyAsync(t.data(), c->max_steps, (size_t)4 * c->nel, hipMemcpyDeviceToHost, c->stream));
        HIPCHK(c, stream_sync(c));
        for (int e = 0; e < c->nel; e++) out[e] = t[e];
        return PLFX_OK;
    }
    double *p;
    size_t comps, n;
    bool soa;
    int rc = state_ptr(c, which, &p, &comps, &n, &soa);
    if (rc) return rc;
    if (!soa) {
        HIPCHK(c, hipMemcpyAsync(out, p, 8 * n, hipMemcpyDeviceToHost, c->stream));
        HIPCHK(c, stream_sync(c));
        return PLFX_OK;
    }
    std::vector<double> t(comps * n);
    if (which == 5) {
        double *tmp = nullptr;
        if ((rc = dalloc(c, &tmp, 21 * n))) return rc;
        launch_tangent_expand(c, tmp, 0);
        hipError_t er = hipGetLastError();
        if (er == hipSuccess) er = hipMemcpyAsync(t.data(), tmp, 8 * comps * n, hipMemcpyDeviceToHost, c->stream);
        if (er == hipSuccess) er = stream_sync(c);
        dfree(tmp);
        HIPCHK(c, er);
    } else {
        HIPCHK(c, hipMemcpyAsync(t.data(), p, 8 * comps * n, hipMemcpyDeviceToHost, c->stream));
        HIPCHK(c, stream_sync(c));
    }
    if (comps == 6) {
        for (size_t e = 0; e < n; e++)
            for (int k = 0; k < 6; k++) out[6 * e + k] = t[(size_t)k * n + e];
    } else {
        for (size_t e = 0; e < n; e++)
            for (int i = 0; i < 6; i++)
                for (int j = 0; j < 6; j++) out[36 * e + 6 * i + j] = t[(size_t)sym_idx(i, j) * n + e];
    }
    return PLFX_OK;
}

int plfx_state_set(plfx_ctx *c, int which, const double *in)
{
    if (!c || !c->sig) return c ? fail(c, PLFX_ERR_STATE, "set_mesh first") : PLFX_ERR_STATE;
    if (!in) return fail(c, PLFX_ERR_ARG, "null input");
    if (which == 10) return fail(c, PLFX_ERR_ARG, "max_steps is read-only");
    double *p;
    size_t comps, n;
    bool soa;
    int rc = (which == 0 || which == 3) ? split_res_sig(c) : 0;
    if (rc) return rc;
    rc = state_ptr(c, which, &p, &comps, &n, &soa);
    if (rc) return rc;
    if (!soa) {
        c->x_is_du = false;
        c->pred_d_kept = false;
        HIPCHK(c, hipMemcpyAsync(p, in, 8 * n, hipMemcpyHostToDevice, c->stream));
        HIPCHK(c, stream_sync(c));
        return PLFX_OK;
    }
    std::vector<double> t(comps * n);
    if (comps == 6) {
        for (size_t e = 0; e < n; e++)
            for (int k = 0; k < 6; k++) t[(size_t)k * n + e] = in[6 * e + k];
    } else {
        for (size_t e = 0; e < n; e++)
            for (int i = 0; i < 6; i++)
                for (int j = i; j < 6; j++) t[(size_t)sym_idx(i, j) * n + e] = in[36 * e + 6 * i + j];
    }
    if (c->plane_cols && (which == 0 || which == 2 || which == 3 || which == 4)) {
        const double *c34 = t.data() + 3 * n;
        for (size_t i = 0; i < 2 * n; i++)
            if (c34[i] != 0.) {
                plane_off(c, PLFX_PLANE_STATE_SET);
                break;
            }
    }
    if (which == 5) plane_off(c, PLFX_PLANE_TANGENT_SET);
    HIPCHK(c, hipMemcpyAsync(p, t.data(), 8 * comps * n, hipMemcpyHostToDevice, c->stream));
    if (which == 5) {
        c->M_dirty = true;
        HIPCHK(c, hipMemsetAsync(c->eltag, TAN_FULL, n, c->stream));
        hipLaunchKernelGGL(k_refresh_M, dim3((c->nel + BLOCK - 1) / BLOCK), dim3(BLOCK), 0, c->stream,
                           c->dmat, c->dcls, c->nel, c->dcls_id, tan_store(c), c->Mel + c->e0, c->nel_total);
        HIPCHK(c, hipGetLastError());
        int rcm = sync_M(c);
        if (rcm) return rcm;
    }
    HIPCHK(c, stream_sync(c));
    return PLFX_OK;
}

int plfx_gather(plfx_ctx *c, int which, int n, const int32_t *idx, double *out)
{
    if (!c || !c->u) return c ? fail(c, PLFX_ERR_STATE, "set_mesh first") : PLFX_ERR_STATE;
    if (n < 0 || !idx || !out) return fail(c, PLFX_ERR_ARG, "bad argument");
    if (n == 0) return PLFX_OK;
    const double *src = which == 6 ? c->u : which == 7 ? c->f : which == 8 ? c->du : nullptr;
    if (!src) return fail(c, PLFX_ERR_ARG, "gather supports u(6), f(7), du(8)");
    for (int k = 0; k < n; k++)
        if (idx[k] < 0 || idx[k] >= c->ndof) return fail(c, PLFX_ERR_ARG, "idx[%d] out of range", k);
    int rc = ensure_tmp(c, n);
    if (rc) return rc;
    HIPCHK(c, hipMemcpyAsync(c->idx_tmp, idx, (size_t)4 * n, hipMemcpyHostToDevice, c->stream));
    hipLaunchKernelGGL(k_gather, dim3((n + BLOCK - 1) / BLOCK), dim3(BLOCK), 0, c->stream, n, c->idx_tmp, src, c->val_tmp);
    HIPCHK(c, hipGetLastError());
    HIPCHK(c, hipMemcpyAsync(out, c->val_tmp, (size_t)8 * n, hipMemcpyDeviceToHost, c->stream));
    HIPCHK(c, stream_sync(c));
    return PLFX_OK;
}

}

namespace {

int step_apply_bc(plfx_ctx *c, const plfx_step *st, const double *dbcr, const double *dbct, const double *dbcn, int *bad)
{
    auto &P = c->plan;
    const double *val[5] = {st->bcl0, st->bcb0, dbcr, dbct, dbcn};
    std::vector<double> seg(P.nseg);
    for (int i = 0; i < P.nseg; i++) seg[i] = val[P.src[i]][P.k[i]];
    const double *fext = nullptr;
    bool any = false;
    size_t o = 0;
    for (size_t f = 0; f < P.fsrc.size(); f++) {
        const double v = val[P.fsrc[f]][P.fk[f]];
        if (v != 0.) {
            if (!any) P.fext.assign(c->ndof, 0.);
            any = true;
            for (int q = 0; q < P.flen[f]; q++) P.fext[P.fidx[o + q]] += v * P.fshare[o + q];
        }
        o += P.flen[f];
    }
    if (any) fext = P.fext.data();
    int b = -1;
    int rc = plfx_apply_bc_plan(c, seg.data(), fext, &b);
    if (bad && *bad < 0) *bad = b;
    return rc;
}

int step_solve(plfx_ctx *c, plfx_step *st, int warm, int site)
{
    int it = 0;
    double rr = 0.;
    const int rc = solve_impl(c, st->rtol, st->maxit, warm, site, &it, &rr);
    if (rc < 0) return rc;
    if (st->nsolves < 40) {
        st->its[st->nsolves] = it;
        st->relres[st->nsolves] = rr;
    }
    st->nsolves++;
    if (rc == 1) st->soft_fail++;
    return 0;
}
}

extern "C" {

int plfx_load_step(plfx_ctx *c, plfx_step *st, double *u_at, double *f_at, double *sums18)
{
    if (!c || !st) return PLFX_ERR_ARG;
    if (!c->plan.valid || !c->plan.sources) return fail(c, PLFX_ERR_STATE, "set_bc_plan / set_bc_sources first");
    if (!c->fin_dev) return fail(c, PLFX_ERR_STATE, "set_finish_set first");
    st->nit = st->nconv = st->nsweeps = st->nsolves = st->soft_fail = 0;
// ... 103 lines not shown
        launch_kdu_uf(c, nullptr);
    else {
        if ((rc = plain_spmv(c, c->du, c->q))) return rc;
        hipLaunchKernelGGL(k_axpy_uf, dim3(grid_for(nd)), dim3(BLOCK), 0, c->stream, nd, c->du, c->q, c->u, c->f);
    }
    const int g = grid_for(c->nel, SUMPART);
    bool swap;
    if ((rc = finish_mode(c, &swap))) return rc;
    if (plane_active(c)) {
        hipLaunchKernelGGL(HIP_KERNEL_NAME(k_update_state_plane<1>), dim3(g), dim3(BLOCK), 0, c->stream, c->dmat, c->nmat, c->dcls, c->ncls,
                           c->nel, c->e0, c->dconn, c->dcls_id, (const double2 *)c->du, (const double2 *)c->u, c->sig, c->epl,
                           tan_store(c), c->res_sig, c->res_depl, c->nonlin ? 1 : 0, swap ? 1 : 0, c->part_g);
        c->n_plane_updates++;
    } else
        hipLaunchKernelGGL(HIP_KERNEL_NAME(k_update_state<1>), dim3(g), dim3(BLOCK), 0, c->stream, c->dmat, c->nmat, c->dcls, c->ncls,
                           c->nel, c->e0, c->dconn, c->dcls_id, (const double2 *)c->du, (const double2 *)c->u, c->sig, c->epl,
                           tan_store(c), c->res_sig, c->res_depl, c->nonlin ? 1 : 0, swap ? 1 : 0, c->part_g,
                           c->strip.on ? c->strip.eown_lo : 0, c->strip.on ? c->strip.eown_hi : 0x7fffffff);
    finish_done(c, swap);
    const int n = c->fin_n;
    const int tot = 2 * n + 18;
    const int sl = c->fin_defer;
    c->fin_defer = -1;
    if (sl >= 0 && c->fin_pin_n < tot) {
        HIPCHK(c, stream_sync(c));
        for (int q = 0; q < 2; q++) {
            if (c->fin_pin[q]) hipHostFree(c->fin_pin[q]);
            c->fin_pin[q] = nullptr;
            HIPCHK(c, hipHostMalloc((void **)&c->fin_pin[q], (size_t)8 * tot, hipHostMallocMapped | hipHostMallocCoherent));
            if (!c->fin_box[q]) {
                HIPCHK(c, hipHostMalloc((void **)&c->fin_box[q], sizeof(CgMbox), hipHostMallocMapped | hipHostMallocCoherent));
                memset(c->fin_box[q], 0, sizeof(CgMbox));
            }
            c->fin_pending[q] = false;
        }
        c->fin_pin_n = tot;
    }
    static const bool direct_ok = !(getenv("PLFX_FINISH_DIRECT") && atoi(getenv("PLFX_FINISH_DIRECT")) == 0);
    const bool direct = sl >= 0 && direct_ok && !comm_active(c);
    double *out = direct ? c->fin_pin[sl] : c->fin_dev;
    hipLaunchKernelGGL(k_finish_out, dim3((n + BLOCK - 1) / BLOCK + 18), dim3(BLOCK), 0, c->stream, n, c->fin_idx, (const double *)c->u,
                       (const double *)c->f, out, out + n, (const double *)c->part_g, 18, g, out + 2 * (size_t)n);
    HIPCHK(c, hipGetLastError());
    if (comm_active(c) &&
        (rc = allreduce(c, c->fin_dev + 2 * (size_t)n, 18, NCCL_FLOAT64, NCCL_SUM, "sums")))
        return rc;
    if (sl >= 0) {
        const unsigned long long seq = ++c->fin_seq[sl];
        launch_mbox_post(c, c->fin_dev, direct ? 0 : tot, c->fin_pin[sl], c->fin_box[sl], seq);
        HIPCHK(c, hipGetLastError());
        c->fin_pending[sl] = true;
        return PLFX_OK;
    }
    if ((rc = fetch_results(c, c->fin_dev, 2 * n + 18, c->fin_host))) return rc;
    if (u_at && n > 0) memcpy(u_at, c->fin_host, (size_t)8 * n);
    if (f_at && n > 0) memcpy(f_at, c->fin_host + n, (size_t)8 * n);
    if (sums18) memcpy(sums18, c->fin_host + 2 * (size_t)n, 18 * 8);
    return PLFX_OK;
}

int plfx_finish_fetch(plfx_ctx *c, int slot, double *u_at, double *f_at, double *sums18)
{
    if (!c || !c->fin_dev) return c ? fail(c, PLFX_ERR_STATE, "set_finish_set first") : PLFX_ERR_STATE;
    if (slot < 0 || slot > 1 || !c->fin_pending[slot]) return fail(c, PLFX_ERR_STATE, "no deferred results in slot %d", slot);
    int rc = mbox_wait(c, c->fin_seq[slot], c->fin_box[slot]);
    if (rc) return rc;
    c->fin_pending[slot] = false;
    const int n = c->fin_n;
    const double *h = c->fin_pin[slot];
    if (u_at && n > 0) memcpy(u_at, h, (size_t)8 * n);
    if (f_at && n > 0) memcpy(f_at, h + n, (size_t)8 * n);
    if (sums18) memcpy(sums18, h + 2 * (size_t)n, 18 * 8);
    return PLFX_OK;
}

static int sweep_once(plfx_ctx *c, int nit, int *changed, int *conv, bool wh_seq)
{
    if (int rct = tex_field_check(c)) return rct;
    c->res_is_sig = false;
    c->res_fresh = true;
    const int dead = (c->dead_arm && c->dead_stores && !comm_active(c) && !c->strip.on && !wh_seq && (c->has_analytic || c->has_princ)) ? 1 : 0;
    c->dead_arm = false;
    c->res_partial = dead != 0;
    EvPair *ev;
    tim_begin(c, 0, &ev);
#define SWEEP_ARGS(lds) c->dmat, c->nmat, c->dcls, c->ncls, lds, c->nel, c->e0, c->dconn, c->dcls_id,          \
                        (const double2 *)c->du, c->sig, c->epl, tan_store(c), c->Mel + c->e0, c->nel_total, \
                        c->res_sig, c->res_depl, c->fyn, c->max_steps, nit, c->flags, c->bflags, c->heavy_list
    int first = 1;
    const unsigned fast = c->svc_row_all;
    const bool svc_thread = c->has_svc && (c->svc6_mask & ~fast);
    const int grid_r = std::max(1, std::min((c->nel + 31) / 32, 1024));
#define ROW_ARGS c->dmat, c->nmat, c->dcls, c->ncls, c->nel, c->e0, c->dconn, c->dcls_id, (const double2 *)c->du,  \
                  c->sig, c->epl, tan_store(c), c->Mel + c->e0, c->nel_total, c->res_sig, c->res_depl, c->fyn,       \
                  c->max_steps, nit, c->flags, c->bflags, c->heavy_list
    if (c->has_analytic || (c->has_elastic && !c->has_princ && !c->has_svc && !c->has_svc3 && !c->has_barlat && !c->has_svcwh && !c->svc_cols_mask)) {
        if (plane_active(c)) {
            hipLaunchKernelGGL(k_sweep_light_plane, dim3(plane_sweep_grid(c)), dim3(BLOCK), 0, c->stream, SWEEP_ARGS(0), first, 0u, dead);
            c->n_plane_sweeps++;
        } else
            hipLaunchKernelGGL(HIP_KERNEL_NAME(k_sweep_light<1>), dim3(c->grid_el), dim3(BLOCK), 0, c->stream,
                               SWEEP_ARGS(0), first, 0u, dead);
        first = 0;
    }
    if (c->has_princ) {
        hipLaunchKernelGGL(HIP_KERNEL_NAME(k_sweep_light<2>), dim3(c->grid_el), dim3(BLOCK), 0, c->stream,
                           SWEEP_ARGS(0), first, 0u, dead);
        first = 0;
    }
    if (c->has_barlat) {
        hipLaunchKernelGGL(HIP_KERNEL_NAME(k_sweep_light<5>), dim3(c->grid_el), dim3(BLOCK), 0, c->stream,
                           SWEEP_ARGS(0), first, 0u, 0);
        first = 0;
    }
    if (svc_thread) {
        hipLaunchKernelGGL(HIP_KERNEL_NAME(k_sweep_light<3>), dim3(c->grid_el), dim3(BLOCK), dyn_lds_bytes(c),
                           c->stream, SWEEP_ARGS(c->svc_lds_need), first, fast, 0);
        first = 0;
        c->n_svc_thread_launches++;
    }
    if (fast) {
        for (int k = 0; k < c->nmat; k++)
            if ((fast >> k) & 1u) {
                LAUNCH_ROW2(c, k, (const int32_t *)c->tex_ids, k_sweep_svc_row, 0, dim3(grid_r), ROW_ARGS, first, k);
                first = 0;
                c->n_svc_row_launches++;
            }
    }
    if (c->has_svc3) {
        hipLaunchKernelGGL(HIP_KERNEL_NAME(k_sweep_light<6>), dim3(c->grid_el), dim3(BLOCK), dyn_lds_bytes(c),
                           c->stream, SWEEP_ARGS(c->svc_lds_need), first, 0u, 0);
        first = 0;
    }
    const bool wh_wave = !(getenv("PLFX_WH_WAVE") && atoi(getenv("PLFX_WH_WAVE")) == 0);
    const int grid_wh = std::max(1, std::min((c->nel + 3) / 4, SWEEP_SLOTS));
    if (c->has_svcwh && wh_wave) {
        hipLaunchKernelGGL(HIP_KERNEL_NAME(k_sweep_wh_wave<0>), dim3(grid_wh), dim3(BLOCK), dyn_lds_bytes(c), c->stream,
                           c->dmat, c->nmat, c->dcls, c->ncls, c->svc_lds_need, c->nel, c->e0, c->dconn, c->dcls_id,
                           (const double2 *)c->du, c->sig, c->epl, tan_store(c), c->Mel + c->e0, c->nel_total, c->res_sig, c->res_depl,
                           c->fyn, c->max_steps, nit, c->flags, c->bflags, c->heavy_list, first, c->kh_el,
                           wh_seq ? c->kh_out : (double *)nullptr, wh_seq ? c->kh_touch : (int32_t *)nullptr);
        first = 0;
    } else if (c->has_svcwh) {
        hipLaunchKernelGGL(HIP_KERNEL_NAME(k_sweep_light<7>), dim3(c->grid_el), dim3(BLOCK), dyn_lds_bytes(c),
                           c->stream, SWEEP_ARGS(c->svc_lds_need), first, 0u, 0, c->kh_el, wh_seq ? c->kh_out : (double *)nullptr,
                           wh_seq ? c->kh_touch : (int32_t *)nullptr);
        first = 0;
    }
    tim_end(c, ev);
    const bool mb_flags = !comm_active(c) && c->mbox && c->mb_cap >= 2;
    const bool skip_heavy = mb_flags && !c->strip.on && c->last_heavy == 0;
    auto launch_phase2 = [&]() {
        tim_begin(c, 6, &ev);
        if (c->has_analytic)
            hipLaunchKernelGGL(HIP_KERNEL_NAME(k_sweep_heavy<1>), dim3(c->grid_el), dim3(BLOCK), 0, c->stream,
                               SWEEP_ARGS(0), 0u);
        if (c->has_princ)
            hipLaunchKernelGGL(HIP_KERNEL_NAME(k_sweep_heavy<2>), dim3(c->grid_el), dim3(BLOCK), 0, c->stream,
                               SWEEP_ARGS(0), 0u);
        if (c->has_barlat)
            hipLaunchKernelGGL(HIP_KERNEL_NAME(k_sweep_heavy<5>), dim3(c->grid_el), dim3(BLOCK), 0, c->stream,
                               SWEEP_ARGS(0), 0u);
        if (svc_thread)
            hipLaunchKernelGGL(HIP_KERNEL_NAME(k_sweep_heavy<3>), dim3(c->grid_el), dim3(BLOCK), dyn_lds_bytes(c),
                               c->stream, SWEEP_ARGS(c->svc_lds_need), fast);
        if (fast)
            for (int k = 0; k < c->nmat; k++)
                if ((fast >> k) & 1u) LAUNCH_ROW2(c, k, (const int32_t *)c->tex_ids, k_sweep_svc_row, 1, dim3(grid_r), ROW_ARGS, 0, k);
        if (c->has_svc3)
            hipLaunchKernelGGL(HIP_KERNEL_NAME(k_sweep_heavy<6>), dim3(c->grid_el), dim3(BLOCK), dyn_lds_bytes(c),
                               c->stream, SWEEP_ARGS(c->svc_lds_need), 0u);
        if (c->has_svcwh && wh_wave)
            hipLaunchKernelGGL(HIP_KERNEL_NAME(k_sweep_wh_wave<1>), dim3(grid_wh), dim3(BLOCK), dyn_lds_bytes(c), c->stream,
                               c->dmat, c->nmat, c->dcls, c->ncls, c->svc_lds_need, c->nel, c->e0, c->dconn, c->dcls_id,
                               (const double2 *)c->du, c->sig, c->epl, tan_store(c), c->Mel + c->e0, c->nel_total, c->res_sig, c->res_depl,
                               c->fyn, c->max_steps, nit, c->flags, c->bflags, c->heavy_list, 0, c->kh_el,
                               wh_seq ? c->kh_out : (double *)nullptr, wh_seq ? c->kh_touch : (int32_t *)nullptr);
        else if (c->has_svcwh)
            hipLaunchKernelGGL(HIP_KERNEL_NAME(k_sweep_heavy<7>), dim3(c->grid_el), dim3(BLOCK), dyn_lds_bytes(c),
                               c->stream, SWEEP_ARGS(c->svc_lds_need), 0u, c->kh_el, wh_seq ? c->kh_out : (double *)nullptr,
                               wh_seq ? c->kh_touch : (int32_t *)nullptr);
        tim_end(c, ev);
    };
#undef SWEEP_ARGS
#undef ROW_ARGS
    if (skip_heavy)
        c->n_heavy_skipped++;
    else
        launch_phase2();
    int h[4];
    const bool spec = c->spec_arm && !comm_active(c) && c->mbox && c->mb_cap >= 2 && matfree(c) && !c->strip.on && c->assembled;
    c->spec_arm = false;
    if (mb_flags) {
        const unsigned long long seq = ++c->mbox_seq;
        hipLaunchKernelGGL(k_sweep_flags, dim3(1), dim3(BLOCK), 0, c->stream, c->bflags, c->flags, c->flags + 4,
                           reinterpret_cast<int *>(c->mb_buf), c->mbox, seq, spec ? c->flags + 8 : (int *)nullptr,
                           spec ? c->spec_sc : (CgScalars *)nullptr, skip_heavy ? 1 : 0);
        if (spec) {
            launch_spec_setup(c);
            launch_kdu_uf(c, c->spec_sc);
            c->spec_was_clean = !c->M_dirty;
            c->spec_setup = c->spec_kdu = true;
        }
        HIPCHK(c, hipGetLastError());
        const int rcw = mbox_wait(c, seq);
        if (rcw) return rcw;
        memcpy(h, c->mb_buf, sizeof(h));
        if (skip_heavy && h[0] < 0) {
            c->n_heavy_recovered++;
            c->spec_setup = c->spec_kdu = false;
            launch_phase2();
            const unsigned long long seq2 = ++c->mbox_seq;
            hipLaunchKernelGGL(k_sweep_flags, dim3(1), dim3(BLOCK), 0, c->stream, c->bflags, c->flags, c->flags + 4,
                               reinterpret_cast<int *>(c->mb_buf), c->mbox, seq2, (int *)nullptr, (CgScalars *)nullptr, 0);
            HIPCHK(c, hipGetLastError());
            const int rcw2 = mbox_wait(c, seq2);
            if (rcw2) return rcw2;
            memcpy(h, c->mb_buf, sizeof(h));
        }
        c->spec_h0 = h[0];
        c->spec_h1 = h[1];
        if (spec && h[0]) c->dinv_ok = false;
    } else {
        hipLaunchKernelGGL(k_sweep_flags, dim3(1), dim3(BLOCK), 0, c->stream, c->bflags, c->flags, c->flags + 4);
        HIPCHK(c, hipGetLastError());
        if (comm_active(c)) {
            const int rca = allreduce(c, c->flags + 4, c->strip.on ? 2 : 4, NCCL_INT32, NCCL_SUM, "flags");
            if (rca) return rca;
        }
        const int rcf = fetch_results(c, reinterpret_cast<const double *>(c->flags + 4), 2, reinterpret_cast<double *>(h));
        if (rcf) return rcf;
    }
    if (h[0] || !c->reuse) {
        int rcm = sync_M(c);
        if (rcm) return rcm;
    }
    if (changed) *changed = h[0];
    if (conv) *conv = h[1] ? 0 : 1;
    if (h[0]) c->M_dirty = true;
    c->n_sweeps++;
    c->n_tangents_rewritten += h[3];
    c->res_partial = dead && h[0];
    if (dead) {
        c->n_dead_sweeps++;
        c->n_dead_tangents += h[3];
    }
    c->last_heavy = h[2];
    return PLFX_OK;
}

static int sweep_wh_sequential(plfx_ctx *c, int nit, int *changed, int *conv)
{
    int rc;
    const size_t ne = c->nel;
    const int nblk = (int)((ne + BLOCK - 1) / BLOCK);
    if (!c->kh_out) {
        if ((rc = dalloc(c, &c->kh_out, ne)) || (rc = dalloc(c, &c->kh_new, ne)) || (rc = dalloc(c, &c->kh_touch, ne)) ||
            (rc = dalloc(c, &c->wh_bmax, (size_t)nblk)) || (rc = dalloc(c, &c->wh_cnt, 4)) ||
            (rc = dalloc(c, &c->wh_snap_el, tan_words(ne))) || (rc = dalloc(c, &c->wh_snap_M, (size_t)6 * c->nel_total)) ||
            (rc = dalloc(c, &c->wh_snap_ms, ne)))
            return rc;
    }
    HIPCHK(c, hipMemcpyAsync(c->wh_snap_el, c->tan_buf, tan_words(ne) * 8, hipMemcpyDeviceToDevice, c->stream));
    HIPCHK(c, hipMemcpyAsync(c->wh_snap_M, c->Mel, (size_t)6 * c->nel_total * 8, hipMemcpyDeviceToDevice, c->stream));
    HIPCHK(c, hipMemcpyAsync(c->wh_snap_ms, c->max_steps, ne * 4, hipMemcpyDeviceToDevice, c->stream));
    const int64_t sw0 = c->n_sweeps, tr0 = c->n_tangents_rewritten;
    int64_t tr_before = tr0;
    bool any_changed = false;
    const bool dirty0 = c->M_dirty;
    int32_t last[16];
    static const int wh_cap = getenv("PLFX_WH_MAXPASS") ? std::max(2, atoi(getenv("PLFX_WH_MAXPASS"))) : 512;
    const int max_pass = (int)std::min<size_t>(ne + 2, (size_t)wh_cap);
    int pass = 0;
    for (;; pass++) {
        if (pass > 0) {
            HIPCHK(c, hipMemcpyAsync(c->tan_buf, c->wh_snap_el, tan_words(ne) * 8, hipMemcpyDeviceToDevice, c->stream));
            HIPCHK(c, hipMemcpyAsync(c->Mel, c->wh_snap_M, (size_t)6 * c->nel_total * 8, hipMemcpyDeviceToDevice, c->stream));
            HIPCHK(c, hipMemcpyAsync(c->max_steps, c->wh_snap_ms, ne * 4, hipMemcpyDeviceToDevice, c->stream));
        }
        int ch = 0, cv = 0;
        tr_before = c->n_tangents_rewritten;
        if ((rc = sweep_once(c, nit, &ch, &cv, true))) return rc;
        any_changed = (ch != 0);
        if (changed) *changed = ch;
        if (conv) *conv = cv;
        HIPCHK(c, hipMemcpyAsync(c->kh_new, c->kh_el, ne * 8, hipMemcpyDeviceToDevice, c->stream));
        HIPCHK(c, hipMemsetAsync(c->wh_cnt, 0, 16, c->stream));
        for (int m = 0; m < c->nmat && m < 16; m++) {
            last[m] = -1;
            if (c->hmat[m].kind != 7) continue;
            hipLaunchKernelGGL(k_wh_blockmax, dim3(nblk), dim3(BLOCK), 0, c->stream, c->nel, m, c->dcls, c->dcls_id, c->kh_touch, c->wh_bmax);
            hipLaunchKernelGGL(k_wh_scan, dim3(1), dim3(BLOCK), 0, c->stream, nblk, c->wh_bmax, c->wh_cnt + 1);
            hipLaunchKernelGGL(k_wh_entry, dim3(nblk), dim3(BLOCK), 0, c->stream, c->nel, m, c->dcls, c->dcls_id, c->kh_touch, c->wh_bmax,
                               (const double *)c->kh_out, c->wh_carry[m], (const double *)c->kh_el, c->kh_new, c->wh_cnt);
            HIPCHK(c, hipGetLastError());
            int32_t h2[2];
            HIPCHK(c, hipMemcpyAsync(h2, c->wh_cnt, 8, hipMemcpyDeviceToHost, c->stream));
            HIPCHK(c, stream_sync(c));
            last[m] = h2[1];
        }
        int32_t nch = 0;
        HIPCHK(c, hipMemcpyAsync(&nch, c->wh_cnt, 4, hipMemcpyDeviceToHost, c->stream));
        HIPCHK(c, stream_sync(c));
        c->n_wh_passes++;
        if (getenv("PLFX_WH_DEBUG")) {
            std::vector<double> ko(ne), ki(ne);
            std::vector<int32_t> tc(ne);
            hipMemcpy(ko.data(), c->kh_out, ne * 8, hipMemcpyDeviceToHost);
            hipMemcpy(ki.data(), c->kh_el, ne * 8, hipMemcpyDeviceToHost);
            hipMemcpy(tc.data(), c->kh_touch, ne * 4, hipMemcpyDeviceToHost);
            int nt = 0;
            double kmax = 0., imax = 0.;
            for (size_t e = 0; e < ne; e++) nt += tc[e], kmax = std::max(kmax, ko[e]), imax = std::max(imax, ki[e]);
            fprintf(stderr, "[wh] sweep %lld pass %d: %d entries changed, %d touched, max entry %.6g, max exit %.6g, last touched %d, carry %.6g\n",
                    (long long)c->n_wh_sweeps, pass, nch, nt, imax, kmax, last[0], c->wh_carry[0]);
        }
        if (nch == 0) break;
        if (pass + 1 >= max_pass) {
            if (c->n_wh_unresolved++ == 0)
                fprintf(stderr, "[plfx] work-hardening carry chain not resolved after %d passes (%d entry moduli still changed): "
                                "PLFX_WH_MAXPASS raises the cap (plfx_wh_info counts such sweeps)\n", pass + 1, (int)nch);
            break;
        }
        std::swap(c->kh_el, c->kh_new);
    }
    for (int m = 0; m < c->nmat && m < 16; m++)
        if (c->hmat[m].kind == 7 && last[m] >= 0)
            HIPCHK(c, hipMemcpy(&c->wh_carry[m], c->kh_out + last[m], 8, hipMemcpyDeviceToHost));
    c->kh_out_valid = true;
    c->n_wh_sweeps++;
    c->n_sweeps = sw0 + 1;
    c->n_tangents_rewritten = tr0 + (c->n_tangents_rewritten - tr_before);
    c->M_dirty = dirty0 || any_changed;
    return PLFX_OK;
}

int plfx_sweep(plfx_ctx *c, int nit, int *changed, int *conv)
{
    if (!c || !c->sig) return c ? fail(c, PLFX_ERR_STATE, "set_mesh first") : PLFX_ERR_STATE;
    if (c->n_noflow) return fail(c, PLFX_ERR_UNSUPPORTED, "a Tresca / Barlat material without flow rule is loaded (material.py:822-825)");
    c->spec_setup = c->spec_kdu = false;
    if (wh_sequential(c)) return sweep_wh_sequential(c, nit, changed, conv);
    return sweep_once(c, nit, changed, conv, false);
}

// ... 267 lines not shown
```

Measured before the change: 5.592 billion.

## Let the plane sweep write tangents straight into the operator snapshot and defer setup

When a speculative, heavy-free, plane-only matrix-free sweep is possible, the light plane sweep kernel writes each changed element tangent directly into the packed operator copy (Mop). With mode bit 2 it can also skip writing the live Mel array. The assembly step then skips its separate setup pass and marks setup and the live Mel copy as owed. These are rebuilt lazily through new ensure_setup, ensure_live_M and before_M_write hooks placed at every consumer and writer of M. The aim is to cut one full-array pass and a kernel launch per load step. The cost is considerable state-tracking complexity and a risk of stale operator or tangent data if any path misses a hook.

```diff
diff --git a/include/plfx.h b/include/plfx.h
--- a/include/plfx.h
+++ b/include/plfx.h
@@ -135,6 +135,7 @@
 int plfx_sweep_launch_info(plfx_ctx *ctx, int64_t *heavy_skipped, int64_t *heavy_recovered);
 int plfx_bc_info(plfx_ctx *ctx, int64_t *rhs_rows_only, int64_t *dinv_kept, int64_t *dinv_refreshed, int64_t *du_early);
 int plfx_short_info(plfx_ctx *ctx, int64_t *dinv_deferred, int64_t *dinv_formed_late, int64_t *d_kept, int64_t *spec_merged);
+int plfx_snap_info(plfx_ctx *ctx, int64_t *direct_sweeps, int64_t *direct_acknowledged, int64_t *setup_formed_late, int64_t *live_restored);
 int plfx_dead_store_info(plfx_ctx *ctx, int64_t *armed_sweeps, int64_t *tangents_rewritten_in_armed_sweeps,
                          int64_t *test_only_starts, int64_t *test_only_retries);
 enum {
diff --git a/pylabfea_amd/_lib.py b/pylabfea_amd/_lib.py
--- a/pylabfea_amd/_lib.py
+++ b/pylabfea_amd/_lib.py
@@ -55,7 +55,7 @@
     'plfx_tex_svc_set', 'plfx_tex_svc_yf', 'plfx_tex_svc_yield_scale', 'plfx_tex_svc_info',
     'plfx_tex_svc_fgrad', 'plfx_tex_svc_full_yf', 'plfx_tex_svc_response', 'plfx_tex_svc_flow_info',
     'plfx_flow_curve', 'plfx_flow_info', 'plfx_load_path', 'plfx_load_path_info',
-    'plfx_dead_store_info', 'plfx_plane_info', 'plfx_short_info',
+    'plfx_dead_store_info', 'plfx_plane_info', 'plfx_short_info', 'plfx_snap_info',
     'plfx_set_svc_cols', 'plfx_mg_info',
     'plfx_set_svc_textures', 'plfx_set_element_textures', 'plfx_response_batch_tid', 'plfx_full_yf_batch_tid',
     'plfx_svc_textures_info',
@@ -736,6 +736,11 @@
         self._chk(self.lib.plfx_short_info(self.h, C.byref(a), C.byref(b), C.byref(r), C.byref(d)))
         return a.value, b.value, r.value, d.value
 
+    def snap_info(self):
+        a, b, r, d = C.c_int64(), C.c_int64(), C.c_int64(), C.c_int64()
+        self._chk(self.lib.plfx_snap_info(self.h, C.byref(a), C.byref(b), C.byref(r), C.byref(d)))
+        return a.value, b.value, r.value, d.value
+
     def dead_store_info(self):
         a, b, r, d = C.c_int64(), C.c_int64(), C.c_int64(), C.c_int64()
         self._chk(self.lib.plfx_dead_store_info(self.h, C.byref(a), C.byref(b), C.byref(r), C.byref(d)))
diff --git a/pylabfea_amd/csrc/plfx.hip b/pylabfea_amd/csrc/plfx.hip
--- a/pylabfea_amd/csrc/plfx.hip
+++ b/pylabfea_amd/csrc/plfx.hip
@@ -489,6 +489,7 @@
     dfree(c->bc_rows);
     c->bc_nrows = 0;
     c->rhs_rows_ok = c->dinv_ok = c->dinv_late = false;
+    c->direct_done = c->setup_owed = c->live_owed = false;
     dfree(c->tex_ids);
     c->htex_ids.clear();
     c->tex_ids_ok = false;
@@ -566,6 +567,7 @@
 int sync_M(plfx_ctx *c)
 {
     if (!comm_active(c) || !c->sharded) return 0;
+    if (int rc = before_M_write(c)) return rc;
     if (c->strip.on) return strip_sync_M(c);
     hipLaunchKernelGGL(k_zero_foreign_M, dim3(grid_for((size_t)6 * c->nel_total)), dim3(BLOCK), 0, c->stream,
                        c->nel_total, c->e0, c->e0 + c->nel, c->Mel);
@@ -703,6 +705,7 @@
 int ensure_dinv(plfx_ctx *c)
 {
     if (!c->dinv_late) return 0;
+    if (int rc = ensure_setup(c)) return rc;
     hipLaunchKernelGGL(k_dinv, dim3(grid_for(c->ndof)), dim3(BLOCK), 0, c->stream, (size_t)c->ndof, c->diag, c->is_presc, c->dinv);
     HIPCHK(c, hipGetLastError());
     c->dinv_late = false;
@@ -713,6 +716,8 @@
 int assemble_fine_val(plfx_ctx *c)
 {
     if (int rc = ensure_dinv(c)) return rc;
+    if (int rc = ensure_setup(c)) return rc;
+    if (int rc = ensure_live_M(c)) return rc;
     hipLaunchKernelGGL(k_assemble, dim3(grid_for(c->nnode), c->nslot), dim3(BLOCK), 0, c->stream,
                        c->dcls, c->ncls, c->nnode, c->nslot, c->nq, c->nel_total, c->dcontrib, c->dcls_all,
                        (matfree(c) && c->assembled) ? c->Mop : c->Mel, c->dcol, c->dval, c->diag,
@@ -732,6 +737,7 @@
 {
     const bool mf = matfree(c);
     const int nl = (int)c->mg.size();
+    if (int rc = ensure_setup(c)) return rc;
     c->mg_dinv_current = mf && c->bc_valid;
     for (int l = 1; l < nl; l++) {
         auto &F = c->mg[l - 1];
@@ -1190,6 +1196,47 @@
                        (double2 *)nullptr, 0x7fffffff, (const int *)(c->flags + 8));
 }
 
+int ensure_live_M(plfx_ctx *c)
+{
+    if (!c->live_owed) return 0;
+    hipLaunchKernelGGL(k_restore_M, dim3(grid_for((size_t)c->nel_total, 1 << 16)), dim3(BLOCK), 0, c->stream, (size_t)c->nel_total,
+                       (const double2 *)c->Mop, c->Mel);
+    HIPCHK(c, hipGetLastError());
+    c->live_owed = false;
+    c->n_live_restored++;
+    return 0;
+}
+
+int ensure_setup(plfx_ctx *c)
+{
+    if (!c->setup_owed) return 0;
+    if (int rc = ensure_live_M(c)) return rc;
+    KOp live = c->op;
+    live.M = c->Mel;
+    LAUNCH_SETUP(0, live, (double2 *)c->diag,
+                       c->Mop, (mg_active(c) && level_plain(c->mg[0])) ? c->mg[1].Mel : (double *)nullptr, (const double2 *)nullptr, 0, 0,
+                       (double2 *)nullptr);
+    HIPCHK(c, hipGetLastError());
+    c->setup_owed = false;
+    c->n_setup_late++;
+    return 0;
+}
+
+int before_M_write(plfx_ctx *c)
+{
+    c->direct_done = false;
+    if (int rc = ensure_setup(c)) return rc;
+    return ensure_live_M(c);
+}
+
+static int snap_settle(plfx_ctx *c)
+{
+    if (int rc = ensure_live_M(c)) return rc;
+    c->direct_done = c->setup_owed = false;
+    c->M_dirty = true;
+    return 0;
+}
+
 }
 }
 
@@ -1228,6 +1275,8 @@
     if (!c->reuse) c->plane_switch = false;
     if (const char *e12 = getenv("PLFX_SHORT_SOLVE")) c->short_solve = atoi(e12) & 3;
     if (!c->reuse) c->short_solve = 0;
+    if (const char *e13 = getenv("PLFX_DIRECT_SNAP")) c->direct_snap = atoi(e13) & 3;
+    if (!(c->direct_snap & 1) || !c->reuse) c->direct_snap = 0;
     if (const char *e9 = getenv("PLFX_PREDICT")) c->predict = atoi(e9) != 0;
     {
         const char *e5 = getenv("PLFX_MAILBOX");
@@ -1575,6 +1624,10 @@
 {
     if (!c || !c->Mel) return c ? fail(c, PLFX_ERR_STATE, "set_mesh first") : PLFX_ERR_STATE;
     if (e < c->e0 || e >= c->e0 + c->nel || !Kel) return fail(c, PLFX_ERR_ARG, "element not owned");
+    if (c->live_owed) {
+        if (int rc = ensure_live_M(c)) return rc;
+        HIPCHK(c, stream_sync(c));
+    }
     double M[6];
     for (int k = 0; k < 6; k++)
         HIPCHK(c, hipMemcpy(&M[k], c->Mel + (size_t)k * c->nel_total + e, 8, hipMemcpyDeviceToHost));
@@ -1790,6 +1843,7 @@
         return fail(c, PLFX_ERR_ARG, "grid %dx%d does not match the mesh", nx, ny);
     if (c->strip.on)
         return fail(c, PLFX_ERR_STATE, "plfx_set_grid after plfx_set_strip: call plfx_set_mesh again");
+    if (int rcs = snap_settle(c)) return rcs;
     const int nrow = ny + 1;
     const bool known = c->hint_nx == nx && c->hint_ny == ny;
     for (int e = 0; e < c->nel_total && !known; e++) {
@@ -1875,6 +1929,7 @@
     if (!c->grid_ok || !c->want_matfree || c->mg.size() < 2)
         return fail(c, PLFX_ERR_UNSUPPORTED, "a strip needs the uniform structured grid (matrix-free operator + multigrid)");
     if (c->colr) return fail(c, PLFX_ERR_UNSUPPORTED, "a strip needs element columns of one width");
+    if (int rcs = snap_settle(c)) return rcs;
     const int nx = c->gx, ny = c->gy, Ld = coarse_level;
     if (c->sharded && (c->e0 != own_col0 * ny || c->nel != (own_col1 - own_col0) * ny))
         return fail(c, PLFX_ERR_STATE, "the owned element range of plfx_set_mesh must be the owned columns of the strip (or the whole local mesh)");
@@ -2023,6 +2078,7 @@
     if (kind != 0 && kind != 1) return fail(c, PLFX_ERR_ARG, "operator kind must be 0 (assembled) or 1 (matrix-free)");
     if (c->strip.on && kind != 1) return fail(c, PLFX_ERR_UNSUPPORTED, "a strip (plfx_set_strip) runs the matrix-free operator only");
     if (kind != c->want_matfree) {
+        if (int rcs = snap_settle(c)) return rcs;
         mg_graph_drop(c);
         c->want_matfree = kind;
         c->assembled = false, c->M_dirty = true;
@@ -2069,6 +2125,16 @@
     if (dinv_formed_late) *dinv_formed_late = c->n_dinv_late;
     if (d_kept) *d_kept = c->n_d_kept;
     if (spec_merged) *spec_merged = 0;
+    return PLFX_OK;
+}
+
+int plfx_snap_info(plfx_ctx *c, int64_t *direct_sweeps, int64_t *direct_acknowledged, int64_t *setup_formed_late, int64_t *live_restored)
+{
+    if (!c) return PLFX_ERR_STATE;
+    if (direct_sweeps) *direct_sweeps = c->n_direct_sweeps;
+    if (direct_acknowledged) *direct_acknowledged = c->n_direct_ack;
+    if (setup_formed_late) *setup_formed_late = c->n_setup_late;
+    if (live_restored) *live_restored = c->n_live_restored;
     return PLFX_OK;
 }
 
@@ -2208,6 +2274,7 @@
                         "smoother chosen before plfx_set_strip");
         return PLFX_OK;
     }
+    if (int rcs = snap_settle(c)) return rcs;
     c->precond = kind;
     if (omega > 0.) c->mg_omega = omega;
     if (nu > 0) c->mg_nu = nu;
@@ -2294,8 +2361,9 @@
 int plfx_assemble(plfx_ctx *c)
 {
     if (!c || !c->dval) return c ? fail(c, PLFX_ERR_STATE, "set_mesh first") : PLFX_ERR_STATE;
-    const bool setup_done = c->spec_setup && c->spec_was_clean && c->spec_h0 != 0 && matfree(c);
-    c->spec_setup = c->spec_kdu = false;
+    const bool direct = c->direct_done && matfree(c) && c->M_dirty;
+    const bool setup_done = (c->spec_setup && c->spec_was_clean && c->spec_h0 != 0 && matfree(c)) || direct;
+    c->spec_setup = c->spec_kdu = c->direct_done = false;
     if (c->reuse && c->assembled && !c->M_dirty) {
         c->n_reuse_assemble++;
         return PLFX_OK;
@@ -2305,12 +2373,18 @@
     if (matfree(c)) {
         KOp live = c->op;
         live.M = c->Mel;
-        if (setup_done)
+        if (direct) {
+            c->n_direct_ack++;
+            c->setup_owed = true;
+        } else if (setup_done)
             c->n_spec_setup++;
-        else
+        else {
+            if (int rc = ensure_live_M(c)) return rc;
             LAUNCH_SETUP(0, live, (double2 *)c->diag,
                                c->Mop, (mg_active(c) && level_plain(c->mg[0])) ? c->mg[1].Mel : (double *)nullptr, (const double2 *)nullptr, 0, 0,
                                (double2 *)nullptr);
+            c->setup_owed = false;
+        }
         c->dinv_ok = false;
         c->val_valid = false;
     } else {
@@ -2493,11 +2567,13 @@
             c->n_dinv_refreshed++;
             c->n_dinv_deferred++;
         } else {
+            if ((rc = ensure_setup(c))) return rc;
             hipLaunchKernelGGL(k_dinv, dim3(grid_for(nd)), dim3(BLOCK), 0, c->stream, nd, c->diag, c->is_presc, c->dinv);
             c->n_dinv_refreshed++;
             c->dinv_late = false;
         }
     } else {
+        if ((rc = ensure_setup(c))) return rc;
         hipLaunchKernelGGL(k_bc_finish, dim3(grid_for(nd)), dim3(BLOCK), 0, c->stream, nd,
                            fext ? c->fext : nullptr, c->kw, c->diag, c->is_presc, c->rhs, c->dinv);
         c->rhs_rows_ok = !fext;
diff --git a/pylabfea_amd/csrc/plfx_host.hpp b/pylabfea_amd/csrc/plfx_host.hpp
--- a/pylabfea_amd/csrc/plfx_host.hpp
+++ b/pylabfea_amd/csrc/plfx_host.hpp
@@ -188,6 +188,9 @@
     bool mg_pending = false, mg_pending_same = true;
     long long n_mg_setup = 0, n_mg_setup_skipped = 0;
     bool spec_arm = false, spec_setup = false, spec_kdu = false, spec_was_clean = false;
+    int direct_snap = 3;
+    bool direct_done = false, setup_owed = false, live_owed = false;
+    long long n_direct_sweeps = 0, n_direct_ack = 0, n_setup_late = 0, n_live_restored = 0;
     bool dead_stores = true, test_starts = true, dead_arm = false, res_partial = false;
     long long n_dead_sweeps = 0, n_dead_tangents = 0, n_test_starts = 0, n_test_retries = 0;
     bool plane_switch = true, plane_mats_ok = false, plane_cols = false;
@@ -514,6 +517,9 @@
 void launch_mbox_post(plfx_ctx *c, const double *src, int n, double *dst, CgMbox *mb, unsigned long long seq);
 void launch_kdu_uf(plfx_ctx *c, CgScalars *spec);
 void launch_spec_setup(plfx_ctx *c);
+int ensure_live_M(plfx_ctx *c);
+int ensure_setup(plfx_ctx *c);
+int before_M_write(plfx_ctx *c);
 
 int ensure_eps(plfx_ctx *c);
 int split_res_sig(plfx_ctx *c);
diff --git a/pylabfea_amd/csrc/plfx_kernels.hpp b/pylabfea_amd/csrc/plfx_kernels.hpp
--- a/pylabfea_amd/csrc/plfx_kernels.hpp
+++ b/pylabfea_amd/csrc/plfx_kernels.hpp
@@ -810,7 +810,8 @@
                                                int oform, const double *ofac, int omax,
                                                double *Mel, int mel_stride, double *res_sig,
                                                double *res_depl, double *fyn, int32_t *max_steps, int nit,
-                                               int &changed, int &nconv, double kh = -1., int dead_ok = 0)
+                                               int &changed, int &nconv, double kh = -1., int dead_ok = 0,
+                                               double *snap = nullptr, size_t snap_nel = 0, size_t snap_e = 0)
 {
     const bool late = MAY_SKIP && dead_ok;
     if (!late) {
@@ -871,8 +872,16 @@
         }
         double M[6];
         tangent_to_M(Dnew, c.kappa, M);
-#pragma unroll
-        for (int k = 0; k < 6; k++) Mel[(size_t)k * mel_stride + e] = M[k];
+        if (!AHEAD || Mel) {
+#pragma unroll
+            for (int k = 0; k < 6; k++) Mel[(size_t)k * mel_stride + e] = M[k];
+        }
+        if (AHEAD && snap) {
+            double2 *S2 = reinterpret_cast<double2 *>(snap);
+            S2[snap_e] = make_double2(M[0], M[1]);
+            S2[snap_nel + snap_e] = make_double2(M[2], M[3]);
+            S2[2 * snap_nel + snap_e] = make_double2(M[4], M[5]);
+        }
         changed += 1;
     }
     if (ns > omax) max_steps[e] = ns;
@@ -1108,7 +1117,8 @@
                     const int32_t *__restrict__ cls, const double2 *__restrict__ du2,
                     const double *__restrict__ sig, const double *__restrict__ epl, TanStore ts,
                     double *Mel, int mel_stride, double *res_sig, double *res_depl, double *fyn,
-                    int32_t *max_steps, int nit, int *flags, int *bflags, int32_t *list, int first_kind, unsigned skip_mask, int dead_ok)
+                    int32_t *max_steps, int nit, int *flags, int *bflags, int32_t *list, int first_kind, unsigned skip_mask, int dead_ok,
+                    double *snap )
 {
     __shared__ SweepTables tb;
     stage_tables(tb, gmat, nmat, gcls, ncls);
@@ -1164,7 +1174,8 @@
                     heavy = true;
                 else
                     sweep_epilogue<true, true, true>(c, m, e, nel, s, ep, depl, st, Ct, fy, 0, ts, in.form, in.fac, 0, Mel, mel_stride,
-                                                     res_sig, res_depl, fyn, max_steps, nit, changed, nconv, -1., dead_ok);
+                                                     res_sig, res_depl, fyn, max_steps, nit, changed, nconv, -1., dead_ok,
+                                                     snap, (size_t)mel_stride, (size_t)e + e_off);
             }
         }
         const unsigned long long mask = __ballot(heavy);
@@ -1534,6 +1545,21 @@
 {
     return pair ? ((size_t)(c >> 1) * nel + e) * 2 + (c & 1) : (size_t)c * nel + e;
 }
+
+#ifdef PLFX_UNIT_OPERATOR
+__global__ void __launch_bounds__(BLOCK)
+k_restore_M(size_t nel, const double2 *__restrict__ snap, double *__restrict__ Mel)
+{
+    for (size_t e = (size_t)blockIdx.x * BLOCK + threadIdx.x; e < nel; e += (size_t)gridDim.x * BLOCK) {
+#pragma unroll
+        for (int p = 0; p < 3; p++) {
+            const double2 v = snap[(size_t)p * nel + e];
+            Mel[(size_t)(2 * p) * nel + e] = v.x;
+            Mel[(size_t)(2 * p + 1) * nel + e] = v.y;
+        }
+    }
+}
+#endif
 
 __host__ __device__ inline void structured_slot(int nx, int ny, int i, int s, int32_t *col, int32_t *codes )
 {
diff --git a/pylabfea_amd/csrc/plfx_step.hip b/pylabfea_amd/csrc/plfx_step.hip
--- a/pylabfea_amd/csrc/plfx_step.hip
+++ b/pylabfea_amd/csrc/plfx_step.hip
@@ -167,6 +167,7 @@
     c->plane_cols = c->plane_off_by == PLFX_PLANE_ON;
     if (c->plane_cols) HIPCHK(c, hipMemsetAsync(c->elfac + 4 * ne, 0, 16 * ne, c->stream));
     c->assembled = false, c->M_dirty = true;
+    c->direct_done = c->setup_owed = c->live_owed = false;
     c->x_is_du = false;
     c->rhs_rows_ok = c->dinv_ok = false;
     c->pred_d_kept = false;
@@ -314,6 +315,7 @@
     HIPCHK(c, hipMemcpyAsync(p, t.data(), 8 * comps * n, hipMemcpyHostToDevice, c->stream));
     if (which == 5) {
         c->M_dirty = true;
+        if (int rcw = before_M_write(c)) return rcw;
         HIPCHK(c, hipMemsetAsync(c->eltag, TAN_FULL, n, c->stream));
         hipLaunchKernelGGL(k_refresh_M, dim3((c->nel + BLOCK - 1) / BLOCK), dim3(BLOCK), 0, c->stream,
                            c->dmat, c->dcls, c->nel, c->dcls_id, tan_store(c), c->Mel + c->e0, c->nel_total);
@@ -583,6 +585,16 @@
     const int dead = (c->dead_arm && c->dead_stores && !comm_active(c) && !c->strip.on && !wh_seq && (c->has_analytic || c->has_princ)) ? 1 : 0;
     c->dead_arm = false;
     c->res_partial = dead != 0;
+    const bool mb_flags = !comm_active(c) && c->mbox && c->mb_cap >= 2;
+    const bool skip_heavy = mb_flags && !c->strip.on && c->last_heavy == 0;
+    const bool spec = c->spec_arm && !comm_active(c) && c->mbox && c->mb_cap >= 2 && matfree(c) && !c->strip.on && c->assembled;
+    c->spec_arm = false;
+    const bool plane_only = plane_active(c) && c->has_analytic && !c->has_princ && !c->has_barlat && !c->has_svc && !c->has_svc3 &&
+                            !c->has_svcwh && !c->svc_row_all;
+    const bool direct = (c->direct_snap & 1) && spec && plane_only && skip_heavy && !c->M_dirty && !c->op.colr && !wh_seq && c->Mop;
+    const bool direct_only = direct && (c->direct_snap & 2);
+    if (!direct)
+        if (int rcw = before_M_write(c)) return rcw;
     EvPair *ev;
     tim_begin(c, 0, &ev);
 #define SWEEP_ARGS(lds) c->dmat, c->nmat, c->dcls, c->ncls, lds, c->nel, c->e0, c->dconn, c->dcls_id,          \
@@ -597,7 +609,14 @@
                   c->max_steps, nit, c->flags, c->bflags, c->heavy_list
     if (c->has_analytic || (c->has_elastic && !c->has_princ && !c->has_svc && !c->has_svc3 && !c->has_barlat && !c->has_svcwh && !c->svc_cols_mask)) {
         if (plane_active(c)) {
-            hipLaunchKernelGGL(k_sweep_light_plane, dim3(plane_sweep_grid(c)), dim3(BLOCK), 0, c->stream, SWEEP_ARGS(0), first, 0u, dead);
+            if (direct)
+                hipLaunchKernelGGL(k_sweep_light_plane, dim3(plane_sweep_grid(c)), dim3(BLOCK), 0, c->stream, c->dmat, c->nmat, c->dcls,
+                                   c->ncls, 0, c->nel, c->e0, c->dconn, c->dcls_id, (const double2 *)c->du, c->sig, c->epl, tan_store(c),
+                                   direct_only ? (double *)nullptr : c->Mel + c->e0, c->nel_total, c->res_sig, c->res_depl, c->fyn,
+                                   c->max_steps, nit, c->flags, c->bflags, c->heavy_list, first, 0u, dead, c->Mop);
+            else
+                hipLaunchKernelGGL(k_sweep_light_plane, dim3(plane_sweep_grid(c)), dim3(BLOCK), 0, c->stream, SWEEP_ARGS(0), first, 0u, dead,
+                                   (double *)nullptr);
             c->n_plane_sweeps++;
         } else
             hipLaunchKernelGGL(HIP_KERNEL_NAME(k_sweep_light<1>), dim3(c->grid_el), dim3(BLOCK), 0, c->stream,
@@ -649,8 +668,6 @@
         first = 0;
     }
     tim_end(c, ev);
-    const bool mb_flags = !comm_active(c) && c->mbox && c->mb_cap >= 2;
-    const bool skip_heavy = mb_flags && !c->strip.on && c->last_heavy == 0;
     auto launch_phase2 = [&]() {
         tim_begin(c, 6, &ev);
         if (c->has_analytic)
@@ -690,26 +707,32 @@
     else
         launch_phase2();
     int h[4];
-    const bool spec = c->spec_arm && !comm_active(c) && c->mbox && c->mb_cap >= 2 && matfree(c) && !c->strip.on && c->assembled;
-    c->spec_arm = false;
     if (mb_flags) {
         const unsigned long long seq = ++c->mbox_seq;
         hipLaunchKernelGGL(k_sweep_flags, dim3(1), dim3(BLOCK), 0, c->stream, c->bflags, c->flags, c->flags + 4,
                            reinterpret_cast<int *>(c->mb_buf), c->mbox, seq, spec ? c->flags + 8 : (int *)nullptr,
                            spec ? c->spec_sc : (CgScalars *)nullptr, skip_heavy ? 1 : 0);
         if (spec) {
-            launch_spec_setup(c);
+            if (!direct) launch_spec_setup(c);
             launch_kdu_uf(c, c->spec_sc);
             c->spec_was_clean = !c->M_dirty;
-            c->spec_setup = c->spec_kdu = true;
+            c->spec_setup = !direct;
+            c->spec_kdu = true;
+            if (direct) c->n_direct_sweeps++;
         }
         HIPCHK(c, hipGetLastError());
+        bool recovered = false;
         const int rcw = mbox_wait(c, seq);
         if (rcw) return rcw;
         memcpy(h, c->mb_buf, sizeof(h));
         if (skip_heavy && h[0] < 0) {
             c->n_heavy_recovered++;
             c->spec_setup = c->spec_kdu = false;
+            recovered = true;
+            if (direct_only) {
+                c->live_owed = true;
+                if (int rcl = ensure_live_M(c)) return rcl;
+            }
             launch_phase2();
             const unsigned long long seq2 = ++c->mbox_seq;
             hipLaunchKernelGGL(k_sweep_flags, dim3(1), dim3(BLOCK), 0, c->stream, c->bflags, c->flags, c->flags + 4,
@@ -722,6 +745,10 @@
         c->spec_h0 = h[0];
         c->spec_h1 = h[1];
         if (spec && h[0]) c->dinv_ok = false;
+        if (direct && h[0] && !recovered) {
+            c->direct_done = true;
+            if (direct_only) c->live_owed = true;
+        }
     } else {
         hipLaunchKernelGGL(k_sweep_flags, dim3(1), dim3(BLOCK), 0, c->stream, c->bflags, c->flags, c->flags + 4);
         HIPCHK(c, hipGetLastError());
@@ -762,6 +789,7 @@
             (rc = dalloc(c, &c->wh_snap_ms, ne)))
             return rc;
     }
+    if ((rc = before_M_write(c))) return rc;
     HIPCHK(c, hipMemcpyAsync(c->wh_snap_el, c->tan_buf, tan_words(ne) * 8, hipMemcpyDeviceToDevice, c->stream));
     HIPCHK(c, hipMemcpyAsync(c->wh_snap_M, c->Mel, (size_t)6 * c->nel_total * 8, hipMemcpyDeviceToDevice, c->stream));
     HIPCHK(c, hipMemcpyAsync(c->wh_snap_ms, c->max_steps, ne * 4, hipMemcpyDeviceToDevice, c->stream));
```

Result: faster. 5.928 billion, median of 6 (+6.0%).
